# rrwick/Autocycler

Measured on AMD Instinct MI355X. Metric: Mbp/sec through compress->unitig GFA (k=51), higher is better.
Workload: dtype u64

## Files before the change

### autocycler_amd/csrc/capi.cpp

```cpp
#include <algorithm>
#include <cstring>
#include <memory>

#include "capi_common.hpp"
#include "gfa_writer.hpp"

using namespace ac;
using namespace ac::abi;

static void select_device(int device, bool refresh_tuning = true) {
    if (refresh_tuning) tuning_refresh();
#ifndef AC_EMU
    int n = 0;
    hipError_t e = hipGetDeviceCount(&n);
    if (e != hipSuccess || n == 0)
        throw DeviceError("no HIP device available: the MI355X backend has no CPU fallback");
    if (device < 0 || device >= n) throw DeviceError("invalid HIP device ordinal " + std::to_string(device));
    AC_HIP_CHECK(hipSetDevice(device));
    hipDeviceProp_t prop;
    AC_HIP_CHECK(hipGetDeviceProperties(&prop, device));
    if (std::string(prop.gcnArchName).rfind("gfx950", 0) != 0)
        throw DeviceError(std::string("device is ") + prop.gcnArchName + "; this library is built for gfx950 only");
#endif
    int& arena_device = device_ctx().arena_device;
    if (arena_device != device) {
        if (arena_device >= 0) {
            if (g_live_shards) throw DeviceError("a sharded build is in flight on device " + std::to_string(arena_device) + ": this process cannot use device " + std::to_string(device) + " until it is freed");
            Arena::device().release_all();
#ifndef AC_EMU
            Mailbox::get().release();
#endif
        }
        arena_device = device;
    }
}

namespace ac {
void select_device_checked(int device) { select_device(device, false); }

namespace abi __attribute__((visibility("hidden"))) {

std::string& last_error() { static thread_local std::string err; return err; }
std::mutex g_build_mutex;
int g_live_shards = 0;
std::atomic<int> g_host_side_device{0};

DeviceCall::DeviceCall(int device, Kind kind) : lock(g_build_mutex) {
    if (g_live_shards && kind != SHARD_PHASE)
        throw DeviceError(kind == SHARD_BEGIN ? "another sharded build is in flight in this process" : "a sharded build is in flight in this process");
    if (kind == ALL_DEVICES) tuning_refresh();
    else select_device(device);
}

void validate(uint32_t k, const ac_seq_view* seqs, uint32_t n_seqs) {
    if (!seqs || n_seqs == 0) throw DeviceError("no sequences found in input assemblies");
    if (k % 2 == 0) throw DeviceError("--kmer must be odd");
    if (n_seqs > 32767) throw DeviceError("no more than 32767 input sequences are allowed");
    for (uint32_t i = 0; i < n_seqs; i++) {
        if (!seqs[i].fwd) throw DeviceError("null sequence pointer");
        if (seqs[i].length < k) throw DeviceError("sequence shorter than k");
    }
}

void validate_layout(uint32_t k, uint64_t n_text, const uint64_t* off, const uint32_t* len, const uint16_t* d1, const uint16_t* d2,
                     uint32_t n_seqs) {
    if (k < 1 || k % 2 == 0) throw DeviceError("--kmer must be odd");
    if (!off || !len || !d1 || !d2) throw DeviceError("null sequence table");
    uint64_t prev_end = 0;
    for (uint32_t i = 0; i < n_seqs; i++) {
        if (len[i] < k) throw DeviceError("sequence " + std::to_string(i + 1) + " is shorter than k");
        const uint64_t plen = (uint64_t)len[i] + k - 1;
        if (off[i] != prev_end + 1) throw DeviceError("sequence table: sequence " + std::to_string(i + 1) + " does not start right behind the separator of the previous one");
        if (off[i] + plen + 1 > n_text) throw DeviceError("sequence table: sequence " + std::to_string(i + 1) + " runs past the end of the text");
        if (d1[i] > k - 1 || d2[i] > k - 1 || (uint32_t)d1[i] + d2[i] > k - 1) throw DeviceError("sequence table: more padding dots than k - 1 on sequence " + std::to_string(i + 1));
        prev_end = off[i] + plen;
    }
    if (n_seqs && prev_end + 1 != n_text) throw DeviceError("sequence table: the text does not end with the separator of the last sequence");
}

std::vector<SeqView> seq_views(const ac_seq_view* seqs, uint32_t n_seqs, std::vector<uint16_t>* seq_ids, std::vector<uint32_t>* seq_lens) {
    std::vector<SeqView> v(n_seqs);
    for (uint32_t i = 0; i < n_seqs; i++) {
        v[i] = SeqView{seqs[i].fwd, seqs[i].length};
        seq_ids->push_back(seqs[i].id);
        seq_lens->push_back(seqs[i].length);
    }
    return v;
}

void set_device_text(GraphBuilder& b, const void* d_text, uint64_t n_text, const uint64_t* seq_off, const uint32_t* seq_len,
                     const uint16_t* ids, const uint16_t* seq_d1, const uint16_t* seq_d2, uint32_t n_seqs,
                     std::vector<uint16_t>* seq_ids, std::vector<uint32_t>* seq_lens) {
    std::vector<uint64_t> off(seq_off, seq_off + n_seqs);
    std::vector<uint32_t> len(seq_len, seq_len + n_seqs);
    std::vector<uint16_t> d1(seq_d1, seq_d1 + n_seqs), d2(seq_d2, seq_d2 + n_seqs);
    seq_ids->assign(ids, ids + n_seqs);
    *seq_lens = len;
    b.set_text_device((const uint8_t*)d_text, n_text, off, len, d1, d2);
}

}
}

static void build_graph(GraphBuilder& b, uint32_t assembly_count, ac_graph* h) {
    b.build(assembly_count, &h->g);
    h->tm = b.timings();
}

template <class T> static size_t copy_sized(const T& full, T* out, size_t out_size) {
    memcpy(out, &full, std::min(out_size, sizeof full));
    return sizeof full;
}

extern "C" {

const char* ac_last_error(void) { return last_error().c_str(); }
const char* ac_version(void) {
#ifdef AC_EMU
    return "autocycler_amd 0.1 (CPU emulation, tests only)";
#else
    return "autocycler_amd 0.1 (gfx950)";
#endif
}
int ac_abi_version(void) { return AC_ABI_VERSION; }
int ac_set_host_side_device(int device) { if (device < 0) return fail("invalid HIP device ordinal"); g_host_side_device.store(device); return 0; }
void ac_set_stage_timing(int on) { set_stage_timing(on != 0); }
int ac_release_memory(void) {
    return guarded([&] {
        std::lock_guard<std::mutex> lock(g_build_mutex);
        if (g_live_shards) throw DeviceError("a sharded build is in flight in this process");
        Arena::device().release_all();
        release_multi_contexts();
        PinnedPool::get().trim();
        release_host_stager();
        scan_pool().release();
#ifndef AC_EMU
        Mailbox::get().release();
#endif
    });
}
uint32_t ac_max_kmer(void) { int m = max_supported_k(); return (uint32_t)(m % 2 ? m : m - 1); }
int ac_device_count(void) {
#ifndef AC_EMU
    int n = 0;
    if (hipGetDeviceCount(&n) != hipSuccess) return 0;
    return n;
#else
    return 0;
#endif
}

uint64_t ac_text_size(uint32_t k, const ac_seq_view* seqs, uint32_t n_seqs) {
    uint64_t n = 1;
    for (uint32_t i = 0; i < n_seqs; i++) n += (uint64_t)seqs[i].length + k - 1 + 1;
    return n;
}
int ac_layout_text(uint32_t k, const ac_seq_view* seqs, uint32_t n_seqs, uint8_t* text, uint64_t* seq_off,
                   uint16_t* seq_d1, uint16_t* seq_d2) {
    return guarded([&] {
        std::vector<SeqView> v(n_seqs);
        for (uint32_t i = 0; i < n_seqs; i++) v[i] = SeqView{seqs[i].fwd, seqs[i].length};
        std::vector<uint64_t> off; std::vector<uint32_t> len; std::vector<uint16_t> d1, d2;
        std::vector<uint8_t> t = layout_text(v, k, &off, &len, &d1, &d2);
        memcpy(text, t.data(), t.size());
        for (uint32_t i = 0; i < n_seqs; i++) { seq_off[i] = off[i]; seq_d1[i] = d1[i]; seq_d2[i] = d2[i]; }
    });
}

int ac_pack_text(const uint8_t* text, uint64_t n_text, uint64_t* bits, uint32_t* mask32, int force_scalar) {
    return guarded([&] {
        if (!text || !bits || !mask32) throw DeviceError("null pointer");
        pack_text_host(text, n_text, bits, mask32, force_scalar != 0);
    });
}

int ac_compress_build(uint32_t k, uint32_t assembly_count, const ac_seq_view* seqs, uint32_t n_seqs, int device,
                      ac_graph** out) {
    return guarded([&] {
        validate(k, seqs, n_seqs);
        DeviceCall call(device);
        auto h = std::make_unique<ac_graph>();
        const std::vector<SeqView> v = seq_views(seqs, n_seqs, &h->seq_ids, &h->seq_lens);
        GraphBuilder b(k);
        b.set_sequences_host(v);
        build_graph(b, assembly_count, h.get());
        *out = h.release();
    });
}

int ac_compress_build_multi(uint32_t k, uint32_t assembly_count, const ac_seq_view* seqs, uint32_t n_seqs, const int* devices, int n_devices,
                            ac_graph** out) {
    return guarded([&] {
        validate(k, seqs, n_seqs);
        if (!devices || n_devices < 1) throw DeviceError("ac_compress_build_multi: no devices");
        if (n_devices > 64) throw DeviceError("ac_compress_build_multi: more than 64 devices");
        DeviceCall call(-1, DeviceCall::ALL_DEVICES);
        auto h = std::make_unique<ac_graph>();
        const std::vector<SeqView> v = seq_views(seqs, n_seqs, &h->seq_ids, &h->seq_lens);
        int transport = MULTI_AUTO;
        if (const int e = tuning_multi_transport()) transport = e == 1 ? MULTI_HOST_STAGED : MULTI_RCCL;
        build_multi(k, assembly_count, v, std::vector<int>(devices, devices + n_devices), transport, &h->g, &h->tm, &h->multi);
        *out = h.release();
    });
}
int ac_multi_info_get(const ac_graph* g, ac_multi_info* o) {
    if (!g || !o) return fail("null pointer");
    const MultiStats& m = g->multi;
    memset(o, 0, sizeof *o);
    o->n_ranks = m.n_ranks; o->transport = m.transport;
    o->bytes_fragments = m.bytes_fragments; o->bytes_bitmap = m.bytes_bitmap; o->bytes_degrees = m.bytes_degrees; o->bytes_links = m.bytes_links;
    o->bytes_queries = m.bytes_queries; o->bytes_answers = m.bytes_answers; o->bytes_reduce = m.bytes_reduce;
    o->queries_total = m.queries_total; o->queries_sent_away = m.queries_sent_away;
    o->table_capacity_max = m.table_capacity_max; o->table_capacity_sum = m.table_capacity_sum;
    o->union_text_bytes = m.union_text_bytes; o->fragments = m.fragments; o->distinct = m.distinct;
    o->seconds_total = m.seconds_total; o->seconds_exchange_max = m.seconds_exchange_max;
    o->candidates_total = m.candidates_total; o->candidates_owned_max = m.candidates_owned_max;
    o->bytes_sibling = m.bytes_sibling; o->bytes_tail = m.bytes_tail; o->degrees_open = m.degrees_open; o->bytes_received_max = m.bytes_received_max;
    o->path_runs_copied = m.path_runs_copied;
    return 0;
}
size_t ac_multi_info_get_sized(const ac_graph* g, ac_multi_info* out, size_t out_size) {
    ac_multi_info t;
    if (!g || !out) { fail("null pointer"); return sizeof t; }
    ac_multi_info_get(g, &t);
    return copy_sized(t, out, out_size);
}

int ac_compress_build_device(uint32_t k, uint32_t assembly_count, const void* d_text, uint64_t n_text,
                             const uint64_t* seq_off, const uint32_t* seq_len, const uint16_t* seq_ids,
                             const uint16_t* seq_d1, const uint16_t* seq_d2, uint32_t n_seqs, int device,
                             ac_graph** out) {
    return guarded([&] {
        if (!d_text || n_seqs == 0) throw DeviceError("no sequences found in input assemblies");
        if (n_seqs > 32767) throw DeviceError("no more than 32767 input sequences are allowed");
        validate_layout(k, n_text, seq_off, seq_len, seq_d1, seq_d2, n_seqs);
        DeviceCall call(device);
        auto h = std::make_unique<ac_graph>();
        GraphBuilder b(k);
        set_device_text(b, d_text, n_text, seq_off, seq_len, seq_ids, seq_d1, seq_d2, n_seqs, &h->seq_ids, &h->seq_lens);
        build_graph(b, assembly_count, h.get());
        *out = h.release();
    });
}

uint32_t ac_graph_seq_count(const ac_graph* g) { return (uint32_t)g->seq_ids.size(); }
int ac_path_counts(const ac_graph* g, uint64_t* counts) {
    for (size_t s = 0; s + 1 < g->g.path_off.size(); s++) counts[s] = g->g.path_off[s + 1] - g->g.path_off[s];
    return 0;
}

uint32_t ac_graph_kmer_size(const ac_graph* g) { return g->g.k; }
int ac_graph_seq_info(const ac_graph* g, uint32_t i, uint16_t* id, uint32_t* length, const char** filename, const char** header) {
    if (i >= g->seq_ids.size()) return fail("sequence index out of range");
    if (id) *id = g->seq_ids[i];
    if (length) *length = g->seq_lens[i];
    if (filename) *filename = i < g->filenames.size() ? g->filenames[i].c_str() : nullptr;
    if (header) *header = i < g->headers.size() ? g->headers[i].c_str() : nullptr;
    return 0;
}

uint64_t ac_kmer_count(const ac_graph* g) { return g->g.n_kmers; }
ac_stats ac_stats_pre(const ac_graph* g) { return ac_stats{g->g.pre.unitigs, g->g.pre.links_one_way, g->g.pre.total_length}; }
ac_stats ac_stats_post(const ac_graph* g) { return ac_stats{g->g.post.unitigs, g->g.post.links_one_way, g->g.post.total_length}; }
uint32_t ac_unitig_count(const ac_graph* g) { return g->g.n_unitigs; }

int ac_unitig(const ac_graph* g, uint32_t idx, const uint8_t** seq, uint32_t* len, double* depth) {
    if (idx >= g->g.n_unitigs) return fail("unitig index out of range");
    if (!g->host_arrays) return fail("this rank kept no host arrays (sharded build, not the writing rank)");
    if (seq) *seq = (const uint8_t*)g->g.seq(idx);
    if (len) *len = g->g.seq_len[idx];
    if (depth) *depth = g->g.depth[idx];
    return 0;
}
int ac_unitig_positions(ac_graph* g, uint32_t idx, int forward, const ac_position** positions, uint32_t* n) {
    if (idx >= g->g.n_unitigs) return fail("unitig index out of range");
    return guarded([&] {
        if (!g->host_arrays || !g->host_paths) throw DeviceError("this rank kept no host arrays (sharded build, not the writing rank)");
        if (!g->positions_built) { build_positions(&g->g, g->seq_ids, g->seq_lens); g->positions_built = true; }
        auto& v = forward ? g->g.fwd_positions[idx] : g->g.rev_positions[idx];
        static_assert(sizeof(ac_position) == sizeof(Position), "layout");
        *positions = (const ac_position*)v.data();
        *n = (uint32_t)v.size();
    });
}
int ac_links(const ac_graph* g, const ac_link** links, uint64_t* n) {
    static_assert(sizeof(ac_link) == sizeof(Link), "layout");
    if (!g->host_arrays) return fail("this rank kept no host arrays (sharded build, not the writing rank)");
    *links = (const ac_link*)g->g.links;
    *n = g->g.n_links;
    return 0;
}
int ac_path(const ac_graph* g, uint32_t seq_index, const int32_t** signed_unitigs, uint32_t* n) {
    if ((size_t)seq_index + 1 >= g->g.path_off.size()) return fail("sequence index out of range");
    if (!g->host_paths) return fail("this rank kept no paths on the host (sharded build)");
    uint64_t b = g->g.path_off[seq_index], e = g->g.path_off[seq_index + 1];
    *signed_unitigs = g->g.path + b;
    *n = (uint32_t)(e - b);
    return 0;
}
int ac_unitigs_bulk(const ac_graph* g, const uint8_t** seq_bytes, const uint64_t** seq_begin, const uint32_t** seq_len, const double** depth) {
    if (!g->host_arrays) return fail("this rank kept no host arrays (sharded build, not the writing rank)");
    if (seq_bytes) *seq_bytes = (const uint8_t*)g->g.seq_block.p;
    if (seq_begin) *seq_begin = g->g.seq_begin;
    if (seq_len) *seq_len = g->g.seq_len;
    if (depth) *depth = g->g.depth;
    return 0;
}
int ac_paths_bulk(const ac_graph* g, const int32_t** path_entries, const uint64_t** path_off, uint64_t* n_entries) {
    if (!g->host_paths) return fail("this rank kept no paths on the host (sharded build)");
    if (path_entries) *path_entries = g->g.path;
    if (path_off) *path_off = g->g.path_off.data();
    if (n_entries) *n_entries = g->g.n_path;
    return 0;
}
int ac_timings_get(const ac_graph* g, ac_timings* o) {
    const BuildTimings& t = g->tm;
    o->h2d = t.h2d; o->pack = t.pack; o->insert = t.insert; o->collect_sort = t.collect_sort; o->degree = t.degree;
    o->segment = t.segment; o->minkey = t.minkey; o->rank = t.rank; o->paths = t.paths; o->links = t.links; o->seqs = t.seqs;
    o->d2h = t.d2h; o->total_device = t.total_device; o->expand = t.expand;
    o->insert_kernel_ms = t.insert_kernel_ms; o->insert_positions = t.insert_positions;
    o->table_capacity = t.table_capacity; o->n_distinct = t.n_distinct; o->n_path_entries = t.n_path_entries;
    o->simplify_passes = t.simplify_passes; o->n_candidates = t.n_candidates; o->n_levels = t.n_levels;
    o->insert_launches = t.insert_launches; o->insert_real = t.insert_real;
    o->analysis = t.analysis; o->finalize = t.finalize;
    o->fragments = t.fragments; o->union_pack = t.union_pack; o->union_insert = t.union_insert;
    o->n_local_distinct = t.n_local_distinct; o->n_fragments = t.n_fragments; o->fragment_bytes = t.fragment_bytes;
    o->upload_device_ms = t.upload_device_ms;
    o->path_runs_copied = t.path_runs_copied; o->path_entries_walked = t.path_entries_walked; o->position_retries = t.position_retries;
    o->n_candidates_owned = t.n_candidates_owned;
    o->launches = t.launches; o->readbacks = t.readbacks; o->n_degrees_open = t.n_degrees_open; o->sort_retries = t.sort_retries;
    o->insert_rest_known = t.insert_rest_known; o->insert_rest_sampled = t.insert_rest_sampled; o->path_stretches = t.path_stretches;
    o->expand_sparse_sweeps = t.expand_sparse_sweeps; o->expand_sparse_start = t.expand_sparse_start;
    return 0;
}
size_t ac_timings_get_sized(const ac_graph* g, ac_timings* out, size_t out_size) {
    ac_timings t;
    memset(&t, 0, sizeof t);
    ac_timings_get(g, &t);
    return out ? copy_sized(t, out, out_size) : sizeof t;
// ... 29 lines not shown
```

### autocycler_amd/csrc/device_rt.hpp

```cpp
#pragma once
#include <cstdio>
#include <cstdlib>
#include <cstring>
#include <stdexcept>
#include <string>
#include <vector>
#include <algorithm>

#include <mutex>
#include <time.h>
#include <unistd.h>

#include "kmer_ops.hpp"
#include "graph_types.hpp"
#include "wave_rt.hpp"

#ifndef AC_EMU
#include <hip/hip_runtime.h>
#endif
#if defined(AC_EMU) && defined(AC_ARENA_GUARD)
#include <sanitizer/asan_interface.h>
#define AC_GUARD_LEVEL AC_ARENA_GUARD
#else
#define AC_GUARD_LEVEL 0
#endif

namespace ac {

struct DeviceError : std::runtime_error { using std::runtime_error::runtime_error; };
struct NeedExactPositions {};
struct NeedCheckedSorts {};

#ifndef AC_EMU
#define AC_HIP_CHECK(expr)                                                                              \
    do {                                                                                                \
        hipError_t _e = (expr);                                                                         \
        if (_e != hipSuccess)                                                                           \
            throw ::ac::DeviceError(std::string("HIP error: ") + hipGetErrorString(_e) + " at " + __FILE__ + ":" + \
                                    std::to_string(__LINE__) + " (" #expr ")");                        \
    } while (0)
typedef hipStream_t stream_t;
#else
typedef int stream_t;
#endif

#ifdef AC_EMU
inline u64 atomic_cas64(u64* p, u64 expected, u64 desired) { u64 old = *p; if (old == expected) *p = desired; return old; }
inline u64 atomic_min64(u64* p, u64 v) { u64 o = *p; if (v < o) *p = v; return o; }
inline void atomic_max64(u64* p, u64 v) { if (v > *p) *p = v; }
inline void atomic_xor64(u64* p, u64 v) { *p ^= v; }
inline u32 atomic_add32(u32* p, u32 v) { u32 o = *p; *p += v; return o; }
inline u64 atomic_add64(u64* p, u64 v) { u64 o = *p; *p += v; return o; }
inline void atomic_or32(u32* p, u32 v) { *p |= v; }
inline void atomic_or64(u64* p, u64 v) { *p |= v; }
inline void atomic_min32(u32* p, u32 v) { if (v < *p) *p = v; }
inline void atomic_max32(u32* p, u32 v) { if (v > *p) *p = v; }
inline u32 atomic_cas32(u32* p, u32 expected, u32 desired) { u32 old = *p; if (old == expected) *p = desired; return old; }
inline u32 atomic_load32(const u32* p) { return *p; }
inline u32 atomic_fetch_or32(u32* p, u32 v) { u32 o = *p; *p |= v; return o; }
inline u32 atomic_fetch_and32(u32* p, u32 v) { u32 o = *p; *p &= v; return o; }
#else
__device__ inline u64 atomic_cas64(u64* p, u64 expected, u64 desired) {
    return (u64)atomicCAS((unsigned long long*)p, (unsigned long long)expected, (unsigned long long)desired);
}
__device__ inline u64 atomic_min64(u64* p, u64 v) { return (u64)atomicMin((unsigned long long*)p, (unsigned long long)v); }
__device__ inline void atomic_max64(u64* p, u64 v) { atomicMax((unsigned long long*)p, (unsigned long long)v); }
__device__ inline void atomic_xor64(u64* p, u64 v) { atomicXor((unsigned long long*)p, (unsigned long long)v); }
__device__ inline u32 atomic_add32(u32* p, u32 v) { return atomicAdd(p, v); }
__device__ inline u64 atomic_add64(u64* p, u64 v) { return (u64)atomicAdd((unsigned long long*)p, (unsigned long long)v); }
__device__ inline void atomic_or32(u32* p, u32 v) { atomicOr(p, v); }
__device__ inline void atomic_or64(u64* p, u64 v) { atomicOr((unsigned long long*)p, (unsigned long long)v); }
__device__ inline void atomic_min32(u32* p, u32 v) { atomicMin(p, v); }
__device__ inline void atomic_max32(u32* p, u32 v) { atomicMax(p, v); }
__device__ inline u32 atomic_cas32(u32* p, u32 expected, u32 desired) { return atomicCAS(p, expected, desired); }
__device__ inline u32 atomic_load32(const u32* p) { return __hip_atomic_load(p, __ATOMIC_RELAXED, __HIP_MEMORY_SCOPE_AGENT); }
__device__ inline u32 atomic_fetch_or32(u32* p, u32 v) { return atomicOr(p, v); }
__device__ inline u32 atomic_fetch_and32(u32* p, u32 v) { return atomicAnd(p, v); }
#endif

struct RtCounters { u32 launches = 0, readbacks = 0; };
inline RtCounters& rt_counters() { static thread_local RtCounters c; return c; }

struct DeviceCtx {
    static const int SLOTS = 10;
    void* obj[SLOTS] = {}; void (*del[SLOTS])(void*) = {};
    int arena_device = -1;
    DeviceCtx() {}
    DeviceCtx(const DeviceCtx&) = delete;
    DeviceCtx& operator=(const DeviceCtx&) = delete;
    ~DeviceCtx() { for (int i = SLOTS; i-- > 0;) if (obj[i]) del[i](obj[i]); }
};
inline DeviceCtx*& tl_device_ctx() { static thread_local DeviceCtx* p = nullptr; return p; }
inline DeviceCtx& device_ctx() {
    static DeviceCtx* const process_wide = new DeviceCtx;
    DeviceCtx* p = tl_device_ctx();
    return p ? *p : *process_wide;
}
inline void set_device_ctx(DeviceCtx* c) { tl_device_ctx() = c; }
enum { CTX_ARENA = 0, CTX_FILLS, CTX_MAILBOX, CTX_SIDE, CTX_SCRATCH, CTX_STAGER, CTX_POOL, CTX_SCANPOOL_RESERVED, CTX_POOL2 };
template <class T> T& ctx_object(int slot) {
    DeviceCtx& c = device_ctx();
    if (!c.obj[slot]) { c.obj[slot] = new T(); c.del[slot] = [](void* p) { delete (T*)p; }; }
    return *(T*)c.obj[slot];
}

class Arena {
  public:
    static Arena& device() { return ctx_object<Arena>(CTX_ARENA); }
    Arena() : host_(false) {}
    ~Arena() { for (auto& b : blocks_) raw_free(b.p); }
    static const size_t COALESCE_LIMIT = (size_t)16 << 30;
#if AC_GUARD_LEVEL
    static const size_t RED_ZONE = 256;
    static void guard_poison(const void* p, size_t n) { if (n) __asan_poison_memory_region(p, n); }
    static void guard_unpoison(const void* p, size_t n) { if (n) __asan_unpoison_memory_region(p, n); }
#else
    static const size_t RED_ZONE = 0;
    static void guard_poison(const void*, size_t) {}
    static void guard_unpoison(const void*, size_t) {}
#endif
    static void keep_readable(const void* p, size_t bytes) { guard_unpoison(p, bytes); }
    void* alloc(size_t bytes) {
        [[maybe_unused]] const size_t asked = bytes;
        bytes = (bytes + 255) & ~(size_t)255;
        if (bytes == 0) bytes = 256;
        bytes += RED_ZONE;
        size_t i = cur_;
        while (i < blocks_.size() && blocks_[i].used + bytes > blocks_[i].cap) i++;
        if (i == blocks_.size()) {
            Block b; b.cap = std::max(bytes, grow_); b.used = 0; b.p = raw_alloc(b.cap);
            blocks_.push_back(b);
        }
        cur_ = i;
        Block& b = blocks_[i];
        void* r = (char*)b.p + b.used;
        b.used += bytes;
        peak_ = std::max(peak_, total_used());
        guard_poison(r, bytes); guard_unpoison(r, asked);
        return r;
    }
    void reset() {
        on_reset();
        const size_t last_peak = peak_;
        peak_ = 0; cur_ = 0;
        size_t total = 0;
        for (auto& b : blocks_) total += b.cap;
        if (blocks_.size() > 1 && total <= COALESCE_LIMIT) {
            for (auto& b : blocks_) raw_free(b.p);
            if (last_peak) total = std::min(total, last_peak + last_peak / 8 + ((size_t)256 << 20));
            blocks_.clear();
            Block b; b.cap = total; b.used = 0; b.p = raw_alloc(total);
            blocks_.push_back(b);
        } else {
            for (auto& b : blocks_) { b.used = 0; guard_poison(b.p, b.cap); }
        }
    }
    void reserve(size_t bytes) {
        if (capacity() >= bytes || total_used() != 0) return;
        release_all();
        Block b; b.cap = bytes; b.used = 0; b.p = raw_alloc(bytes);
        blocks_.push_back(b);
    }
    void release_all() {
        on_reset();
        for (auto& b : blocks_) raw_free(b.p);
        blocks_.clear(); cur_ = 0;
    }
    struct Mark { size_t block, used; bool empty; };
    Mark mark() const { return blocks_.empty() ? Mark{0, 0, true} : Mark{cur_, blocks_[cur_].used, false}; }
    void rewind(const Mark& m) {
        on_rewind();
        if (blocks_.empty()) return;
        cur_ = m.empty ? 0 : m.block;
        const size_t keep = m.empty ? 0 : m.used;
        if (AC_GUARD_LEVEL >= 2) {
            if (blocks_[cur_].used > keep) guard_poison((char*)blocks_[cur_].p + keep, blocks_[cur_].used - keep);
            for (size_t i = cur_ + 1; i < blocks_.size(); i++) guard_poison(blocks_[i].p, blocks_[i].used);
        }
        blocks_[cur_].used = keep;
        for (size_t i = cur_ + 1; i < blocks_.size(); i++) blocks_[i].used = 0;
    }
    size_t peak() const { return peak_; }
    double alloc_seconds() const { return alloc_s_; }
    size_t total_used() const { size_t t = 0; for (auto& b : blocks_) t += b.used; return t; }
    size_t capacity() const { size_t t = 0; for (auto& b : blocks_) t += b.cap; return t; }
    void set_grow(size_t g) { grow_ = g; }
    size_t grow() const { return grow_; }
    bool locate(const void* p, size_t* block, size_t* offset, size_t* used) const {
        for (size_t i = 0; i < blocks_.size(); i++) {
            const char* lo = (const char*)blocks_[i].p;
            if ((const char*)p < lo || (const char*)p >= lo + blocks_[i].cap) continue;
            *block = i; *offset = (size_t)((const char*)p - lo); *used = blocks_[i].used;
            return true;
        }
        return false;
    }

  private:
    struct Block { void* p; size_t cap, used; };
    void on_reset();
    void on_rewind();
    static double wall() { timespec ts; clock_gettime(CLOCK_MONOTONIC, &ts); return (double)ts.tv_sec + 1e-9 * (double)ts.tv_nsec; }
    void* raw_alloc(size_t bytes) {
        const double t0 = wall();
        struct Acc { double& a; double t0; ~Acc() { a += wall() - t0; } } acc{alloc_s_, t0};
#ifdef AC_EMU
        void* p = malloc(bytes);
        if (!p) throw DeviceError("emu malloc failed");
        guard_poison(p, bytes);
        return p;
#else
        void* p = nullptr;
        if (host_) AC_HIP_CHECK(hipHostMalloc(&p, bytes, hipHostMallocDefault));
        else AC_HIP_CHECK(hipMalloc(&p, bytes));
        return p;
#endif
    }
    void raw_free(void* p) {
        const double t0 = wall();
#ifdef AC_EMU
        for (auto& b : blocks_) if (b.p == p) guard_unpoison(b.p, b.cap);
        free(p);
#else
        if (host_) (void)hipHostFree(p); else (void)hipFree(p);
#endif
        alloc_s_ += wall() - t0;
    }
    double alloc_s_ = 0;
    bool host_;
    std::vector<Block> blocks_;
    size_t grow_ = (size_t)64 << 20;
    size_t peak_ = 0, cur_ = 0;
};

class PinnedPool {
  public:
    static PinnedPool& get() { static PinnedPool p; return p; }
    HostBlock alloc(size_t bytes) {
        if (bytes == 0) bytes = 1;
        HostBlock b;
        {
            std::lock_guard<std::mutex> lock(mu_);
            size_t best = free_.size();
            for (size_t i = 0; i < free_.size(); i++)
                if (free_[i].cap >= bytes && free_[i].cap <= 2 * bytes + 4096 && (best == free_.size() || free_[i].cap < free_[best].cap)) best = i;
            if (best != free_.size()) {
                b.p = free_[best].p; b.bytes = free_[best].cap;
                held_ -= free_[best].cap;
                free_.erase(free_.begin() + (long)best);
            }
        }
        if (!b.p) {
// ... 671 lines not shown
```

### autocycler_amd/csrc/graph_build.hpp

```cpp
#pragma once
#include <cstdint>
#include <functional>
#include <string>
#include <vector>

#include "graph_types.hpp"
#include "trim_host.hpp"
#include "resolve_host.hpp"
#include "components_host.hpp"
#include "merge_host.hpp"
#include "subset_host.hpp"
#include "trim_apply_host.hpp"
#include "finish_host.hpp"
#include "apply_host.hpp"
#include "clean_host.hpp"
#include "cluster_host.hpp"
#include "cluster_qc_host.hpp"

namespace ac {

struct SeqView {
    const uint8_t* fwd;
    uint32_t length;
};

struct BuildTimings {
    double h2d = 0, pack = 0, insert = 0, collect_sort = 0, degree = 0, segment = 0, minkey = 0, rank = 0,
           paths = 0, links = 0, seqs = 0, d2h = 0, total_device = 0;
    double expand = 0;
    double analysis = 0;
    double finalize = 0;
    double insert_kernel_ms = 0;
    uint64_t insert_positions = 0;
    uint64_t table_capacity = 0;
    uint64_t n_distinct = 0;
    uint64_t n_path_entries = 0;
    uint32_t insert_launches = 0;
    uint64_t insert_real = 0;
    uint32_t simplify_passes = 0, n_candidates = 0, n_levels = 0;
    uint32_t n_candidates_owned = 0;
    uint32_t local_hint = 0, graph_hint = 0;
    double fragments = 0;
    double union_pack = 0, union_insert = 0;
    uint64_t n_local_distinct = 0, n_fragments = 0, fragment_bytes = 0;
    double upload_device_ms = 0;
    double insert_rest_known = 0;
    uint64_t path_stretches = 0;
    uint32_t expand_sparse_sweeps = 0;
    uint32_t expand_sparse_start = 0;
    double insert_rest_sampled = 0;
    uint32_t sort_retries = 0;
    uint32_t position_retries = 0;
    uint32_t launches = 0, readbacks = 0;
    uint64_t n_degrees_open = 0;
    uint64_t path_runs_copied = 0, path_entries_walked = 0;
};

struct RepairTimings { double total = 0, scan_ms = 0; uint64_t hits = 0, matches = 0; uint32_t patterns = 0; };

class GraphBuilder {
  public:
    explicit GraphBuilder(uint32_t k);
    ~GraphBuilder();
    void set_sequences_host(const std::vector<SeqView>& seqs, bool pack_now = true);
    void repair_ends(RepairTimings* tm);
    void set_text_device(const uint8_t* d_text, uint64_t n_text, const std::vector<uint64_t>& off,
                         const std::vector<uint32_t>& len, const std::vector<uint16_t>& d1,
                         const std::vector<uint16_t>& d2);
    void build(uint32_t assembly_count_hint, FinalGraph* out);

    void shard_begin(uint32_t local_assembly_hint);
    uint64_t local_distinct_count() const;
    void set_distinct_upper_bound(uint64_t n);
    uint64_t fragment_text_bytes() const;
    uint64_t fragment_count() const;
    void fragments_export(void* d_text_out, void* d_meta_out);
    uint64_t fragment_packed_words(uint64_t union_off) const;
    void fragments_export_packed(uint64_t union_off, void* d_words_out, void* d_meta_out);
    void shard_build_union_packed(uint32_t rank, uint32_t n_shards, const void* d_staged_words, const uint64_t* first_word, const uint64_t* n_words,
                                  uint64_t n_union_text, const void* d_meta, uint64_t n_frags_total);
    void shard_build_union(uint32_t rank, uint32_t n_shards, const uint8_t* d_union_text, uint64_t n_union_text,
                           const void* d_meta, uint64_t n_frags_total);
    uint64_t bitmap_words() const;
    void bitmap_export(void* d_out);
    void shard_build_novel(const void* d_bitmap_sum);
    uint64_t sib_words() const;
    void sib_export(void* d_out);
    void shard_degrees(const void* d_sib_sum);
    uint64_t degree_bytes() const;
    uint64_t distinct_count() const;
    void degrees_export(void* d_out);
    void shard_build_graph(const void* d_kinfo_sum);
    uint32_t unitig_count() const;
    void links_export(void* d_links_i32, void* d_wlinks_i64);
    void links_import(const void* d_links_i32, const void* d_wlinks_i64);
    uint64_t query_count() const;
    uint32_t query_key_words() const;
    void queries_export(void* d_out);
    void answer_queries(const void* d_keys, uint64_t n, void* d_out);
    void shard_walk(const void* d_answers_mine);
    void queries_route(uint32_t n_shards, void* d_routed_keys, uint64_t* counts_host);
    void shard_walk_routed(const void* d_routed_answers);
    void reduce_export(int32_t* d_sum, int32_t* d_min);
    void reduce_import(const int32_t* d_sum, const int32_t* d_min);
    void set_tail_exchange(std::function<void(void*, uint64_t, int, int)> all_reduce);
    void shard_finish(FinalGraph* out, bool want_graph, bool want_paths);
    uint64_t path_entry_count() const;
    void paths_export(void* d_out);
    const BuildTimings& timings() const { return tm_; }
    void set_sequence_index_base(uint64_t n);
    static void set_upload_threads_cap(int n);
    uint64_t n_text() const;
    uint64_t n_bases() const;

    struct Impl;

  private:
    void build_union_impl(uint32_t rank, uint32_t n_shards, const uint8_t* d_union_text, const void* d_staged_words, const uint64_t* first_word,
                          const uint64_t* n_words, uint64_t n_union_text, const void* d_meta, uint64_t n_frags_total);
    void upload_packed(const std::vector<SeqView>& seqs, const std::vector<uint64_t>& off);
    Impl* impl_;
    BuildTimings tm_;
};

std::vector<uint8_t> layout_text(const std::vector<SeqView>& seqs, uint32_t k, std::vector<uint64_t>* off,
                                 std::vector<uint32_t>* len, std::vector<uint16_t>* d1, std::vector<uint16_t>* d2);

void end_repair_device(uint32_t k, uint8_t* d_text, uint64_t n_text, const std::vector<uint64_t>& off, const std::vector<uint32_t>& len,
                       std::vector<uint16_t>* d1, std::vector<uint16_t>* d2, RepairTimings* tm, bool reset_arena = true);

void pairwise_distances_device(const FinalGraph& g, uint32_t n_seqs, double* out);

struct VerifyReport {
    uint32_t failed = 0;
    uint64_t first_bad_unitig = ~0ULL, first_bad_link = ~0ULL, first_bad_path_entry = ~0ULL, first_bad_sequence = ~0ULL, first_bad_base = ~0ULL;
    uint64_t unitigs = 0, links = 0, path_entries = 0, bases_checked = 0, self_mirror_links = 0;
    double seconds = 0;
    uint32_t checks = 0;
    uint64_t first_bad_junction = ~0ULL;
};
void verify_graph_device(const FinalGraph& g, const uint8_t* d_text, uint64_t n_text, const std::vector<uint64_t>& off,
                         const std::vector<uint32_t>& len, VerifyReport* rep);

void decompress_device(const FinalGraph& g, const std::vector<uint32_t>& seq_len, uint8_t* out_host);
struct TrimDeviceStats { double seconds_device = 0; uint64_t cells = 0; uint32_t jobs = 0, launches = 0; };
void overlap_alignment_batch(const std::vector<AlignJob>& jobs, const uint32_t* weights, uint32_t max_unitigs, std::vector<AlignOut>* outs,
                             TrimDeviceStats* st);
uint32_t trim_max_unitigs();
struct ResolveDeviceStats { double seconds_device = 0; uint64_t cells = 0, jobs = 0, largest_job_cells = 0; uint32_t launches = 0; };
void path_distance_batch(const PathPool& pool, const std::vector<PathPair>& pairs, const uint32_t* weights, std::vector<uint32_t>* dist,
                         ResolveDeviceStats* st);
uint32_t resolve_max_path();
struct ClusterDeviceStats { double seconds = 0; uint64_t rescans = 0, compares = 0; uint32_t launches = 0; };
void cluster_merges_device(const double* asym, uint32_t n, std::vector<ClusterRowMerge>* merges, ClusterDeviceStats* st);
void cluster_merges_graph_device(const FinalGraph& g, uint32_t n_seqs, double* asym_out, std::vector<ClusterRowMerge>* merges, ClusterDeviceStats* st);
uint32_t cluster_max_seqs();
struct ClusterQcDeviceStats {
    double seconds = 0;
    uint32_t launches = 0, readbacks = 0, evaluations = 0, pair_batches = 0;
    uint64_t alternatives = 0, pairs_counted = 0, bytes_read_back = 0;
};
void cluster_qc_device(const double* asym, uint32_t n, const uint32_t* dfs_tip, double cutoff, const std::function<void(const ClusterQcEvaluate&)>& body,
                       ClusterQcDeviceStats* st);
void components_device(uint32_t n_unitigs, const Link* links, uint64_t n_links, const uint32_t* unitig_len, const uint8_t* alive, const uint8_t* marked,
                       ComponentsResult* out);
struct MergePlanInput {
    uint32_t n_unitigs = 0; const Link* links = nullptr; uint64_t n_links = 0; const uint32_t* unitig_len = nullptr; const uint8_t* alive = nullptr;
    const uint8_t* seed_fixed = nullptr; const int32_t* path = nullptr; uint64_t n_path = 0;
    const uint8_t* seq_bytes = nullptr; const uint64_t* seq_begin = nullptr; uint64_t seq_total = 0;
};
void merge_plan_device(const MergePlanInput& in, MergeResult* out);
struct SubsetInput {
    uint32_t n_unitigs = 0; const Link* links = nullptr; uint64_t n_links = 0; const uint32_t* unitig_len = nullptr; const uint8_t* alive = nullptr;
    const int32_t* path = nullptr; const uint64_t* path_off = nullptr; uint32_t n_clusters = 0; const SubsetPlan* plan = nullptr;
};
void subsets_device(const SubsetInput& in, SubsetResult* out);
struct MergedPathsInput {
    uint32_t n_unitigs = 0; const uint32_t* unitig_len = nullptr; const int32_t* path = nullptr; const uint64_t* path_off = nullptr;
    const SubsetPlan* plan = nullptr; size_t kept_first = 0, kept_count = 0; const MergeResult* merge = nullptr;
};
void merged_paths_device(const MergedPathsInput& in, MergedPathsResult* out);
struct TrimApplyInput {
    uint32_t n_unitigs = 0; const Link* links = nullptr; uint64_t n_links = 0; const uint32_t* unitig_len = nullptr; const uint8_t* alive = nullptr;
    const int32_t* path = nullptr; const uint64_t* path_off = nullptr; double mad = 0;
};
void trim_apply_device(const TrimApplyInput& in, TrimApplyPlan* tp, SubsetPlan* plan, SubsetResult* out);
struct FinishInput {
    uint32_t n_unitigs = 0; const Link* links = nullptr; uint64_t n_links = 0; const uint32_t* unitig_len = nullptr; const uint8_t* alive = nullptr;
    const double* depth = nullptr; const uint8_t* type = nullptr; const uint8_t* seq_bytes = nullptr; const uint64_t* seq_begin = nullptr; uint64_t seq_total = 0;
    const MergeResult* plan = nullptr; const int32_t* path = nullptr; uint64_t n_path = 0; bool renumber = false; uint64_t unitigs_after = 0;
};
void merge_finish_device(const FinishInput& in, FinishResult* out);
void apply_bridges_device(const ApplyInput& in, const ApplyPlan& plan, ApplyResult* out);
void clean_device(const CleanInput& in, CleanResult* out);
void primitives_selftest(uint64_t n, uint64_t seed, int end_bit, int key_kind);
void selftest_scan(int kind, const void* in, uint64_t n, bool in_place, int misalign_in, int misalign_out, void* out);
void selftest_radix(const uint64_t* keys, const void* vals, uint64_t n, int begin_bit, int end_bit, int val_kind, uint64_t prep_n, int prep_bits, bool prep_reuse,
                    uint64_t* keys_out, void* vals_out);
void selftest_segments(int op, const uint32_t* seg, const uint64_t* vals, uint64_t n, uint64_t n_segments, bool deferred_err, void* out, uint32_t* err_out);
void selftest_sort_cmp(int form, const uint64_t* a, const uint32_t* b, const uint32_t* vals, uint64_t n, uint64_t* a_out, uint32_t* b_out, uint32_t* vals_out);
void selftest_scan_pool(int op, uint64_t value, uint64_t* out);
void selftest_wave(int program, const uint64_t* in_u64, const int32_t* aux_i32, const uint64_t* live_mask, uint64_t* out_u64);
void selftest_fills(const uint64_t* regions, uint64_t n_regions, int trigger, int mode, uint8_t* span, uint64_t span_bytes, uint32_t* launches_out);
void selftest_fill_order(uint64_t n, int byte1, uint64_t w_lo, uint64_t w_hi, int w_val, uint64_t from2, int byte2, uint64_t upto3, int byte3, uint8_t* out);
void selftest_readback(const uint8_t* data, uint64_t n_data, int path, const uint64_t* items, uint64_t n_items, uint8_t* out, uint32_t* counters_out);
void selftest_scalar_chain(const uint64_t* values, uint64_t n, uint64_t* out, uint32_t* counters_out);
void selftest_arena(const uint64_t* ops, uint64_t n_ops, uint64_t* totals_out, uint64_t* allocs_out, const uint8_t* live, uint64_t* wrong_out);
void selftest_launch(int which, uint64_t n, uint64_t* slots_out, uint32_t* info_out);
void selftest_atomics(int op, uint64_t init, uint64_t expected, const uint64_t* operand, const uint32_t* target, uint32_t n_words, uint64_t* words_out, uint64_t* returns_out);
void selftest_side_order(int mode, int which, uint32_t seed, uint64_t n_words, uint32_t* out_words);
void selftest_event_ring(int op, const uint8_t* kinds, uint32_t n_more, uint64_t* out);

void random_access_ceilings(double* cas_gops, double* read_gops, uint64_t table_slots = (uint64_t)1 << 24);

void device_warmup(int device, uint32_t k = 0, uint64_t text_bytes_estimate = 0);

void pack_text_host(const uint8_t* text, uint64_t n_text, uint64_t* bits, uint32_t* mask32, bool force_scalar);

void release_host_stager();

int max_supported_k();
void tuning_refresh();
int tuning_multi_transport();
bool tuning_multi_fragments_as_bytes();
bool tuning_multi_tail_replicated();
void set_stage_timing(bool on);
bool stage_timing();

}
```

### autocycler_amd/csrc/graph_impl.hpp

```cpp
#pragma once
#include "graph_build.hpp"

#include <chrono>
#include <cmath>
#include <map>
#include <string>
#include <algorithm>
#include <atomic>
#include <thread>
#include <functional>
#include <condition_variable>
#include <mutex>
#include <fcntl.h>
#include <unistd.h>
#if defined(__x86_64__)
#include <immintrin.h>
#endif

#include "device_rt.hpp"

namespace ac {

static double now_s() {
    return std::chrono::duration<double>(std::chrono::steady_clock::now().time_since_epoch()).count();
}



static const int MAX_PROBES = 1 << 14;
static const int MAX_PROBES_INSERT = 1 << 10;
#ifndef AC_W_ONLY
#define AC_W_ONLY 0
#endif
extern bool g_stage_timing;

static const u32 KI_OUT_MASK = 7u, KI_IN_SHIFT = 3, KI_FIRST_T = 1u << 6, KI_FIRST_RCT = 1u << 7;

struct TextCtx {
    const u64* bits;
    const u64* mask;
    u64 n_text;
    int k;
    const u64* seq_off;
    const u32* seq_len;
    const u16* seq_d1;
    const u16* seq_d2;
    u32 n_seqs;
};

struct Table {
    u64* slots;
    u64 cap_mask;
    const u64* occ;
    u64* novel;
    u32 n_owners;
    u32 my_owner;
    u64* sflags;
    u64* full_at;
    u64* runs; u32* run_count; u64 run_row0;
};
static const u64 RUN_MIN = 128;
static const u32 RUN_ROW = 128;
AC_D void run_note(const Table& tb, u64 wave, u32& noted, u64 pj, u64 qj, bool same, u64 n) {
    if (!tb.runs || n < RUN_MIN || noted >= RUN_ROW) return;
    u64* rec = tb.runs + 3 * ((tb.run_row0 + wave) * RUN_ROW + noted);
    noted++;
    const bool with_anchor = ((tb.novel[qj >> 6] >> (qj & 63)) & 1) != 0;
    if (with_anchor) { rec[0] = pj; rec[1] = n + 1; rec[2] = qj | ((u64)(same ? 1 : 0) << 63); }
    else { rec[0] = pj + 1; rec[1] = n; rec[2] = (same ? qj + 1 : qj - 1) | ((u64)(same ? 1 : 0) << 63); }
}
AC_D void run_note_done(const Table& tb, u64 wave, u32 noted) { if (tb.runs) tb.run_count[tb.run_row0 + wave] = noted; }
AC_D void sib_note(const Table& tb, u64 s, u32 fl) { if (fl) atomic_or64(&tb.sflags[s >> 5], (u64)fl << (2 * (s & 31))); }
AC_HD u32 sib_bits(u64 v, u64 mine) {
    const u64 d = v ^ mine;
    if ((d >> TAG_MFP_SHIFT) != 0 || slot_isdot(v) || (d >> 41) == 0) return 0;
    return (((d >> TAG_X_SHIFT) & 3) == 0 ? 1u : 0u) | (((d >> TAG_Y_SHIFT) & 3) == 0 ? 2u : 0u);
}
AC_HD bool table_owns(const Table& tb, u64 home_hash) { return tb.n_owners <= 1 || (u32)((home_hash >> 40) % tb.n_owners) == tb.my_owner; }

AC_HD bool locate(const TextCtx& t, u64 p, u32* s_out, u32* f_out) {
    if (t.n_seqs == 0 || p < t.seq_off[0]) return false;
    u32 lo = 0, hi = t.n_seqs;
    while (hi - lo > 1) {
        u32 mid = lo + ((hi - lo) >> 1);
        if (t.seq_off[mid] <= p) lo = mid; else hi = mid;
    }
    u64 f = p - t.seq_off[lo];
    if (f >= (u64)t.seq_len[lo]) return false;
    *s_out = lo; *f_out = (u32)f;
    return true;
}

template <int W> AC_HD bool xkmer_at(const TextCtx& t, u64 p, XKmer<W>* x) {
    u32 s, f;
    if (!locate(t, p, &s, &f)) return false;
    int k = t.k;
    int plen = (int)t.seq_len[s] + k - 1;
    int ld = (int)t.seq_d1[s] - (int)f;
    int td = (int)f + k - (plen - (int)t.seq_d2[s]);
    x->ld = ld > 0 ? ld : 0;
    x->td = td > 0 ? td : 0;
    x->fwd = text_extract<W>(t.bits, p, k);
    return true;
}

template <int W> AC_HD int claimant_match(const TextCtx& t, u64 v, const Key<W>& ukey) {
    XKmer<W> y;
    if (!slot_isdot(v)) {
        y.fwd = text_extract<W>(t.bits, slot_pos(v), t.k);
        y.ld = 0; y.td = 0;
    } else {
        if (!xkmer_at<W>(t, slot_pos(v), &y)) return 0;
    }
    bool yf;
    Key<W> yk = xk_canonical<W>(y, t.k, &yf);
    if (!key_eq<W>(yk, ukey)) return 0;
    return yf ? 2 : 1;
}

struct FindResult { u64 pos; int claimant_flipped; bool found; };

template <int W> AC_HD FindResult table_find(const TextCtx& t, const Table& tb, const Key<W>& ukey, bool isdot) {
    const KeyPlace pl = key_place<W>(ukey, t.k, isdot, key_hash<W>(ukey));
    u64 tag = slot_make(pl.tag, isdot, 0);
    const u64 hh = pl.home;
    u64 s = hh & tb.cap_mask;
    FindResult r; r.found = false; r.pos = 0; r.claimant_flipped = 0;
    if (!table_owns(tb, hh)) return r;
    if (tb.occ && !((tb.occ[s >> 6] >> (s & 63)) & 1)) return r;
    for (int probes = 0; probes < MAX_PROBES; probes++) {
        u64 v = tb.slots[s];
        if (v == SLOT_EMPTY) return r;
        if (slot_tag_eq(v, tag)) {
            int m = claimant_match<W>(t, v, ukey);
            if (m) { r.found = true; r.pos = slot_pos(v); r.claimant_flipped = (m == 2); return r; }
        }
        s = (s + 1) & tb.cap_mask;
    }
    return r;
}

template <int W> AC_HD bool find_xk(const TextCtx& t, const Table& tb, const XKmer<W>& x, u64* pos, bool* rel_same) {
    bool flipped;
    Key<W> uk = xk_canonical<W>(x, t.k, &flipped);
    FindResult r = table_find<W>(t, tb, uk, x.ld > 0 || x.td > 0);
    if (!r.found) return false;
    *pos = r.pos;
    *rel_same = ((r.claimant_flipped != 0) == flipped);
    return true;
}

template <int W> AC_HD bool owns_xk(const TextCtx& t, const Table& tb, const XKmer<W>& x) {
    if (tb.n_owners <= 1) return true;
    bool flipped;
    Key<W> uk = xk_canonical<W>(x, t.k, &flipped);
    return table_owns(tb, key_home<W>(uk, t.k, x.ld > 0 || x.td > 0, key_hash<W>(uk)));
}

struct Novel {
    const u64* bm;
    const u32* wprefix;
};
AC_HD int popc64(u64 x) {
#ifdef AC_EMU
    return __builtin_popcountll(x);
#else
    return __popcll(x);
#endif
}
AC_HD u32 novel_rank(const Novel& nv, u64 pos) {
    u64 w = pos >> 6;
    int b = (int)(pos & 63);
    u64 below = b ? (nv.bm[w] & ((1ULL << b) - 1)) : 0;
    return nv.wprefix[w] + (u32)popc64(below);
}

static const u64 NOREF = ~0ULL;

template <int W> AC_D u64 table_insert(const TextCtx& t, const Table& tb, const Key<W>& ukey, bool isdot, bool flipped, u64 p,
                                       u32* claimed, u32* err, bool* same, bool* mine_now) {
    const KeyPlace pl = key_place<W>(ukey, t.k, isdot, key_hash<W>(ukey));
    u64 mine = slot_make(pl.tag, isdot, p);
    const u64 hh = pl.home;
    u64 s = hh & tb.cap_mask;
    *mine_now = false;
    if (!table_owns(tb, hh)) return NOREF;
    const bool note = tb.sflags != nullptr && !isdot;
    u32 my_fl = 0;
    for (int probes = 0; probes < MAX_PROBES_INSERT; probes++) {
        u64 v = tb.slots[s];
        if (v == SLOT_EMPTY) {
            u64 old = atomic_cas64(&tb.slots[s], SLOT_EMPTY, mine);
            if (old == SLOT_EMPTY) { (*claimed)++; *mine_now = true; if (note) sib_note(tb, s, my_fl); return NOREF; }
            v = old;
        }
        if (slot_tag_eq(v, mine)) {
            if (slot_pos(v) == p) { if (note) sib_note(tb, s, my_fl); return NOREF; }
            int m = claimant_match<W>(t, v, ukey);
            if (m) {
                if (note) sib_note(tb, s, my_fl);
                if (slot_pos(v) > p) {
                    u64 old = atomic_min64(&tb.slots[s], mine);
                    if (old > mine) {
                        *mine_now = true;
                        u64 q = slot_pos(old);
                        atomic_xor64(&tb.novel[q >> 6], 1ULL << (q & 63));
                    }
                    return NOREF;
                }
                *same = ((m == 2) == flipped);
                return slot_pos(v);
            }
        } else if (note) {
            const u32 fl = sib_bits(v, mine);
            if (fl) { sib_note(tb, s, fl); my_fl |= fl; }
        }
        s = (s + 1) & tb.cap_mask;
    }
    atomic_or32(err, 1u);
    if (tb.full_at) atomic_max64(tb.full_at, ~p);
    return NOREF;
}

struct alignas(16) V16 { u32 a, b, c, d; };

#include "kernels_table.inc"
#include "kernels_unitigs.inc"
#include "kernels_paths.inc"
#include "kernels_tail.inc"
#include "kernels_shard.inc"
struct PathRemapJob {
    int32_t* path = nullptr; u64 n_ent = 0;
    const int32_t* rec_val = nullptr; const u32* rec_pos = nullptr; u64 n_rec = 0;
    const u32* number = nullptr; u32 n_unitigs = 0;
    u64 ent_limit = ~0ULL;
    void* landed = nullptr; SideStream* side = nullptr;
    int dev = 0;
    std::atomic<u64> next{0}; std::atomic<int> ready{0};
    std::atomic<u32> bad{0};
    u64 ticket = 0; bool started = false;
    std::atomic<double> t_ready{0}, t_last{0};
};
void path_remap_range(int32_t* p, u64 n, const u32* number, u32 n_unitigs, std::atomic<u32>* bad);
void path_stretch_range(const PathRemapJob& j, u64 s0, u64 s1, std::atomic<u32>* bad);
bool path_remap_is_wide();
void path_remap_start(PathRemapJob& j, int threads);
void path_remap_finish(PathRemapJob& j) noexcept;
struct SeqExpandJob {
    const u64* words = nullptr; u8* out = nullptr; u64 total = 0;
    void* landed = nullptr; SideStream* side = nullptr; int dev = 0;
    std::atomic<u64> next{0}; std::atomic<int> ready{0};
    u64 ticket = 0; bool started = false;
    std::atomic<double> t_start{0}, t_ready{0}, t_last{0};
};
void seq_expand_range(const u64* words, u8* out, u64 b, u64 e);
void seq_expand_start(SeqExpandJob& j, int threads);
void seq_expand_finish(SeqExpandJob& j) noexcept;
[[maybe_unused]] static int key_words(int k) { int w = words_for_k(k); return w <= 4 ? w : (w <= 8 ? 8 : 16); }
[[maybe_unused]] static u64 next_pow2(u64 x) { u64 p = 1; while (p < x) p <<= 1; return p; }
[[maybe_unused]] static size_t arena_estimate(u64 n_text, bool owns_text) { return (size_t)n_text * (owns_text ? 8 : 7) + ((size_t)768 << 20); }
struct Knobs {
    int minkey_variant;
    int path_copy;
    u64 run_piece;
    u32 pos_cap;
    bool path_filter;
    int host_remap_mode;
    u32 remap_block;
    int minkey_prefix_bases;
    bool seed_prefix_sort;
    u32 seed_max_group;
    int seed_prefix_bits;
    u32 degree_region_cap;
    int upload_direct_mode;
    int upload_slots;
    int degree_flags;
    int table_shift;
    u64 wave_chunk_max;
    u64 insert_chunk_rest_env;
    bool host_pack;
    u32 expand_level_table;
    bool shard_path_copy;
    bool expand_rewrite_always;
    u32 expand_sparse_max, expand_sparse_list, expand_sparse_batch;
    u32 stretch_device_share;
    int seq_codes_transfer;
    int late_copies;
    bool seq_writer_plain;
    bool seq_writer_forced;
    u64 seed_radix_limit;
    bool upload_overlap;
    bool sort_checks_deferrable;
    bool shard_host_remap;
    bool shard_degree_flags;
    bool insert_adaptive;
    u64 insert_growth;
    u64 insert_waves_target;
    bool renum_two_pass;
    u32 renum_max_group;
    u32 path_chunk_env;
    long upload_threads_env;
    bool debug_arena;
    bool degree_diag;
    int multi_transport;
    int multi_fragments;
    int multi_tail;
    u64 trim_batch_bytes;
    u64 resolve_batch_bytes;
    static Knobs read() {
        Knobs k;
        k.minkey_variant = [&]() -> int { const char* e = getenv("AC_MINKEY_VARIANT"); return e ? atoi(e) : -1; }();
        k.path_copy = [&]() -> int { const char* e = getenv("AC_PATH_COPY"); return e ? (atoi(e) != 0 ? 1 : 0) : 2; }();
        k.run_piece = [&]() -> u64 { const char* e = getenv("AC_RUN_PIECE"); const long v = e ? atol(e) : 0; return v > 0 ? (u64)v : 4096; }();
        k.pos_cap = [&]() -> u32 { const char* e = getenv("AC_POS_CAP"); const long v = e ? atol(e) : 65536; return v < 0 ? 0u : (u32)std::min<long>(v, 0x3FFFFFFF); }();
        k.path_filter = [&]() -> bool { const char* e = getenv("AC_PATH_FILTER"); return e ? atoi(e) != 0 : true; }();
        k.host_remap_mode = [&]() -> int { const char* e = getenv("AC_HOST_REMAP"); return e ? (atoi(e) == 2 ? 2 : (atoi(e) != 0 ? 1 : 0)) : -1; }();
        k.remap_block = [&]() -> u32 { const char* e = getenv("AC_REMAP_BLOCK"); int v = e ? atoi(e) : 4096; v = v < 64 ? 64 : (v > 65536 ? 65536 : v); return (u32)(v & ~63); }();
        k.minkey_prefix_bases = [&]() -> int { const char* e = getenv("AC_MINKEY_PREFIX_BASES"); int v = e ? atoi(e) : 31; return v < 1 ? 1 : (v > 31 ? 31 : v); }();
        k.seed_prefix_sort = [&]() -> bool { const char* e = getenv("AC_SEED_PREFIX_SORT"); return e ? atoi(e) != 0 : true; }();
        k.seed_max_group = [&]() -> u32 { const char* e = getenv("AC_SEED_MAX_GROUP"); int v = e ? atoi(e) : 1024; return (u32)(v < 1 ? 1 : v); }();
        k.seed_prefix_bits = [&]() -> int { const char* e = getenv("AC_SEED_PREFIX_BITS"); if (!e) return 0; int v = atoi(e); return v < 1 ? 1 : (v > 64 ? 64 : v); }();
        k.degree_region_cap = [&]() -> u32 { const char* e = getenv("AC_DEGREE_REGION_CAP"); int v = e ? atoi(e) : 0; return (u32)(v < 0 ? 0 : v); }();
        k.upload_direct_mode = [&]() -> int { const char* e = getenv("AC_UPLOAD_DIRECT"); return e ? (atoi(e) != 0 ? 1 : 0) : -1; }();
        k.upload_slots = [&]() -> int { const char* e = getenv("AC_UPLOAD_SLOTS"); int v = e ? atoi(e) : 1 << 20; return v < 1 ? 1 : v; }();
        k.degree_flags = [&]() -> int { const char* e = getenv("AC_DEGREE_FLAGS"); return e ? (atoi(e) != 0 ? 1 : 0) : 1; }();
        k.table_shift = [&]() -> int { const char* e = getenv("AC_TABLE_SHIFT"); if (!e) return -1; int v = atoi(e); return v < 0 ? 0 : (v > 3 ? 3 : v); }();
        k.wave_chunk_max = [&]() -> u64 { const char* e = getenv("AC_INSERT_CHUNK"); u64 x = e ? (u64)atoll(e) : 8192; return (std::max<u64>(x, 256) + 63) & ~63ULL; }();
        k.insert_chunk_rest_env = [&]() -> u64 { const char* e = getenv("AC_INSERT_CHUNK_REST"); if (!e) return 0; return (std::max<u64>((u64)atoll(e), 256) + 63) & ~63ULL; }();
        k.host_pack = [&]() -> bool { const char* e = getenv("AC_HOST_PACK"); return e ? atoi(e) != 0 : true; }();
        k.expand_level_table = [&]() -> u32 { const char* e = getenv("AC_EXPAND_LEVEL_TABLE"); int v = e ? atoi(e) : 1024; return (u32)(v < 1 ? 1 : v); }();
        k.shard_path_copy = [&]() -> bool { const char* e = getenv("AC_SHARD_PATH_COPY"); return !(e && atoi(e) == 0); }();
        k.expand_rewrite_always = [&]() -> bool { return getenv("AC_EXPAND_REWRITE_ALWAYS") != nullptr; }();
        k.expand_sparse_max = [&]() -> u32 { const char* e = getenv("AC_EXPAND_SPARSE_MAX"); int v = e ? atoi(e) : 256; return (u32)(v < 0 ? 0 : v); }();
        k.late_copies = [&]() -> int { const char* e = getenv("AC_LATE_COPIES"); return e ? atoi(e) : 1; }();
        k.seq_codes_transfer = [&]() -> int { const char* e = getenv("AC_SEQ_CODES"); return e ? atoi(e) : 1; }();
        k.stretch_device_share = [&]() -> u32 { const char* e = getenv("AC_STRETCH_DEVICE_SHARE"); int v = e ? atoi(e) : 30; return (u32)(v < 0 ? 0 : v); }();
        k.expand_sparse_list = [&]() -> u32 { const char* e = getenv("AC_EXPAND_SPARSE_LIST"); int v = e ? atoi(e) : 0; return (u32)(v < 0 ? 0 : v); }();
        k.expand_sparse_batch = [&]() -> u32 { const char* e = getenv("AC_EXPAND_SPARSE_BATCH"); int v = e ? atoi(e) : 4096; return (u32)(v < 1 ? 1 : v); }();
        k.seq_writer_plain = [&]() -> bool { const char* e = getenv("AC_SEQ_WRITER"); return e && atoi(e) == 0; }();
        k.seq_writer_forced = [&]() -> bool { const char* e = getenv("AC_SEQ_WRITER"); return e && atoi(e) == 1; }();
        k.seed_radix_limit = [&]() -> u64 { const char* e = getenv("AC_SEED_RADIX_LIMIT"); return e ? (u64)atoll(e) : (1u << 19); }();
        k.upload_overlap = [&]() -> bool { const char* e = getenv("AC_UPLOAD_OVERLAP"); return e ? atoi(e) != 0 : true; }();
        k.sort_checks_deferrable = [&]() -> bool { const char* e = getenv("AC_SORT_CHECKS"); return !(e && atoi(e) == 1); }();
        k.shard_host_remap = [&]() -> bool { const char* e = getenv("AC_SHARD_HOST_REMAP"); return e ? atoi(e) != 0 : true; }();
        k.shard_degree_flags = [&]() -> bool { const char* e = getenv("AC_SHARD_DEGREE_FLAGS"); return e ? atoi(e) != 0 : true; }();
        k.insert_adaptive = [&]() -> bool { const char* e = getenv("AC_INSERT_ADAPT"); return e ? atoi(e) != 0 : true; }();
        k.insert_growth = [&]() -> u64 { const char* e = getenv("AC_INSERT_GROWTH"); long x = e ? atol(e) : 2; return (u64)(x < 2 ? 2 : x); }();
        k.insert_waves_target = [&]() -> u64 { const char* e = getenv("AC_INSERT_WAVES"); long x = e ? atol(e) : 16384; return (u64)(x < 1024 ? 1024 : x); }();
        k.renum_two_pass = [&]() -> bool { const char* e = getenv("AC_RENUM_TWO_PASS"); return e && atoi(e) != 0; }();
        k.renum_max_group = [&]() -> u32 { const char* e = getenv("AC_RENUM_MAX_GROUP"); int v = e ? atoi(e) : 64; return (u32)(v < 1 ? 1 : (v > 64 ? 64 : v)); }();
        k.path_chunk_env = [&]() -> u32 { const char* e = getenv("AC_PATH_CHUNK"); if (!e) return 0; int v = atoi(e); return (u32)(v < 64 ? 64 : (v > 4096 ? 4096 : v)); }();
        k.upload_threads_env = [&]() -> long { const char* e = getenv("AC_UPLOAD_THREADS"); return e ? atol(e) : 24; }();
        k.debug_arena = [&]() -> bool { return getenv("AC_DEBUG_ARENA") != nullptr; }();
        k.degree_diag = [&]() -> bool { return getenv("AC_DEGREE_DIAG") != nullptr; }();
        k.multi_transport = [&]() -> int { const char* e = getenv("AC_MULTI_TRANSPORT"); return !e ? 0 : (!strcmp(e, "host") ? 1 : (!strcmp(e, "rccl") ? 2 : 0)); }();
        k.multi_fragments = [&]() -> int { const char* e = getenv("AC_MULTI_FRAGMENTS"); return e && !strcmp(e, "bytes") ? 1 : 0; }();
        k.multi_tail = [&]() -> int { const char* e = getenv("AC_MULTI_TAIL"); return e && !strcmp(e, "replicated") ? 1 : 0; }();
        k.trim_batch_bytes = [&]() -> u64 { const char* e = getenv("AC_TRIM_BATCH_BYTES"); const long long v = e ? atoll(e) : 0; return v > 0 ? (u64)v : (u64)4 << 30; }();
        k.resolve_batch_bytes = [&]() -> u64 { const char* e = getenv("AC_RESOLVE_BATCH_BYTES"); const long long v = e ? atoll(e) : 0; return v > 0 ? (u64)v : (u64)1 << 30; }();
        return k;
    }
};
const Knobs& knobs();
void knobs_refresh();

[[maybe_unused]] static int minkey_variant() { return knobs().minkey_variant; }
[[maybe_unused]] static int path_copy() { return knobs().path_copy; }
[[maybe_unused]] static bool path_copy_pays(u64 n_text, u32 assemblies, u32 k, double r2) {
    const double A = (double)std::max<u32>(assemblies, 1);
    const double entries = (double)n_text * std::min(1.0, 2.0 * A * r2 / (double)k);
    const double saving = entries * 53e-12 * std::max(0.0, 1.0 - 2.0 / A), cost = 0.25e-3 + 0.3e-12 * (double)n_text;
    return saving > 1.5 * cost;
}
[[maybe_unused]] static u64 run_piece() { return knobs().run_piece; }
[[maybe_unused]] static u32 pos_cap() { return knobs().pos_cap; }
[[maybe_unused]] static bool path_filter() { return knobs().path_filter; }
#ifdef AC_MEASUREMENT_KNOBS
[[maybe_unused]] static int path_diag() { const char* e = getenv("AC_PATH_DIAG"); return e ? (atoi(e) & 3) : 0; }
#else
[[maybe_unused]] static int path_diag() { return 0; }
#endif
[[maybe_unused]] static u32 path_chunk(u64 n_kmers, u32 n_unitigs) {
    if (knobs().path_chunk_env) return knobs().path_chunk_env;
    const u64 want = 5 * n_kmers / std::max<u32>(n_unitigs, 1);
    u32 pc = 64;
    while (pc < 2048 && (u64)pc * 3 / 2 < want) pc *= 2;
    return pc;
}
[[maybe_unused]] static int host_remap_mode() { return knobs().host_remap_mode; }
[[maybe_unused]] static u32 remap_block() { return knobs().remap_block; }
[[maybe_unused]] static int minkey_prefix_bases() { return knobs().minkey_prefix_bases; }
[[maybe_unused]] static bool seed_prefix_sort() { return knobs().seed_prefix_sort; }
[[maybe_unused]] static u32 seed_max_group() { return knobs().seed_max_group; }
[[maybe_unused]] static int seed_prefix_bits() { return knobs().seed_prefix_bits; }
[[maybe_unused]] static u32 degree_region_cap() { return knobs().degree_region_cap; }
[[maybe_unused]] static u64 upload_chunk_bytes() { return (u64)64 << 20; }
[[maybe_unused]] static int upload_direct_mode() { return knobs().upload_direct_mode; }
[[maybe_unused]] static int upload_slots() { return knobs().upload_slots; }
[[maybe_unused]] static int degree_flags() { return knobs().degree_flags; }
[[maybe_unused]] static int table_shift() { return knobs().table_shift; }
[[maybe_unused]] static u64 wave_chunk_max() { return knobs().wave_chunk_max; }
[[maybe_unused]] static u64 wave_chunk_rest() { return 16384; }
[[maybe_unused]] static u64 insert_chunk_rest_env() { return knobs().insert_chunk_rest_env; }
static thread_local int tl_upload_threads_cap = 0;
[[maybe_unused]] static u64 upload_threads() {

    long x = knobs().upload_threads_env;
    if (tl_upload_threads_cap > 0 && x > tl_upload_threads_cap) x = tl_upload_threads_cap;
    return (u64)(x < 1 ? 1 : (x > 128 ? 128 : x));
}
[[maybe_unused]] static bool host_pack() { return knobs().host_pack; }
[[maybe_unused]] static bool insert_profile() { static const bool v = getenv("AC_INSERT_PROFILE") != nullptr; return v; }
[[maybe_unused]] static u32 expand_level_table() { return knobs().expand_level_table; }
[[maybe_unused]] static bool shard_path_copy() { return knobs().shard_path_copy; }
[[maybe_unused]] static u32 expand_sparse_max() { return knobs().expand_sparse_max; }
[[maybe_unused]] static int late_copies() { return knobs().late_copies; }
[[maybe_unused]] static int seq_codes_transfer() { return knobs().seq_codes_transfer; }
[[maybe_unused]] static u32 stretch_device_share() { return knobs().stretch_device_share; }
[[maybe_unused]] static u32 expand_sparse_list() { return knobs().expand_sparse_list; }
[[maybe_unused]] static u32 expand_sparse_batch() { return knobs().expand_sparse_batch; }
[[maybe_unused]] static bool expand_rewrite_always() { return knobs().expand_rewrite_always; }
[[maybe_unused]] static bool seq_writer_plain() { return knobs().seq_writer_plain; }
[[maybe_unused]] static bool seq_writer_forced() { return knobs().seq_writer_forced; }
[[maybe_unused]] static u64 seed_radix_limit() { return knobs().seed_radix_limit; }
[[maybe_unused]] static bool upload_overlap() { return knobs().upload_overlap; }
[[maybe_unused]] static bool sort_checks_deferrable() { return knobs().sort_checks_deferrable; }
[[maybe_unused]] static bool shard_host_remap() { return knobs().shard_host_remap; }
[[maybe_unused]] static bool shard_degree_flags() { return knobs().shard_degree_flags; }
[[maybe_unused]] static bool insert_adaptive() { return knobs().insert_adaptive; }
[[maybe_unused]] static u64 insert_growth() { return knobs().insert_growth; }
[[maybe_unused]] static u64 insert_waves_target() { return knobs().insert_waves_target; }

struct PackedText {
    const u8* d_text = nullptr;
    u64 n_text = 0, n_bases = 0;
    u32 n_seqs = 0;
    int any_dots = 0; u64 n_dotted = 0;
    DBuf<u64> seq_off; DBuf<u32> seq_len; DBuf<u16> seq_d1, seq_d2; DBuf<u8> seq_flags;
    bool has_flags = false;
    DBuf<u64> bits, mask;
    DBuf<u32> pack_bad; bool check_alphabet = false; int k = 0; u64 expected_nonbase = 0;
    u64 index_base = 0;
    PackCheck chk() const { return PackCheck{seq_off.ptr(), seq_len.ptr(), seq_d1.ptr(), seq_d2.ptr(), n_seqs, k, check_alphabet ? const_cast<u32*>(pack_bad.ptr()) : nullptr}; }
    std::vector<u64> h_off; std::vector<u32> h_len;
    void set_table(const std::vector<uint64_t>& off, const std::vector<uint32_t>& len, const std::vector<uint16_t>& d1,
                   const std::vector<uint16_t>& d2, const std::vector<uint8_t>* flags = nullptr) {
        n_seqs = (u32)off.size();
        h_off = off; h_len = len;
        seq_off.alloc(n_seqs); seq_len.alloc(n_seqs); seq_d1.alloc(n_seqs); seq_d2.alloc(n_seqs);
        copy_h2d(seq_off.ptr(), off.data(), (size_t)n_seqs * 8);
        copy_h2d(seq_len.ptr(), len.data(), (size_t)n_seqs * 4);
        copy_h2d(seq_d1.ptr(), d1.data(), (size_t)n_seqs * 2);
        copy_h2d(seq_d2.ptr(), d2.data(), (size_t)n_seqs * 2);
        has_flags = flags != nullptr;
        if (flags) { seq_flags.alloc(n_seqs); copy_h2d(seq_flags.ptr(), flags->data(), n_seqs); }
        n_bases = 0; any_dots = 0; n_dotted = 0; expected_nonbase = (u64)n_seqs + 1;
        for (u32 i = 0; i < n_seqs; i++) { n_bases += len[i]; if (d1[i] || d2[i]) { any_dots = 1; n_dotted++; } expected_nonbase += (u64)d1[i] + d2[i]; }
        stream_sync();
    }
    void alloc_table(u32 n) { n_seqs = n; h_off.clear(); h_len.clear(); seq_off.alloc(n); seq_len.alloc(n); seq_d1.alloc(n); seq_d2.alloc(n); seq_flags.alloc(n); has_flags = true; }
    void set_sums(u64 bases, u64 dotted, u64 dots) { n_bases = bases; n_dotted = dotted; any_dots = dotted ? 1 : 0; expected_nonbase = (u64)n_seqs + 1 + dots; }
    TextCtx ctx(int k) const { return TextCtx{bits.ptr(), mask.ptr(), n_text, k, seq_off.ptr(), seq_len.ptr(), seq_d1.ptr(), seq_d2.ptr(), n_seqs}; }
    bool packed = false;
    void pack_alloc(stream_t s = 0) {
        u64 n_bits_words = n_text / 32 + 24, n_mask_words = n_text / 64 + 12;
        bits.alloc(n_bits_words); mask.alloc(n_mask_words);
        const u64 groups = (n_text + 31) / 32;
        bits.fill_bytes_from(groups * 8, 0, s);
        mask.fill_bytes_from(groups * 4, 0xFF, s);
        if (check_alphabet) { pack_bad.alloc(2); pack_bad.fill_bytes(0xFF, s); }
    }
    void verify_alphabet(const u32* bad) const {
        if (!check_alphabet) return;
        if (bad[0] != 0xFFFFFFFFu) throw DeviceError("input sequence " + std::to_string(index_base + bad[0]) + " contains non-ACGT characters");
        const u64 found = (u64)(u32)(bad[1] + 1u);
        if (found != (expected_nonbase & 0xFFFFFFFFULL))
            throw DeviceError("the text does not match its sequence table: " + std::to_string(expected_nonbase) + " padding dots and separators expected, " +
                              std::to_string(found) + " non-ACGT characters found");
    }
    void pack() {
        if (packed) return;
        pack_alloc();
        launch((n_text + 31) / 32, PackFunctor{d_text, n_text, bits.ptr(), (u32*)mask.ptr(), 0, chk()});
        packed = true;
    }
};

struct GraphBuilder::Impl {
    u32 k = 0;
    DBuf<u8> text_owned;
    PackedText loc;
    PackedText uni;
    PackedText* G = &loc;
    BuildTimings* tm = nullptr;
    double t0 = 0, t_begin = 0;
    void lap(double* acc) { if (!g_stage_timing) return; stream_sync(); double t = now_s(); *acc += t - t0; t0 = t; }

    DBuf<u32> counters;
    DBuf<u64> slots; u64 cap = 0; u64 N = 0;
    DBuf<u64> bm; DBuf<u32> wprefix; DBuf<u64> npos;
    u32 U = 0;
    DBuf<u32> kinfo, head, scan, ustart, order, rank, ulen;
    DBuf<u64> ustartpos, useq_off; DBuf<u8> uorient;
    DBuf<int32_t> links; DBuf<u64> wlinks;
    DBuf<u32> depth, minpos_fwd, minpos_rev; DBuf<u64> path_off; DBuf<int32_t> ent_val; u64 n_ent = 0;
    DBuf<u64> wl_text; DBuf<u32> depth_u, minpos_fwd_u, minpos_rev_u, run_start, run_end;
    void walk_arrays();
    void walk_tables(bool filter);
    void walk_to_seed_order();
    bool walked_plain = false;
    DBuf<u8> fs0, fe0;
    u32 pos_cap_now = 0xFFFFFFFFu; bool exact_positions = false;
    bool host_remap_allowed = false;
    bool paths_in_seed_numbers = false;
    bool checked_sorts = false; DBuf<u32> sort_flags;
    bool deferred_sort_checks() const { return host_remap_allowed_build && !checked_sorts && sort_checks_deferrable(); }
    bool host_remap_allowed_build = false;
    DBuf<u8> maybe_dest; bool maybe_dest_valid = false;
    DBuf<u8> frag_text; DBuf<u64> frag_meta, frag_fpos, frag_boff; u64 frag_bytes = 0, n_frags = 0;
    u64 distinct_upper = 0;

    void begin(BuildTimings* t) {
        tm = t; t_begin = t0 = now_s();
        rt_counters() = RtCounters();
        host_remap_allowed = false;
        counters.alloc(8); counters.fill_bytes(0);
        sort_flags.alloc(2); sort_flags.fill_bytes(0);
    }
    void check_sizes(const PackedText& t) const {
        if (t.n_text >= POS_MASK) throw DeviceError("input too large for 40-bit text positions");
        if (t.n_seqs == 0 || t.n_text < (u64)k + 2) throw DeviceError("no sequences");
    }
    template <int W> void insert(const PackedText& t, u32 hint, DBuf<u64>* slots_out, u64* cap_out, u64* n_distinct_out, DBuf<u64>* bm_out, bool want_sib = false);
    DBuf<u64> sflags;
    DBuf<u64> runs; DBuf<u32> run_count; u64 run_rows = 0, run_rows_cap = 0;
    DBuf<u64> loc_bm; DBuf<u32> loc_wprefix; bool local_insert_of_shard = false;
    struct CopyPlan { bool ok = false; u64 R = 0, NW = 0, Rb = 0; DBuf<RunRec> rr; DBuf<u32> rseq; DBuf<u64> wfirst, w_begin, w_end; DBuf<u32> w_gap; } cplan;
    void occupancy_bitmap(const DBuf<u64>& sl, u64 c, DBuf<u64>* occ_out, const u64* sflags_in, u64* sib_out, stream_t s = 0);
    DBuf<u64> occ;
    DBuf<u64> sib;
    DBuf<u64> sibn; bool sib_pending = false;
    DBuf<u32> kcontrib, pend, pidx; u64 n_pending = 0, n_first = 0;
    DBuf<u64> endset, endset_bloom; u64 endset_mask = 0;
    u32 n_owners = 1, my_owner = 0;
    void* upload_done = nullptr; u64 upload_avail = 0; bool upload_pending = false;
    struct UploadJob {
#ifndef AC_EMU
        const std::vector<SeqView>* seqs = nullptr;
        std::vector<uint64_t> off;
        uint32_t k = 0; u64 n = 0, CH = 0, SUB = 0, n_chunks = 0, slot_bytes = 0; int NSLOT = 0, dev = 0;
        hipStream_t up = nullptr, pk = nullptr;
        u64* d_bits = nullptr;
        bool direct = false;
        double t_start = 0; std::atomic<u64> chunks_issued{0}; std::atomic<double> t_last{0};
        hipEvent_t fills_done = nullptr;
        std::atomic<u64> next{0}, nonbase{0}, bar_sink{0}; u64 expected_nonbase = 0;
        std::vector<std::atomic<u32>> done, slot_state, issued;
        std::vector<hipEvent_t> landed;
        std::mutex hip_mu; std::string fail; std::atomic<bool> stop{false};
        u64 ticket = 0;
        void* stager = nullptr;
        u64 next_wait = 0;
        void run();
#endif
    };
    UploadJob* job = nullptr;
    u64 upload_rest_limit(u64 pb) const;
    void need_text(u64 upto);
    void finish_upload();
    ~Impl();
    void pack_overlapped(u32 hint) {
        PackedText& pt = loc;
        if (pt.packed) return;
#ifndef AC_EMU
        const u64 p_end_all = pt.n_text - (u64)k + 1;
        const u64 first = std::max<u64>(p_end_all / std::max<u32>(hint, 1), 1u << 16);
        const u64 H = (first + (u64)k + 8192 + 4095) & ~4095ULL;
        const u64 cap_est = next_pow2(std::max<u64>(1024, pt.n_bases / std::max<u32>(hint, 1) * 3 + 4096));
        if (cap_est <= (1ULL << 25) && H + (1u << 22) < pt.n_text) {
            pt.pack_alloc();
            launch(H / 32, PackFunctor{pt.d_text, pt.n_text, pt.bits.ptr(), (u32*)pt.mask.ptr(), 0, pt.chk()});
            SideStream& side = SideStream::get();
            side.after_main();
            launch((pt.n_text + 31) / 32 - H / 32, PackFunctor{pt.d_text, pt.n_text, pt.bits.ptr(), (u32*)pt.mask.ptr(), H / 32, pt.chk()}, side.stream());
            upload_done = side.mark(); upload_avail = H; upload_pending = true;
            pt.packed = true;
            return;
        }
#endif
        pt.pack();
    }
    Table graph_table() const { return Table{const_cast<u64*>(slots.ptr()), cap - 1, occ.ptr(), nullptr, n_owners, my_owner, nullptr, nullptr, nullptr, nullptr, 0}; }
    template <int W> void fragments();
    template <int W> void table();
    void novel_list(u64 known_n);
    template <int W> void degrees();
    template <int W> void walk_queries();
    template <int W> void answer_queries(const u64* d_keys, u64 n, u64* d_out);
    DBuf<u64> qkeys; u64 n_queries = 0;
    DBuf<u32> qidx;
    DBuf<u64> qanswers;
    template <int W> void route_queries(u32 n_shards, u64* d_routed_keys, u64* counts_host);
    const u64* walk_answers = nullptr;
    template <int W> void unitigs();
    template <int W> void walk();
    template <int W> bool walk_copy_prepare(u32 PC, const Novel& nv_text);
    template <int W> void walk_copy_finish(u32 PC);
    void tail(FinalGraph* out, bool want_graph, bool want_paths);
    std::function<void(void*, uint64_t, int, int)> tail_xchg;
};

inline void GraphBuilder::Impl::occupancy_bitmap(const DBuf<u64>& sl, u64 c, DBuf<u64>* occ_out, const u64* sflags_in, u64* sib_out, stream_t s) {
    occ_out->alloc((c + 63) / 64);
#ifdef AC_EMU
    occ_out->fill_bytes(0);
#endif
    launch_full(c, MarkFunctor{sl.ptr(), occ_out->ptr(), sflags_in, sib_out}, s);
}
inline void GraphBuilder::Impl::novel_list(u64 known_n) {
    PackedText& g = *G;
    u64 n_bm_words = g.n_text / 64 + 1;
    DBuf<u32> wcnt(n_bm_words + 1);
    wprefix.alloc(n_bm_words + 1);
    launch(n_bm_words + 1, PopcFunctor{bm.ptr(), wcnt.ptr(), n_bm_words});
    exclusive_scan_u32(wcnt.ptr(), wprefix.ptr(), n_bm_words + 1);
    if (known_n) N = known_n;
    else {
        N = read_scalar(wprefix.ptr() + n_bm_words);
        if (N == 0) throw DeviceError("internal error: no k-mers in the union of the shards");
        tm->n_distinct = N;
    }
    npos.alloc(N);
    launch_wave_kernel(fill_novel_wave_kernel<0>, (n_bm_words + 255) / 256, 0, (const u64*)bm.ptr(), (const u32*)wprefix.ptr(), npos.ptr(), n_bm_words);
    kinfo.alloc(N, true);
    head.alloc(N + 1); scan.alloc(N + 1);
    head.fill_bytes_from(N * 4, 0); scan.fill_bytes_from(N * 4, 0);
    lap(&tm->collect_sort);
}

inline void GraphBuilder::Impl::walk_arrays() {
    wl_text.alloc((u64)U * 10);
    depth_u.alloc(U, true); minpos_fwd_u.alloc(U); minpos_rev_u.alloc(U);
    run_start.alloc((u64)U + 1, true); run_end.alloc((u64)U + 1, true);
}
inline void GraphBuilder::Impl::walk_tables(bool filter) {
    launch((u64)U * 10, WlinkFlagFunctor{filter ? maybe_dest.ptr() : nullptr, wlinks.ptr(), counters.ptr() + 4});
    const u32 pos_init = pos_cap_now == 0xFFFFFFFFu ? 0xFFFFFFFFu : ((pos_cap_now + 1) | POS_BOUND);
    launch((u64)U * 10, WlinkTextOrderFunctor{wlinks.ptr(), rank.ptr(), order.ptr(), uorient.ptr(), wl_text.ptr(), minpos_fwd_u.ptr(), minpos_rev_u.ptr(), pos_init});
}
inline void GraphBuilder::Impl::walk_to_seed_order() {
    depth.alloc(U); minpos_fwd.alloc(U); minpos_rev.alloc(U);
    DBuf<u32> started, ended;
    if (walked_plain) {
        started.alloc((u64)U + 1); ended.alloc((u64)U + 1);
        inclusive_scan_u32(run_start.ptr(), started.ptr(), (u64)U + 1);
        exclusive_scan_u32(run_end.ptr(), ended.ptr(), (u64)U + 1);
    }
    launch(U, WalkToSeedOrderFunctor{order.ptr(), depth_u.ptr(), walked_plain ? started.ptr() : nullptr, walked_plain ? ended.ptr() : nullptr,
                                     minpos_fwd_u.ptr(), minpos_rev_u.ptr(), depth.ptr(), minpos_fwd.ptr(), minpos_rev.ptr()});
}

template <int W> struct Stages {
    static void table(GraphBuilder::Impl& m);
    static void degrees(GraphBuilder::Impl& m);
    static void walk_queries(GraphBuilder::Impl& m);
    static void answer_queries(GraphBuilder::Impl& m, const u64* d_keys, u64 n, u64* d_out);
    static void route_queries(GraphBuilder::Impl& m, u32 n_shards, u64* d_routed_keys, u64* counts_host);
    static void unitigs(GraphBuilder::Impl& m);
    static void walk(GraphBuilder::Impl& m);
    static void fragments(GraphBuilder::Impl& m);
    static void warm();
};

void tail_warm();

#define AC_DISPATCH_W(NAME, ARGS)                                        \
    switch (key_words((int)impl_->k)) {                                  \
        case 1: Stages<1>::NAME ARGS; break;                             \
        case 2: Stages<2>::NAME ARGS; break;                             \
        case 3: Stages<3>::NAME ARGS; break;                             \
        case 4: Stages<4>::NAME ARGS; break;                             \
        case 8: Stages<8>::NAME ARGS; break;                             \
        case 16: Stages<16>::NAME ARGS; break;                           \
        default: throw DeviceError("unsupported k");                     \
    }

}
```

### autocycler_amd/csrc/graph_stages.hip

```cpp
#include "graph_impl.hpp"

namespace ac {

template <int W>
void GraphBuilder::Impl::insert(const PackedText& pt, u32 hint, DBuf<u64>* slots_out, u64* cap_out, u64* n_distinct_out, DBuf<u64>* bm_out, bool want_sib) {
    TextCtx t = pt.ctx((int)k);
    const u64 p_end_all = pt.n_text - (u64)k + 1;
    if (hint == 0) hint = 1;
    u64 est = pt.n_bases / hint;
    u64 c = next_pow2(std::max<u64>(1024, est * 3 + 4096));
    if (&pt == &uni && distinct_upper) {
        const u64 mine = distinct_upper / std::max<u32>(n_owners, 1) + distinct_upper / (8 * (u64)std::max<u32>(n_owners, 1)) + 4096;
        c = next_pow2(std::max<u64>(1024, mine * 10 / 7));
    }
    if (c > next_pow2(pt.n_bases * 2 + 1024)) c = next_pow2(pt.n_bases * 2 + 1024);
    const int shift = table_shift() >= 0 ? table_shift() : (c > (1ULL << 25) ? 0 : 1);
    c <<= shift;
    struct CapMemo { u64 n_text = 0, cap = 0; u32 k = 0; int shift = -2; u32 owners = 0; };
    static thread_local CapMemo memo[4]; static thread_local unsigned memo_next = 0;
    const u32 memo_owners = (&pt == &uni) ? n_owners : 1u;
    for (const CapMemo& m : memo)
        if (pt.n_text == m.n_text && k == m.k && m.shift == table_shift() && m.owners == memo_owners && m.cap > c) c = m.cap;
    const int copy_mode = (&pt == &loc && (want_sib || (local_insert_of_shard && shard_path_copy()))) ? path_copy() : 0;
    bool want_runs = false;
    DBuf<InsertStats> istats(257);
    DBuf<u64> sl;
    DBuf<u64> nbm(pt.n_text / 64 + 2);
    u64 n_distinct = 0;
    const Arena::Mark retry_mark = Arena::device().mark();
    std::vector<u64> phase_end;
    for (;;) {
        sl.alloc(c);
        sl.fill_bytes(0xFF);
        nbm.fill_bytes(0);
        counters.fill_bytes(0);
        istats.fill_bytes(0);
        if (want_sib) { sflags.alloc(c / 32 + 1); sflags.fill_bytes(0); }
        else sflags = DBuf<u64>();
        u32* ierr = (u32*)&istats.ptr()[256].real;
        Table tb{sl.ptr(), c - 1, nullptr, nbm.ptr(), (&pt == &uni) ? n_owners : 1u, (&pt == &uni) ? my_owner : 0u, want_sib ? sflags.ptr() : nullptr,
                 &istats.ptr()[256].claimed, nullptr, nullptr, 0};
        if (&pt == &loc) { runs = DBuf<u64>(); run_count = DBuf<u32>(); run_rows = run_rows_cap = 0; cplan = CopyPlan(); }
        phase_end.clear();
        stream_sync();
#ifndef AC_EMU
        std::vector<hipEvent_t> evs;
        flush_fills();
#endif
        u32 launches = 0;
        u64 rest_chunk = wave_chunk_rest();
        u64 first = std::max<u64>(p_end_all / hint, 1u << 16);
        u64 pb = 0;
        bool rest_at_once = false;
        while (pb < p_end_all) {
            const bool diverse = launches >= 2 && !rest_at_once && insert_adaptive();
            u64 pe = (pb == 0) ? first : pb * (diverse ? std::max<u64>(insert_growth(), 4) : insert_growth());
            if (rest_at_once || pe > p_end_all || p_end_all - pe < (1u << 16)) pe = p_end_all;
#ifndef AC_EMU
            if (upload_pending && &pt == &loc && pe + (u64)k + 8192 > upload_avail) {
                flush_fills();
                SideStream::get().consumed(upload_done);
                AC_HIP_CHECK(hipStreamWaitEvent(0, (hipEvent_t)upload_done, 0));
                upload_pending = false;
            }
            if (job && &pt == &loc) {
                if (rest_at_once) pe = std::min<u64>(pe, upload_rest_limit(pb));
                need_text(pe + (u64)k + 8192);
            }
#endif
            const u64 len = pe - pb;
            {
                u64 c = (len / (diverse ? std::max<u64>(insert_waves_target(), 65536) : insert_waves_target()) + 63) & ~63ULL;
                u32 chunk = (u32)std::min<u64>(std::max<u64>(c, 256), rest_at_once ? rest_chunk : wave_chunk_max());
                u64 n_waves = (len + chunk - 1) / chunk;
                if (want_runs && rest_at_once) {
                    if (!run_rows_cap) {
                        run_rows_cap = 2 * ((p_end_all - pb) / chunk + 1) + n_waves + 64;
                        run_rows_cap = std::min<u64>(run_rows_cap, 4 * (pt.n_text / rest_chunk + 1) + n_waves + 1024);
                        runs.alloc(3 * run_rows_cap * RUN_ROW); run_count.alloc(run_rows_cap + 1);
                        run_count.fill_bytes(0);
                    }
                    if (run_rows + n_waves <= run_rows_cap) { tb.runs = runs.ptr(); tb.run_count = run_count.ptr(); tb.run_row0 = run_rows; run_rows += n_waves; }
                    else tb.runs = nullptr;
                }
                const u64 blocks = (n_waves + 3) / 4;
#ifndef AC_EMU
                if (insert_profile()) {
                    DBuf<u64> prof(16);
                    prof.fill_bytes(0);
                    launch_wave_kernel(insert_wave_kernel<W, true>, blocks, 0, t, tb, pb, pe, chunk, istats.ptr(), ierr, prof.ptr());
                    std::vector<u64> h = to_host(prof, 16);
                    fprintf(stderr, "insert launch %u: positions %llu chunk %u waves %llu | opener %llu steps avg %.0f cy | wide %llu steps avg %.0f cy | follow %llu runs avg %.0f cy | "
                            "wave avg %.0f cy, longest %llu cy\n", launches, (unsigned long long)len, chunk, (unsigned long long)h[7],
                            (unsigned long long)h[1], h[1] ? (double)h[0] / h[1] : 0.0, (unsigned long long)h[3], h[3] ? (double)h[2] / h[3] : 0.0,
                            (unsigned long long)h[5], h[5] ? (double)h[4] / h[5] : 0.0, h[7] ? (double)h[6] / h[7] : 0.0, (unsigned long long)h[8]);
                } else {
                    hipEvent_t ea, eb;
                    AC_HIP_CHECK(hipEventCreate(&ea)); AC_HIP_CHECK(hipEventCreate(&eb));
                    evs.push_back(ea); evs.push_back(eb);
                    flush_fills();
                    AC_HIP_CHECK(hipEventRecord(ea, 0));
                    launch_wave_kernel(insert_wave_kernel<W, false>, blocks, 0, t, tb, pb, pe, chunk, istats.ptr(), ierr, (u64*)nullptr);
                    AC_HIP_CHECK(hipEventRecord(eb, 0));
                }
#else
                launch_wave_kernel(insert_wave_kernel<W, false>, blocks, 0, t, tb, pb, pe, chunk, istats.ptr(), ierr, (u64*)nullptr);
#endif
            }
            launches++;
            pb = pe;
            phase_end.push_back(pe);
            if (launches == 2 && insert_adaptive() && pb < p_end_all && (p_end_all - pb) > 4 * first) {
                u64 probe_end = p_end_all;
#ifndef AC_EMU
                if (&pt == &loc) {
                    if (job) {
                        need_text(std::min<u64>(p_end_all, pb + (1u << 20)) + (u64)k + 8192);
                        const u64 avail = job ? std::min<u64>(job->n, job->next_wait * job->CH) : pt.n_text;
                        probe_end = std::min<u64>(p_end_all, avail > (u64)k + 64 ? avail - (u64)k - 64 : 0);
                    } else if (upload_pending) probe_end = std::min<u64>(p_end_all, upload_avail > (u64)k + 64 ? upload_avail - (u64)k - 64 : 0);
                }
#endif
                if (probe_end < pb) probe_end = pb;
                DBuf<u32> probe(2);
                probe.fill_bytes(0);
                const u64 n_probe = std::min<u64>(32768, (probe_end - pb) / 4096 + 1);
                if (probe_end > pb) launch(n_probe, RestProbeFunctor<W>{t, tb, pb, probe_end, (probe_end - pb) / n_probe, probe.ptr()});
                tm->insert_rest_sampled = (double)(probe_end - pb) / (double)(p_end_all - pb);
                std::vector<InsertStats> st2(257); u32 h_probe[2] = {0, 0};
                { ReadBatch rb; rb.add(st2.data(), istats.ptr(), 257 * sizeof(InsertStats)); rb.add(h_probe, probe.ptr(), 8); rb.run(); }
                u64 claimed = 0;
                for (size_t q = 0; q < 256; q++) claimed += st2[q].claimed;
                if (st2[256].real == 0 && claimed * 4 <= first * 5) rest_at_once = true;
                const double known = h_probe[0] ? (double)h_probe[1] / (double)h_probe[0] : 1.0;
                rest_chunk = insert_chunk_rest_env() ? insert_chunk_rest_env() : (known >= 0.9 ? 16384 : known >= 0.6 ? 8192 : known >= 0.3 ? 4096 : 2048);
                tm->insert_rest_known = known;
                const double r2 = claimed > first ? (double)(claimed - first) / (double)first : 0.0;
                want_runs = rest_at_once && (copy_mode == 1 || (copy_mode == 2 && path_copy_pays(pt.n_text, hint, k, r2)));
                if (knobs().debug_arena) fprintf(stderr, "insert: second stretch %.4f new, one-launch rest %d, copying walk %d (mode %d)\n", r2, (int)rest_at_once, (int)want_runs, copy_mode);
            }
        }
#ifndef AC_EMU
        flush_fills();
        if (!evs.empty()) AC_HIP_CHECK(hipEventSynchronize(evs.back()));
        for (size_t i = 0; i + 1 < evs.size(); i += 2) {
            float ms = 0; AC_HIP_CHECK(hipEventElapsedTime(&ms, evs[i], evs[i + 1]));
            tm->insert_kernel_ms += ms;
        }
        for (hipEvent_t e : evs) (void)hipEventDestroy(e);
#endif
        tm->insert_launches += launches;
        std::vector<InsertStats> st = to_host(istats, 257);
        const bool ins_err = st[256].real != 0;
        const u64 full_at = ~st[256].claimed;
        st.pop_back();
        n_distinct = 0;
        u64 real = 0;
        for (auto& x : st) { n_distinct += x.claimed; real += x.real; }
        bool overflow = ins_err || (n_distinct * 10 > c * 7);
        if (!overflow) { tm->insert_real += real; tm->insert_positions += pt.n_text; break; }
        const u64 c_max = next_pow2(pt.n_bases * 4 + 1024);
        if (c >= c_max) throw DeviceError("k-mer table overflow");
        u64 want = c * 4;
        if (!ins_err) want = std::max(want, next_pow2(n_distinct * 2));
        else {
            u64 pb_full = 0, pe_full = p_end_all;
            for (u64 e : phase_end) { if (full_at < e) { pe_full = e; break; } pb_full = e; }
            const double done = std::sqrt((double)std::max<u64>(pb_full, pe_full / 4) * (double)pe_full);
            const double need = (double)c * 0.7 * (double)p_end_all / std::max(done, 1.0);
            want = std::max(want, next_pow2((u64)std::min(need * 2.0, 9.0e18)));
        }
        c = std::min(want, c_max);
        tm->insert_kernel_ms = 0; tm->insert_launches = 0;
        stream_sync();
        sl = DBuf<u64>(); sflags = DBuf<u64>();
        Arena::device().rewind(retry_mark);
    }
    if (n_distinct >= 0xFFFFFFF0ULL) throw DeviceError("too many distinct k-mers for 32-bit novel indices");
    {
        CapMemo* slot = nullptr;
        for (CapMemo& m : memo) if (m.n_text == pt.n_text && m.k == k && m.owners == memo_owners) slot = &m;
        if (!slot) slot = &memo[memo_next++ % 4];
        slot->n_text = pt.n_text; slot->k = k; slot->shift = table_shift(); slot->owners = memo_owners;
        slot->cap = (n_distinct * 2 > c && c * 2 <= next_pow2(pt.n_bases * 4 + 1024)) ? c * 2 : c;
    }
    *slots_out = std::move(sl);
    *cap_out = c;
    *n_distinct_out = n_distinct;
    *bm_out = std::move(nbm);
}

template <int W> void GraphBuilder::Impl::fragments() {
    DBuf<u64> lslots; DBuf<u64>& lbm = loc_bm; u64 lcap = 0, ln = 0;
    local_insert_of_shard = true;
    insert<W>(loc, tm->local_hint, &lslots, &lcap, &ln, &lbm);
    local_insert_of_shard = false;
    tm->n_local_distinct = ln;
    lap(&tm->insert);
    u64 nw = loc.n_text / 64 + 1;
    DBuf<u32> ns(nw + 1), ne(nw + 1), so(nw + 1), eo(nw + 1);
    ns.fill_bytes(0); ne.fill_bytes(0);
    launch(nw, RunEdgeCountFunctor{lbm.ptr(), nw, ns.ptr(), ne.ptr()});
    exclusive_scan_u32(ns.ptr(), so.ptr(), nw + 1);
    exclusive_scan_u32(ne.ptr(), eo.ptr(), nw + 1);
    u64 n_runs = read_scalar(so.ptr() + nw);
    if (n_runs != (u64)read_scalar(eo.ptr() + nw)) throw DeviceError("internal error: unbalanced novel runs");
    DBuf<u64> run_start(n_runs), run_end(n_runs);
    launch(nw, RunEdgeFillFunctor{lbm.ptr(), nw, so.ptr(), eo.ptr(), run_start.ptr(), run_end.ptr()});
    n_frags = n_runs + 2 * (u64)loc.n_seqs;
    DBuf<u64> blen(n_frags + 1);
    DBuf<u64>& fpos = frag_fpos; DBuf<u64>& boff = frag_boff;
    fpos.alloc(n_frags); boff.alloc(n_frags + 1);
    frag_meta.alloc(n_frags);
    launch(n_frags + 1, FragMetaFunctor{loc.ctx((int)k), run_start.ptr(), run_end.ptr(), n_runs, n_frags, fpos.ptr(), frag_meta.ptr(),
                                        blen.ptr(), counters.ptr() + 6});
    exclusive_scan_u64(blen.ptr(), boff.ptr(), n_frags + 1);
    frag_bytes = read_scalar(boff.ptr() + n_frags);
    {
        u32 frag_err = 0, pack_bad[2] = {0xFFFFFFFFu, 0xFFFFFFFFu};
        ReadBatch rb;
        rb.add(&frag_err, counters.ptr() + 6, 4);
        if (loc.check_alphabet && loc.pack_bad.size()) rb.add(pack_bad, loc.pack_bad.ptr(), 8);
        rb.run();
        if (loc.pack_bad.size()) loc.verify_alphabet(pack_bad);
        if (frag_err) throw DeviceError("internal error: novel run outside a sequence");
    }
    tm->n_fragments = n_frags; tm->fragment_bytes = frag_bytes;
    lap(&tm->fragments);
}

template <int W> void GraphBuilder::Impl::table() {
    PackedText& g = *G;
    check_sizes(g);
    const bool want_sib = k >= 3 && degree_flags() && (n_owners <= 1 || shard_degree_flags());
    insert<W>(g, tm->graph_hint, &slots, &cap, &N, &bm, want_sib);
    tm->table_capacity = cap;
    tm->n_distinct = N;
    lap(G == &loc ? &tm->insert : &tm->union_insert);
    const bool sib_by_pos = want_sib && n_owners <= 1;
    if (sib_by_pos) { sib.alloc(2 * (g.n_text / 64 + 2)); sib.fill_bytes(0); }
    else sib = DBuf<u64>();
    sibn = DBuf<u64>(); sib_pending = false;
    occupancy_bitmap(slots, cap, &occ, sib_by_pos ? sflags.ptr() : nullptr, sib_by_pos ? sib.ptr() : nullptr);
    if (n_owners <= 1) novel_list(N);
}

template <int W> void GraphBuilder::Impl::degrees() {
    PackedText& g = *G;
    Table tb = graph_table();
    Novel nv{bm.ptr(), wprefix.ptr()};
    kcontrib = DBuf<u32>(); pend = DBuf<u32>(); pidx = DBuf<u32>(); n_pending = n_first = 0;
    u32* kout = kinfo.ptr();
    const bool by_index = n_owners > 1 && sibn.size() != 0;
    const u64* sib_ptr = by_index ? sibn.ptr() : (sib.size() ? sib.ptr() : nullptr);
    EndSet es{nullptr, 0, nullptr, nullptr};
    if (sib_ptr && g.any_dots) {
        endset_mask = next_pow2(4 * (g.has_flags ? g.n_dotted : (u64)g.n_seqs) + 16) - 1;
        endset.alloc((endset_mask + 1) * W);
        endset.fill_bytes(0xFF);
        endset_bloom.alloc(2 * ENDSET_BLOOM_WORDS);
        endset_bloom.fill_bytes(0);
        es = EndSet{endset.ptr(), endset_mask, endset_bloom.ptr(), endset_bloom.ptr() + ENDSET_BLOOM_WORDS};
    }
    auto fill_end_set = [&] { if (es.keys) launch(2 * (u64)g.n_seqs, EndSetFunctor<W>{g.ctx((int)k), es}); };
    const u8* fflags = g.has_flags ? g.seq_flags.ptr() : nullptr;
    if (sib_ptr && degree_flags() == 1 && (!g.any_dots || es.keys)) {
        DBuf<u32> fslot;
        if (by_index) {
            pend.alloc(N + 1); pidx.alloc(N + 1);
            pend.fill_bytes_from(N * 4, 0);
            fslot.alloc((u64)g.n_seqs + 1);
            DBuf<u32> fcnt((u64)g.n_seqs + 1);
            fill_end_set();
            launch((u64)g.n_seqs + 1, FirstSlotCountFunctor{fflags, g.n_seqs, fcnt.ptr()});
            exclusive_scan_u32(fcnt.ptr(), fslot.ptr(), (u64)g.n_seqs + 1);
        }
        const Arena::Mark deg_mark = Arena::device().mark();
        DegWork wk;
        const u64 max_generic = std::min<u64>(N, 2 * ((u64)k - 1) * g.n_seqs);
        wk.rcap[0] = (u32)(N / DEG_REGIONS + N / (4 * DEG_REGIONS) + 64 * DEG_BATCH); wk.ocap[0] = N;
        wk.rcap[1] = (u32)(max_generic / DEG_REGIONS + 64 * DEG_BATCH); wk.ocap[1] = max_generic;
        if (degree_region_cap()) { wk.rcap[0] = std::min(wk.rcap[0], degree_region_cap()); wk.rcap[1] = std::min(wk.rcap[1], degree_region_cap()); }
        DBuf<u64> items(wk.words()); DBuf<u32> counts(DEG_LISTS * (DEG_REGIONS + 1));
        counts.fill_bytes(0);
        wk.items = items.ptr(); wk.counts = counts.ptr();
        if (!by_index) fill_end_set();
        const u64 n_thr = (((N + DEG_BATCH - 1) / DEG_BATCH) + 63) & ~63ULL;
        launch_full(n_thr, DegreeLightFunctor<W>{g.ctx((int)k), npos.ptr(), kinfo.ptr(), g.any_dots, bm.ptr(), sib_ptr, es, wk, N, n_thr, by_index ? 1 : 0,
                                                 by_index ? pend.ptr() : nullptr});
        DBuf<u32> kc_tmp;
        if (by_index) {
            exclusive_scan_u32(pend.ptr(), pidx.ptr(), N + 1);
            u32 hp[2];
            { ReadBatch rb; rb.add(&hp[0], pidx.ptr() + N, 4); rb.add(&hp[1], fslot.ptr() + g.n_seqs, 4); rb.run(); }
            n_pending = hp[0]; n_first = hp[1];
            kc_tmp.alloc(n_pending + n_first + 1); kc_tmp.fill_bytes(0);
            kout = kc_tmp.ptr();
        }
        launch((u64)DEG_LISTS * DEG_REGIONS * DEG_PROBE_THREADS, DegreeProbeFunctor<W>{g.ctx((int)k), tb, npos.ptr(), kout, g.any_dots, wk, es, by_index ? pidx.ptr() : nullptr});
#ifdef AC_EMU
        if (knobs().degree_diag) {
            u64 c0 = 0, c1 = 0;
            for (u32 r = 0; r <= DEG_REGIONS; r++) { c0 += wk.count(0)[r]; c1 += wk.count(1)[r]; }
            fprintf(stderr, "degree diag: N %llu, queued real %llu, generic %llu, left open %llu, any_dots %d\n", (unsigned long long)N,
                    (unsigned long long)c0, (unsigned long long)c1, (unsigned long long)n_pending, (int)g.any_dots);
        }
#endif
        if (by_index) launch(g.n_seqs, FirstFunctor<W>{g.ctx((int)k), tb, nv, kinfo.ptr(), fflags, fslot.ptr(), kc_tmp.ptr() + n_pending});
        items = DBuf<u64>(); counts = DBuf<u32>();
        const u32* kc_src = kc_tmp.ptr();
        kc_tmp = DBuf<u32>();
        Arena::device().rewind(deg_mark);
        if (by_index) {
            kcontrib.alloc(n_pending + n_first + 1);
            const u64 kc_bytes = (n_pending + n_first + 1) * 4;
            if (kcontrib.ptr() != kc_src) {
                const u8* dst_b = (const u8*)kcontrib.ptr(); const u8* src_b = (const u8*)kc_src;
                if (dst_b + kc_bytes <= src_b || src_b + kc_bytes <= dst_b) { Arena::keep_readable(kc_src, kc_bytes); copy_d2d(kcontrib.ptr(), kc_src, kc_bytes); }
                else {
                    const Arena::Mark bounce_mark = Arena::device().mark();
                    DBuf<u32> pad((u64)(src_b + kc_bytes - dst_b) / 4 + 1), bounce(n_pending + n_first + 1);
                    Arena::keep_readable(kc_src, kc_bytes);
                    copy_d2d(bounce.ptr(), kc_src, kc_bytes);
                    copy_d2d(kcontrib.ptr(), bounce.ptr(), kc_bytes);
                    stream_sync();
                    pad = DBuf<u32>(); bounce = DBuf<u32>();
                    Arena::device().rewind(bounce_mark);
                }
            }
            tm->n_degrees_open = n_pending;
            lap(&tm->degree);
            return;
        }
    } else {
        fill_end_set();
        launch(N, DegreeFunctor<W>{g.ctx((int)k), tb, npos.ptr(), kinfo.ptr(), g.any_dots, 0, bm.ptr(), sib.size() && n_owners <= 1 ? sib.ptr() : nullptr, es});
    }
    launch(g.n_seqs, FirstFunctor<W>{g.ctx((int)k), tb, nv, kout, fflags, nullptr, nullptr});
    lap(&tm->degree);
}

template <int W> void GraphBuilder::Impl::unitigs() {
    PackedText& g = *G;
    TextCtx t = g.ctx((int)k);
    Table tb = graph_table();
    Novel nv{bm.ptr(), wprefix.ptr()};
    launch(N, HeadFunctor{npos.ptr(), kinfo.ptr(), head.ptr(), N});
    inclusive_scan_u32(head.ptr(), scan.ptr(), N);
    U = read_scalar(scan.ptr() + (N - 1));
    ustart.alloc((u64)U + 1);
    int seed_keep = seed_prefix_bits();
    if (seed_keep <= 0) { int lg = 1; while ((1ULL << lg) < (u64)U) lg++; seed_keep = std::min(64, ((2 * lg + 8 + 7) / 8) * 8); }
    RadixScratch seed_rs; DBuf<u32> seed_big(1, true);
    if (seed_prefix_sort()) seed_rs.prepare(U, seed_keep);
    launch(N, UnitigStartFunctor{head.ptr(), scan.ptr(), ustart.ptr(), N});
    lap(&tm->segment);

    DBuf<MinVal<W>> umin(U);
    const int mk = minkey_variant() >= 0 ? minkey_variant() : ((W > 4 || (W >= 3 && N >= 32 * (u64)U)) ? 2 : 1);
    if (mk == 2) {
        const u64 n_waves = (N + 63) / 64;
        DBuf<MinPre> upre(U), wfirst(n_waves), wlast(n_waves);
        MinPreArgs a{t, npos.ptr(), scan.ptr(), N, upre.ptr(), wfirst.ptr(), wlast.ptr(), minkey_prefix_bases()};
        launch_wave_kernel(minpre_wave_kernel<W>, (N + 255) / 256, 0, a);
        launch(U, MinFinishFunctor<W>{t, npos.ptr(), ustart.ptr(), U, N, upre.ptr(), wfirst.ptr(), wlast.ptr(), umin.ptr()});
    } else if constexpr (W <= 4) {
        if (mk == 1) {
            const u64 n_waves = (N + 63) / 64;
            DBuf<MinVal<W>> wfirst(n_waves), wlast(n_waves);
            MinWaveArgs<W> a{t, npos.ptr(), scan.ptr(), N, umin.ptr(), wfirst.ptr(), wlast.ptr()};
            launch_wave_kernel(minkey_wave_kernel<W>, (N + 255) / 256, 0, a);
            launch(U, MinJoinFunctor<W>{ustart.ptr(), U, N, wfirst.ptr(), wlast.ptr(), umin.ptr()});
        } else {
            DBuf<MinVal<W>> vals(N); DBuf<u32> seg(N);
            launch(N, CKeyFunctor<W>{t, npos.ptr(), scan.ptr(), vals.ptr(), seg.ptr()});
            reduce_by_segment(seg.ptr(), vals.ptr(), N, umin.ptr(), U, MinOp<W>(), counters.ptr() + 3);
        }
    } else {
        DBuf<u32> umin_idx(U);
        segment_argmin(scan.ptr(), N, umin_idx.ptr(), U, MinIdxOp<W>{t, npos.ptr()}, counters.ptr() + 3);
        launch(U, UnitigMinFunctor<W>{t, npos.ptr(), umin_idx.ptr(), umin.ptr()});
    }
    lap(&tm->minkey);

    order.alloc(U);
    bool seeds_ordered = false;
    if (seed_prefix_sort()) {
        DBuf<u64> wkey(U);
        const int keep = seed_keep;
        DBuf<u32> by_prefix(U);
        launch(U, SeedPrefixFunctor<W>{umin.ptr(), (int)k, wkey.ptr(), keep, by_prefix.ptr()});
        sort_pairs_u64_u32(wkey, by_prefix, U, 64, 0, 64 - keep, &seed_rs);
        DBuf<u32> settled(U); DBuf<u32>& big = seed_big;
        const bool defer = deferred_sort_checks();
        launch(U, SeedTieFunctor<W>{by_prefix.ptr(), wkey.ptr(), U, umin.ptr(), settled.ptr(), seed_max_group(), defer ? sort_flags.ptr() : big.ptr()});
        if (defer || read_scalar(big.ptr()) == 0) {
// ... 245 lines not shown
```

### autocycler_amd/csrc/graph_tail.hip

```cpp
#include "graph_impl.hpp"

namespace ac {

[[maybe_unused]] static bool renum_two_pass() { return knobs().renum_two_pass; }
[[maybe_unused]] static u32 renum_max_group() { return knobs().renum_max_group; }
[[maybe_unused]] static void renumber_sort(DBuf<u32>& order, u32 U, const u32* len, const u64* off, const u8* seq, const u32* depth, u32* flag, bool deferred = false,
                                           RadixScratch* sc = nullptr, int len_bits = 32, bool order_is_identity = false) {
    if (U <= 1) return;
    DBuf<u32> backup(deferred && !renum_two_pass() ? 0 : U);
    if (backup.size()) copy_d2d(backup.ptr(), order.ptr(), (size_t)U * 4);
    DBuf<u64> prefix(U), key(U);
    UnitigLess less{len, off, seq, depth};
    u32 zero = 0;
    if (!renum_two_pass()) {
        if (order_is_identity) launch(U, RenumKeyPassFunctor{RenumKeyFunctor{len, off, seq, prefix.ptr()}, RenumPassFunctor{order.ptr(), len, depth, prefix.ptr(), 2, key.ptr()}});
        else {
            launch(U, RenumKeyFunctor{len, off, seq, prefix.ptr()});
            launch(U, RenumPassFunctor{order.ptr(), len, depth, prefix.ptr(), 2, key.ptr()});
        }
        sort_pairs_u64_u32(key, order, U, 32 + std::min(std::max(len_bits, 1), 32), 0, 0, sc);
        launch(U, RenumTieFunctor{order.ptr(), U, len, depth, prefix.ptr(), less, flag, 0, renum_max_group()});
#ifdef AC_EMU
        if (knobs().degree_diag) {
            u64 groups = 0, members = 0, biggest = 0, cur = 1, longest = 0;
// ... 361 lines not shown
        {
            ReadBatch rb;
            rb.add(&final_total, noff.ptr() + U, 8);
            rb.add(&min_neg, lens3.ptr() + (u64)U * 3, 4);
            rb.add(&n_cand_owned, owned_count.ptr(), 4);
            rb.run();
        }
        passes = -min_neg;
        if (final_total > seq_alt.size()) throw DeviceError("internal error: merged sequences longer than before expand_repeats");
        const u32 per = 16;
        launch((final_total + per - 1) / per, MergeSeqFunctor{e, fown.ptr(), gpre.ptr(), gpost.ptr(), m.my_owner, lens3.ptr(), noff.ptr(), U, final_total, alt, per});
        stream_sync();
        m.tail_xchg(alt, final_total, 0, 0);
        launch(U, ExpResetFunctor{e, noff.ptr(), coff.ptr(), clen.ptr()});
        std::swap(cur, alt);
        e.cur = cur;
    }

    void send_sequences() {
        if (!want_graph) return;
        const u32 U = m.U;
        out->seq_block = PinnedPool::get().alloc(final_total + 64);
        const u64 other_late = (u64)U * 28 + n_links * sizeof(Link);
        if (seq_codes_transfer() == 2 || (seq_codes_transfer() == 1 && final_total >= ((u64)32 << 20) && final_total > 2 * other_late)) {
            const u64 nw = (final_total + 31) / 32;
            seq_words.alloc(nw); seq_bad.alloc(1); seq_bad.fill_bytes(0);
            launch(nw, SeqPack2Functor{cur, final_total, seq_words.ptr(), seq_bad.ptr()});
            seq_words_block = PinnedPool::get().alloc(nw * 8);
            side.after_main();
            copy_d2h_async(seq_words_block.p, seq_words.ptr(), nw * 8, side.stream());
            seq_job.words = (const u64*)seq_words_block.p; seq_job.out = (u8*)out->seq_block.p; seq_job.total = final_total;
            seq_job.landed = side.mark(); seq_job.side = &side;
#ifndef AC_EMU
            AC_HIP_CHECK(hipGetDevice(&seq_job.dev));
            seq_expand_start(seq_job, 12);
#endif
            seq_as_codes = true;
        } else {
            side.after_main();
            copy_d2h_async(out->seq_block.p, cur, final_total, side.stream());
        }
    }

    void finalise_records() {
        const u32 U = m.U;
        order2.alloc(U);
        copy_d2d(order2.ptr(), order1.ptr(), (size_t)U * 4);
        renumber_sort(order2, U, clen.ptr(), coff.ptr(), cur, m.depth.ptr(), defer_sorts ? m.sort_flags.ptr() + 1 : renum_flag.ptr(), defer_sorts, &sort2, len_bits);
        number_len.alloc(U); number_len_text.alloc(U); loff.alloc((u64)U + 1);
        number_only.alloc(host_numbers ? U : 0);
        meta.alloc((size_t)U * 24);
        u64* d_seq_begin = (u64*)meta.ptr();
        double* d_depth = (double*)(meta.ptr() + (size_t)U * 8);
        u32* d_seq_len = (u32*)(meta.ptr() + (size_t)U * 16);
        u32* d_seed_index = (u32*)(meta.ptr() + (size_t)U * 20);
        out->k = m.k;
        out->n_kmers = 2 * (u64)m.N;
        out->n_unitigs = U;
        late_by_host = late_copies() == 2 || (late_copies() == 1 && final_total + (u64)U * 28 + n_links * sizeof(Link) >= ((u64)256 << 20));
        launch(U, FinalMetaFunctor{order2.ptr(), coff.ptr(), clen.ptr(), m.depth.ptr(), lcnt.ptr(), number_len.ptr(), d_seq_begin, d_depth,
                                   d_seq_len, lcount.ptr(), host_numbers ? number_only.ptr() : nullptr, d_seed_index, m.order.ptr(), number_len_text.ptr(), m.uorient.ptr()});
        if (host_numbers) {
            number_block = PinnedPool::get().alloc((size_t)U * 4);
            remap_job.path = (int32_t*)out->path_block.p; remap_job.n_ent = m.n_ent;
            if (host_stretch) { remap_job.rec_val = (const int32_t*)rec_val_block.p; remap_job.rec_pos = (const u32*)rec_pos_block.p; remap_job.n_rec = n_stretch; }
            remap_job.number = (const u32*)number_block.p; remap_job.n_unitigs = U;
            remap_job.ent_limit = host_stretch ? (u64)stretch_split_wave * remap_block() : ~0ULL;
            const u32* d_number_only = number_only.ptr();
            const int remap_threads = (int)(host_stretch ? 2 * upload_threads() : upload_threads());
            late_copy([this, U, d_number_only, remap_threads]() {
                copy_d2h_async(number_block.p, d_number_only, (size_t)U * 4, side.stream());
                remap_job.landed = side.mark(); remap_job.side = &side;
#ifndef AC_EMU
                AC_HIP_CHECK(hipGetDevice(&remap_job.dev));
                path_remap_start(remap_job, remap_threads);
#endif
            });
        }
        if (want_graph) {
            out->meta_block = PinnedPool::get().alloc((size_t)U * 24);
            const u8* d_meta = meta.ptr();
            late_copy([this, U, d_meta]() { copy_d2h_async(out->meta_block.p, d_meta, (size_t)U * 24, side.stream()); });
        }
        exclusive_scan_u64(lcount.ptr(), loff.ptr(), (u64)U + 1);
        links_out.alloc(n_links);
        launch(U, LinkOutFunctor{order2.ptr(), L, number_len.ptr(), loff.ptr(), links_out.ptr()});
        if (want_graph) {
            out->links_block = PinnedPool::get().alloc(n_links * sizeof(Link));
            const Link* d_links_out = links_out.ptr();
            late_copy([this, d_links_out]() { copy_d2h_async(out->links_block.p, d_links_out, n_links * sizeof(Link), side.stream()); });
        }
    }

    void finalise_paths() {
        const u64 n_ent = m.n_ent;
        if (host_numbers) {
            const u64 RB = remap_block();
            const u64 n_waves = (n_ent + RB - 1) / RB;
            const u64 w_split = host_stretch ? std::min<u64>(stretch_split_wave, n_waves) : n_waves;
            if (w_split) launch_full(w_split * 64, RemapFunctor{m.ent_val.ptr(), number_len_text.ptr(), m.path_off.ptr(), n_seqs, n_ent, sums.ptr(), 0, (u32)RB, nullptr, false});
            if (w_split < n_waves) {
                const u64 n_chunks = 4, per_chunk = std::max<u64>((n_waves - w_split + n_chunks - 1) / n_chunks, 64);
                for (u64 w = w_split; w < n_waves; w += per_chunk) {
                    const u64 cnt = std::min<u64>(per_chunk, n_waves - w);
                    launch_full(cnt * 64, RemapFunctor{m.ent_val.ptr(), number_len_text.ptr(), m.path_off.ptr(), n_seqs, n_ent, sums.ptr(), w, (u32)RB, nullptr, true});
                    const u64 b = w * RB, e2 = std::min<u64>((w + cnt) * RB, n_ent);
                    const int32_t* d_ent = m.ent_val.ptr();
                    late_copy([this, d_ent, b, e2]() { copy_d2h_async((int32_t*)out->path_block.p + b, d_ent + b, (e2 - b) * 4, side.stream()); });
                }
            }
        } else {
            if (want_paths) out->path_block = PinnedPool::get().alloc(n_ent * 4);
            const u64 RB = remap_block();
            const u64 n_waves = (n_ent + RB - 1) / RB;
            const u64 n_chunks = n_ent * 4 >= ((u64)256 << 20) ? 8 : 4;
            const u64 per_chunk = std::max<u64>((n_waves + n_chunks - 1) / n_chunks, 64);
            int turn = 0;
            for (u64 w = 0; w < n_waves; w += per_chunk) {
                u64 cnt = std::min<u64>(per_chunk, n_waves - w);
                launch_full(cnt * 64, RemapFunctor{m.ent_val.ptr(), number_len_text.ptr(), m.path_off.ptr(), n_seqs, n_ent, sums.ptr(), w, (u32)RB, nullptr, true});
                if (want_paths) {
                    u64 b = w * RB, e2 = std::min<u64>((w + cnt) * RB, n_ent);
                    const int which = n_chunks == 8 ? (turn++ & 1) : 0;
                    side.after_main(which);
                    copy_d2h_async((int32_t*)out->path_block.p + b, m.ent_val.ptr() + b, (e2 - b) * 4, side.stream(which));
                }
            }
        }
        issue_late_copies();
        m.lap(&m.tm->finalize);
    }

    void collect_and_check() {
        const u32 U = m.U; const u64 n_ent = m.n_ent;
        PackedText& loc = m.loc;
        std::vector<u64> h_sums(n_seqs);
        out->path_off.resize((size_t)n_seqs + 1);
        std::vector<u32> errs(8);
        u32 pack_bad[2] = {0xFFFFFFFFu, 0xFFFFFFFFu};
        u32 h_sort_flags[2] = {0, 0};
        u64 n_links_check = 0, final_total_read = 0; u32 h_seq_bad = 0;
        {
            ReadBatch rb;
            rb.add(h_sums.data(), sums.ptr(), (size_t)n_seqs * 8);
            rb.add(out->path_off.data(), m.path_off.ptr(), ((size_t)n_seqs + 1) * 8);
            rb.add(errs.data(), m.counters.ptr(), 8 * 4);
            rb.add(h_sort_flags, m.sort_flags.ptr(), 8);
            rb.add(&n_links_check, loff.ptr() + U, 8);
            if (final_total_pending) rb.add(&final_total_read, noff.ptr() + U, 8);
            if (loc.check_alphabet && loc.pack_bad.size()) rb.add(pack_bad, loc.pack_bad.ptr(), 8);
            if (seq_as_codes) rb.add(&h_seq_bad, seq_bad.ptr(), 4);
            rb.run();
        }
        const double t_main_done = now_s();
        side.sync();
        const double t_copies_done = now_s();
        if (seq_as_codes) {
#ifdef AC_EMU
            for (u64 b = 0; b < final_total; b += 4096) seq_expand_range(seq_job.words, seq_job.out, b, std::min<u64>(b + 4096, final_total));
#endif
            seq_expand_finish(seq_job);
            if (seq_job.ready.load() == 3) throw DeviceError("internal error: the sequence codes did not reach the host");
            if (h_seq_bad) {
                copy_d2h_async(out->seq_block.p, cur, final_total, side.stream());
                side.sync();
            }
        }
        if (host_numbers) {
#ifdef AC_EMU
            if (host_stretch) { for (u64 b = 0; b < n_stretch; b += 7) path_stretch_range(remap_job, b, std::min<u64>(b + 7, n_stretch), &remap_job.bad); }
            else path_remap_range(remap_job.path, n_ent, remap_job.number, U, &remap_job.bad);
#endif
            path_remap_finish(remap_job);
        }
        m.tm->path_stretches = host_stretch ? n_stretch : 0;
        if (knobs().debug_arena && seq_as_codes)
            fprintf(stderr, "d2h: sequence codes: job started %.3f ms before stream 0 drained, its codes had landed %.3f ms after that start, %.1f MB written out in %.3f ms more\n",
                    (t_main_done - seq_job.t_start.load()) * 1e3, (seq_job.t_ready.load() - seq_job.t_start.load()) * 1e3, final_total / 1e6, (seq_job.t_last.load() - seq_job.t_ready.load()) * 1e3);
        if (knobs().debug_arena && host_numbers)
            fprintf(stderr, "d2h: the host's renumbering threads started %.3f ms %s stream 0 drained (their table had landed) and were done %.3f ms later\n",
                    std::fabs(remap_job.t_ready.load() - t_main_done) * 1e3, remap_job.t_ready.load() < t_main_done ? "before" : "after", (remap_job.t_last.load() - remap_job.t_ready.load()) * 1e3);
        if (knobs().debug_arena)
            fprintf(stderr, "d2h: copies landed %.3f ms after stream 0 drained, host renumbering done %.3f ms later; late results %.1f MB (sequences %.1f, unitig records %.1f, links %.1f, number table %.1f), entries %.1f MB\n",
                    (t_copies_done - t_main_done) * 1e3, (now_s() - t_copies_done) * 1e3, (final_total + (double)U * 24 + n_links * sizeof(Link) + (host_numbers ? (double)U * 4 : 0)) / 1e6,
                    final_total / 1e6, (double)U * 24 / 1e6, n_links * sizeof(Link) / 1e6, host_numbers ? (double)U * 4 / 1e6 : 0.0, n_ent * 4 / 1e6);
        if (loc.pack_bad.size()) loc.verify_alphabet(pack_bad);
        if (errs[7] & 128u) throw NeedExactPositions();
        if (h_sort_flags[0] || h_sort_flags[1]) {
            if (!m.deferred_sort_checks()) throw DeviceError("internal error: a sort flag was left set by a checked sort");
            throw NeedCheckedSorts();
        }
        if (errs[7]) throw DeviceError("internal error: expand_repeats pool overflow");
        if (n_links_check != n_links) throw DeviceError("internal error: link counts disagree");
        if (final_total_pending) { if (final_total_read > final_total) throw DeviceError("internal error: expand_repeats lengthened the sequences"); final_total = final_total_read; }
        if (errs[3] || errs[4])
            throw DeviceError("internal error: inconsistent unitig ends (codes " + std::to_string(errs[3]) + "/" + std::to_string(errs[4]) + ")");
        if (remap_job.bad.load()) throw DeviceError("internal error: path entries without a unitig");
        if (want_graph) {
            out->seq_begin = (const u64*)out->meta_block.p;
            out->depth = (const double*)((const u8*)out->meta_block.p + (size_t)U * 8);
            out->seq_len = (const u32*)((const u8*)out->meta_block.p + (size_t)U * 16);
            out->seed_index = (const u32*)((const u8*)out->meta_block.p + (size_t)U * 20);
            out->links = (const Link*)out->links_block.p;
        }
        if (want_paths) out->path = (const int32_t*)out->path_block.p;
        out->n_links = n_links;
        out->n_path = n_ent;
        u64 n_self = errs[5];
        u64 links_one_way = (n_links + n_self) / 2;
        out->pre = GraphStats{U, links_one_way, total};
        out->post = GraphStats{U, links_one_way, final_total};
        out->simplify_passes = passes;
        for (u32 s = 0; s < n_seqs; s++)
            if (h_sums[s] != (u64)loc.h_len[s])
                throw DeviceError("internal error: path length mismatch for sequence " + std::to_string(s + 1));
        m.lap(&m.tm->d2h);
        m.tm->total_device = now_s() - m.t_begin;
        m.tm->launches = rt_counters().launches; m.tm->readbacks = rt_counters().readbacks;
        if (knobs().debug_arena)
            fprintf(stderr, "arena: used %.1f MB (peak %.1f) of %.1f MB (n_text %.1f MB), %.3f s in hipMalloc / hipFree so far\n", Arena::device().total_used() / 1e6,
                    Arena::device().peak() / 1e6, Arena::device().capacity() / 1e6, loc.n_text / 1e6, Arena::device().alloc_seconds());
    }
};

}

void GraphBuilder::Impl::tail(FinalGraph* out, bool want_graph, bool want_paths) {
    TailRun run(*this, out, want_graph, want_paths);
    run.run();
}

void tail_warm() {
#ifndef AC_EMU
    hipLaunchKernelGGL((expand_wave_kernel<16>), dim3(1), dim3(256), 0, 0, ExpState{}, (const u32*)nullptr, (u64)0, (u64)0, 0u, (u32*)nullptr);
    (void)hipGetLastError();
#endif
}

}
```

### autocycler_amd/csrc/graph_upload.hip

```cpp
#include "upload_rt.hpp"

namespace ac {

#ifndef AC_EMU
template <int UNUSED> __global__ void __launch_bounds__(256) bar_selftest_kernel(const u64* p, u64 n, u64* out) {
    u64 acc = 0;
    for (u64 i = (u64)blockIdx.x * 256 + threadIdx.x; i < n; i += (u64)gridDim.x * 256) acc += p[i] * (i + 1);
    if (acc) atomicAdd((unsigned long long*)out, (unsigned long long)acc);
}
static bool bar_selftest(int dev) {
    const u64 n = (u64)1 << 17;
    u64* d = nullptr; u64* d_out = nullptr;
    bool ok = false;
    int fd = -1;
    do {
        if (hipSetDevice(dev) != hipSuccess) break;
        if (hipMalloc((void**)&d, n * 8) != hipSuccess || hipMalloc((void**)&d_out, 8) != hipSuccess) break;
        if (hipMemset(d, 0, n * 8) != hipSuccess || hipMemset(d_out, 0, 8) != hipSuccess || hipDeviceSynchronize() != hipSuccess) break;
        fd = ::open("/dev/zero", O_RDONLY);
        if (fd < 0) break;
        if (::read(fd, (void*)d, 4096) != 4096 || ::read(fd, (void*)(d + n - 512), 4096) != 4096) break;
        u64 expect = 0;
        for (u64 i = 0; i < n; i++) { const u64 v = (i * 0x9E3779B97F4A7C15ULL) | 1ULL; d[i] = v; expect += v * (i + 1); }
#if defined(__x86_64__)
// ... 68 lines not shown
        }
        bits[g] = w;
        if (mask) mask[g] = m;
        nonbase += (u64)__builtin_popcount(m);
    }
    return nonbase;
}
#if defined(__x86_64__)
}
#include <immintrin.h>
namespace ac {
__attribute__((target("avx2,bmi2,popcnt"))) static u64 pack_groups_avx2(const u8* t, u64 n_groups, u64* bits, u32* mask) {
    const __m256i vA = _mm256_set1_epi8('A'), vC = _mm256_set1_epi8('C'), vG = _mm256_set1_epi8('G'), vT = _mm256_set1_epi8('T');
    const __m256i three = _mm256_set1_epi8(3);
    const u64 M = 0x0303030303030303ULL;
    u64 nonbase = 0;
    for (u64 g = 0; g < n_groups; g++) {
        const __m256i v = _mm256_loadu_si256((const __m256i*)(t + g * 32));
        const __m256i good = _mm256_or_si256(_mm256_or_si256(_mm256_cmpeq_epi8(v, vA), _mm256_cmpeq_epi8(v, vC)),
                                             _mm256_or_si256(_mm256_cmpeq_epi8(v, vG), _mm256_cmpeq_epi8(v, vT)));
        __m256i c = _mm256_and_si256(_mm256_xor_si256(_mm256_srli_epi16(v, 1), _mm256_srli_epi16(v, 2)), three);
        c = _mm256_and_si256(c, good);
        const u32 bad = ~(u32)_mm256_movemask_epi8(good);
        if (mask) mask[g] = bad;
        nonbase += (u64)__builtin_popcount(bad);
        alignas(32) u64 q[4];
        _mm256_store_si256((__m256i*)q, c);
        bits[g] = (_pext_u64(__builtin_bswap64(q[0]), M) << 48) | (_pext_u64(__builtin_bswap64(q[1]), M) << 32) |
                  (_pext_u64(__builtin_bswap64(q[2]), M) << 16) | _pext_u64(__builtin_bswap64(q[3]), M);
    }
    return nonbase;
}
__attribute__((target("avx512f,avx512bw,avx512vl,ssse3,popcnt"))) static u64 pack_groups_avx512(const u8* t, u64 n_groups, u64* bits, u32* mask) {
    const __m512i vA = _mm512_set1_epi8('A'), vC = _mm512_set1_epi8('C'), vG = _mm512_set1_epi8('G'), vT = _mm512_set1_epi8('T');
    const __m512i three = _mm512_set1_epi8(3);
    const __m512i w1 = _mm512_set1_epi16(0x0104);
    const __m512i w2 = _mm512_set1_epi32(0x00010010);
    const __m128i rev = _mm_set_epi8(8, 9, 10, 11, 12, 13, 14, 15, 0, 1, 2, 3, 4, 5, 6, 7);
    u64 g = 0, nonbase = 0;
    for (; g + 2 <= n_groups; g += 2) {
        const __m512i v = _mm512_loadu_si512((const void*)(t + g * 32));
        const __mmask64 good = _mm512_cmpeq_epi8_mask(v, vA) | _mm512_cmpeq_epi8_mask(v, vC) | _mm512_cmpeq_epi8_mask(v, vG) | _mm512_cmpeq_epi8_mask(v, vT);
        __m512i c = _mm512_and_si512(_mm512_xor_si512(_mm512_srli_epi16(v, 1), _mm512_srli_epi16(v, 2)), three);
        c = _mm512_maskz_mov_epi8(good, c);
        const __m512i n16 = _mm512_maddubs_epi16(c, w1);
        const __m512i n32 = _mm512_madd_epi16(n16, w2);
        const __m128i by = _mm_shuffle_epi8(_mm512_cvtepi32_epi8(n32), rev);
        _mm_storeu_si128((__m128i*)(bits + g), by);
        const u64 bad = ~(u64)good;
        if (mask) { mask[g] = (u32)bad; mask[g + 1] = (u32)(bad >> 32); }
        nonbase += (u64)__builtin_popcountll(bad);
    }
    if (g < n_groups) nonbase += pack_groups_avx2(t + g * 32, n_groups - g, bits + g, mask ? mask + g : nullptr);
    return nonbase;
}
#endif
static u64 pack_groups(const u8* t, u64 n_groups, u64* bits, u32* mask) {
#if defined(__x86_64__)
    static const bool simd_off = getenv("AC_PACK_SCALAR") != nullptr;
    static const bool fast = __builtin_cpu_supports("avx2") && __builtin_cpu_supports("bmi2") && !simd_off;
    static const bool wide = fast && __builtin_cpu_supports("avx512f") && __builtin_cpu_supports("avx512bw") && __builtin_cpu_supports("avx512vl") &&
                             getenv("AC_PACK_AVX2") == nullptr;
    if (wide) return pack_groups_avx512(t, n_groups, bits, mask);
    if (fast) return pack_groups_avx2(t, n_groups, bits, mask);
#endif
    return pack_groups_scalar(t, n_groups, bits, mask);
}

static void path_remap_scalar(int32_t* p, u64 n, const u32* number, u32 n_unitigs, std::atomic<u32>* bad) {
    u32 wrong = 0;
    for (u64 i = 0; i < n; i++) {
        const int32_t v = p[i];
        const u32 r = (u32)(v > 0 ? v : -v) - 1u;
        if (r >= n_unitigs) { wrong++; continue; }
        const int32_t f = (int32_t)number[r], m = v >> 31;
        p[i] = (f ^ m) - m;
    }
    if (wrong) bad->fetch_add(wrong);
}
#if defined(__x86_64__)
__attribute__((target("avx512f"))) static void path_remap_avx512(int32_t* p, u64 n, const u32* number, u32 n_unitigs, std::atomic<u32>* bad) {
    const __m512i one = _mm512_set1_epi32(1), zero = _mm512_setzero_si512(), lim = _mm512_set1_epi32((int)n_unitigs);
    u64 i = 0;
    for (; i + 16 <= n; i += 16) {
        const __m512i v = _mm512_loadu_si512((const void*)(p + i));
        const __m512i r = _mm512_sub_epi32(_mm512_abs_epi32(v), one);
        const __mmask16 ok = _mm512_cmplt_epu32_mask(r, lim);
        if (ok != 0xFFFF) { path_remap_scalar(p + i, 16, number, n_unitigs, bad); continue; }
        __m512i f = _mm512_i32gather_epi32(r, (const void*)number, 4);
        f = _mm512_mask_sub_epi32(f, _mm512_cmplt_epi32_mask(v, zero), zero, f);
        _mm512_storeu_si512((void*)(p + i), f);
    }
    path_remap_scalar(p + i, n - i, number, n_unitigs, bad);
}
#endif
void path_stretch_range(const PathRemapJob& j, u64 s0, u64 s1, std::atomic<u32>* bad) {
    u32 wrong = 0;
    const u64 AHEAD = 16;
    for (u64 s = s0; s < s1; s++) {
        if (s + AHEAD < s1) { const int64_t va = j.rec_val[s + AHEAD]; const u64 fa = (u64)(va > 0 ? va : -va) - 1; if (fa < (u64)j.n_unitigs) __builtin_prefetch(j.number + fa); }
        const int64_t v0 = j.rec_val[s];
        const u64 b = j.rec_pos[s], e = s + 1 < j.n_rec ? (u64)j.rec_pos[s + 1] : j.n_ent, len = e - b;
        if (b >= j.ent_limit) break;
        int32_t* out = j.path + b;
        if (e > j.n_ent || e <= b) { wrong++; continue; }
        if (v0 > 0) {
            const u64 first = (u64)v0 - 1;
            if (first + len > (u64)j.n_unitigs) { wrong++; continue; }
            const u32* src = j.number + first;
            for (u64 i = 0; i < len; i++) out[i] = (int32_t)src[i];
        } else {
            const u64 first = (u64)(-v0) - 1;
            if (v0 == 0 || first >= (u64)j.n_unitigs || len > first + 1) { wrong++; continue; }
            const u32* src = j.number + first;
            for (u64 i = 0; i < len; i++) out[i] = -(int32_t)*(src - i);
        }
    }
    if (wrong) bad->fetch_add(wrong);
}
static void seq_expand_scalar(const u64* words, u8* out, u64 b, u64 e) {
    for (u64 i = b; i < e; i++) out[i] = (u8)"ACGT"[(words[i >> 5] >> (2 * (i & 31))) & 3];
}
#if defined(__x86_64__)
__attribute__((target("ssse3"))) static void seq_expand_ssse3(const u64* words, u8* out, u64 b, u64 e) {
    const __m128i m3 = _mm_set1_epi8(3), lut = _mm_setr_epi8('A', 'C', 'G', 'T', 'A', 'C', 'G', 'T', 'A', 'C', 'G', 'T', 'A', 'C', 'G', 'T');
    const u8* src = (const u8*)words;
    u64 i = b;
    for (; i + 64 <= e; i += 64) {
        const __m128i v = _mm_loadu_si128((const __m128i*)(src + i / 4));
        const __m128i x0 = _mm_and_si128(v, m3), x1 = _mm_and_si128(_mm_srli_epi16(v, 2), m3), x2 = _mm_and_si128(_mm_srli_epi16(v, 4), m3), x3 = _mm_and_si128(_mm_srli_epi16(v, 6), m3);
        const __m128i a = _mm_unpacklo_epi8(x0, x1), c = _mm_unpacklo_epi8(x2, x3), d = _mm_unpackhi_epi8(x0, x1), f = _mm_unpackhi_epi8(x2, x3);
        _mm_storeu_si128((__m128i*)(out + i), _mm_shuffle_epi8(lut, _mm_unpacklo_epi16(a, c)));
        _mm_storeu_si128((__m128i*)(out + i + 16), _mm_shuffle_epi8(lut, _mm_unpackhi_epi16(a, c)));
        _mm_storeu_si128((__m128i*)(out + i + 32), _mm_shuffle_epi8(lut, _mm_unpacklo_epi16(d, f)));
        _mm_storeu_si128((__m128i*)(out + i + 48), _mm_shuffle_epi8(lut, _mm_unpackhi_epi16(d, f)));
    }
    seq_expand_scalar(words, out, i, e);
}
#endif
void seq_expand_range(const u64* words, u8* out, u64 b, u64 e) {
#if defined(__x86_64__)
    static const bool fast = __builtin_cpu_supports("ssse3") && getenv("AC_PACK_SCALAR") == nullptr;
    if (fast) { seq_expand_ssse3(words, out, b, e); return; }
#endif
    seq_expand_scalar(words, out, b, e);
}
#ifndef AC_EMU
void seq_expand_start(SeqExpandJob& j, int threads) {
    const u64 BLOCK = (u64)1 << 18;
    const int T = (int)std::max<u64>(1, std::min<u64>({(j.total + BLOCK - 1) / BLOCK, (u64)std::max(threads, 1), (u64)std::max(1u, std::thread::hardware_concurrency())}));
    SeqExpandJob* job = &j;
    j.started = true;
    j.t_start.store(now_s());
    j.ticket = UploadPool::second().start(T, [job, BLOCK] {
        int expect = 0;
        if (job->ready.compare_exchange_strong(expect, 1)) {
            if (job->side) job->side->consumed(job->landed);
            const bool ok = hipSetDevice(job->dev) == hipSuccess && hipEventSynchronize((hipEvent_t)job->landed) == hipSuccess;
            job->t_ready.store(now_s());
            job->ready.store(ok ? 2 : 3, std::memory_order_release);
        } else {
            while (job->ready.load(std::memory_order_acquire) < 2) std::this_thread::yield();
        }
        if (job->ready.load(std::memory_order_acquire) != 2) return;
        for (u64 b; (b = job->next.fetch_add(BLOCK)) < job->total;) seq_expand_range(job->words, job->out, b, std::min(b + BLOCK, job->total));
        job->t_last.store(now_s());
    });
}
void seq_expand_finish(SeqExpandJob& j) noexcept {
    if (!j.started) return;
    UploadPool::second().wait(j.ticket);
    j.started = false;
}
#else
void seq_expand_start(SeqExpandJob&, int) {}
void seq_expand_finish(SeqExpandJob&) noexcept {}
#endif
bool path_remap_is_wide() {
#if defined(__x86_64__)
    static const bool wide = __builtin_cpu_supports("avx512f") && getenv("AC_PACK_SCALAR") == nullptr && getenv("AC_PACK_AVX2") == nullptr;
    return wide;
#else
    return false;
#endif
}
void path_remap_range(int32_t* p, u64 n, const u32* number, u32 n_unitigs, std::atomic<u32>* bad) {
#if defined(__x86_64__)
    if (path_remap_is_wide() && n_unitigs < 0x7FFFFFFFu) { path_remap_avx512(p, n, number, n_unitigs, bad); return; }
#endif
    path_remap_scalar(p, n, number, n_unitigs, bad);
}
#ifndef AC_EMU
void path_remap_start(PathRemapJob& j, int threads) {
    const u64 BLOCK = (u64)1 << 15;
    const u64 work_items = j.rec_val ? (j.n_rec + 4095) / 4096 : (j.n_ent + BLOCK - 1) / BLOCK;
    const int T = (int)std::max<u64>(1, std::min<u64>({work_items, (u64)std::max(threads, 1), (u64)std::max(1u, std::thread::hardware_concurrency())}));
    PathRemapJob* job = &j;
    j.started = true;
    j.ticket = UploadPool::get().start(T, [job, BLOCK] {
        int expect = 0;
        if (job->ready.compare_exchange_strong(expect, 1)) {
            if (job->side) job->side->consumed(job->landed);
            const bool ok = hipSetDevice(job->dev) == hipSuccess && hipEventSynchronize((hipEvent_t)job->landed) == hipSuccess;
            job->t_ready.store(now_s());
            job->ready.store(ok ? 2 : 3, std::memory_order_release);
        } else {
            while (job->ready.load(std::memory_order_acquire) < 2) std::this_thread::yield();
        }
        if (job->ready.load(std::memory_order_acquire) != 2) { job->bad.fetch_add(1); return; }
        if (job->rec_val) {
            const u64 SB = 4096;
            for (u64 b; (b = job->next.fetch_add(SB)) < job->n_rec;) path_stretch_range(*job, b, std::min(b + SB, job->n_rec), &job->bad);
            job->t_last.store(now_s());
            return;
        }
        for (u64 b; (b = job->next.fetch_add(BLOCK)) < job->n_ent;)
            path_remap_range(job->path + b, std::min(BLOCK, job->n_ent - b), job->number, job->n_unitigs, &job->bad);
        job->t_last.store(now_s());
    });
}
void path_remap_finish(PathRemapJob& j) noexcept {
    if (!j.started) return;
    UploadPool::get().wait(j.ticket);
    j.started = false;
}
#else
void path_remap_start(PathRemapJob&, int) {}
void path_remap_finish(PathRemapJob&) noexcept {}
#endif

void pack_text_host(const uint8_t* text, uint64_t n_text, uint64_t* bits, uint32_t* mask32, bool force_scalar) {
    const u64 full = n_text / 32;
    if (force_scalar) pack_groups_scalar(text, full, bits, mask32); else pack_groups(text, full, bits, mask32);
    if (n_text % 32) {
        u8 tail[32];
        for (u64 i = 0; i < 32; i++) tail[i] = (full * 32 + i < n_text) ? text[full * 32 + i] : (u8)'$';
        if (force_scalar) pack_groups_scalar(tail, 1, bits + full, mask32 + full); else pack_groups(tail, 1, bits + full, mask32 + full);
    }
}

static u64 pack_text_groups(const std::vector<SeqView>& seqs, const std::vector<uint64_t>& off, uint32_t k, u64 n_text, u64 g0, u64 g1,
                            u64* bits, u32* mask) {
    const u64 b = g0 * 32;
    size_t lo = 0, hi = seqs.size();
    while (lo < hi) { size_t mid = (lo + hi) / 2; if (off[mid] + (u64)seqs[mid].length + k - 1 + 1 <= b) lo = mid + 1; else hi = mid; }
    size_t i = lo;
    u64 g = g0, nonbase = 0;
    auto slow = [&](u64 gg) {
        u8 tmp[32];
        const u64 tb = gg * 32, te = std::min(n_text, tb + 32);
        if (tb < te) fill_text_range(seqs, off, k, tb, te, tmp);
        for (u64 j = te > tb ? te - tb : 0; j < 32; j++) tmp[j] = '$';
        nonbase += pack_groups(tmp, 1, bits + (gg - g0), mask ? mask + (gg - g0) : nullptr);
    };
    while (g < g1) {
        while (i < seqs.size() && off[i] + (u64)seqs[i].length + k - 1 <= g * 32) i++;
        if (i >= seqs.size()) { slow(g++); continue; }
        const u64 s0 = off[i], s1 = s0 + (u64)seqs[i].length + k - 1;
        if (g * 32 < s0) { slow(g++); continue; }
        const u64 g_in = std::min(g1, s1 / 32);
        if (g_in > g) {
            nonbase += pack_groups(seqs[i].fwd + (g * 32 - s0), g_in - g, bits + (g - g0), mask ? mask + (g - g0) : nullptr);
            g = g_in;
        } else {
            slow(g++);
        }
    }
    return nonbase;
}
[[maybe_unused]] static void throw_bad_alphabet(const std::vector<SeqView>& seqs, uint32_t k, u64 expected, u64 found, u64 index_base = 0) {
    for (size_t i = 0; i < seqs.size(); i++) {
        const u64 plen = (u64)seqs[i].length + k - 1;
        u64 a = 0, b = 0;
        while (a < plen && seqs[i].fwd[a] == '.') a++;
        while (b < plen - a && seqs[i].fwd[plen - 1 - b] == '.') b++;
        for (u64 j = a; j < plen - b; j++) {
            const u8 c = seqs[i].fwd[j];
            if (c != 'A' && c != 'C' && c != 'G' && c != 'T') throw DeviceError("input sequence " + std::to_string(index_base + i + 1) + " contains non-ACGT characters");
        }
    }
    throw DeviceError("internal error: the packed text holds " + std::to_string(found) + " non-base positions, " + std::to_string(expected) + " expected");
}

void GraphBuilder::upload_packed(const std::vector<SeqView>& seqs, const std::vector<uint64_t>& off) {
    const uint32_t k = impl_->k;
    PackedText& loc = impl_->loc;
    const u64 n = loc.n_text;
    HostStager& st = HostStager::get();
    st.ensure();
    const u64 CH = upload_chunk_bytes(), SUB = (u64)1 << 20;
    const u64 SLOT_BYTES = CH / 4;
    [[maybe_unused]] const int NSLOT = std::max(1, std::min((int)((HostStager::SLOT * HostStager::NS) / SLOT_BYTES), upload_slots()));
    [[maybe_unused]] const u64 n_chunks = (n + CH - 1) / CH, subs = CH / SUB;
    [[maybe_unused]] auto chunk_len = [&](u64 c) { return std::min(n, (c + 1) * CH) - c * CH; };
#ifdef AC_EMU
    loc.pack_alloc();
    u64 nonbase = 0;
    for (u64 b = 0; b < n; b += SUB) {
        const u64 e = std::min(n, b + SUB);
        nonbase += pack_text_groups(seqs, off, k, n, b / 32, (e + 31) / 32, loc.bits.ptr() + b / 32, (u32*)loc.mask.ptr() + b / 32);
    }
    const u64 expected = loc.expected_nonbase + ((n + 31) / 32 * 32 - n);
    if (nonbase != expected) throw_bad_alphabet(seqs, k, expected, nonbase, loc.index_base);
    {
        DBuf<u64> derived(loc.mask.size());
        derived.fill_bytes(0xFF);
        memset(derived.ptr(), 0, (size_t)((n + 63) / 64) * 8);
        launch((u64)loc.n_seqs + 1, MaskTableFunctor{loc.seq_off.ptr(), loc.seq_len.ptr(), loc.seq_d1.ptr(), loc.seq_d2.ptr(), loc.n_seqs, (int)k, n, derived.ptr()});
        if (memcmp(derived.ptr(), loc.mask.ptr(), loc.mask.size() * 8) != 0) throw DeviceError("internal error: the mask plane derived from the sequence table differs from the packed one");
    }
#else
    Impl::UploadJob* job = new Impl::UploadJob();
    impl_->job = job;
    job->seqs = &seqs; job->off = off; job->k = k; job->n = n; job->CH = CH; job->SUB = SUB; job->NSLOT = NSLOT; job->n_chunks = n_chunks;
    job->slot_bytes = SLOT_BYTES;
    job->stager = &st;
    job->expected_nonbase = loc.expected_nonbase + ((n + 31) / 32 * 32 - n);
    AC_HIP_CHECK(hipGetDevice(&job->dev));
    job->up = st.stream(); job->pk = st.pack_stream();
    flush_fills();
    AC_HIP_CHECK(hipEventRecord(st.begin(), 0));
    AC_HIP_CHECK(hipStreamWaitEvent(job->pk, st.begin(), 0));
    loc.pack_alloc(job->pk);
    AC_HIP_CHECK(hipMemsetAsync(loc.mask.ptr(), 0, (size_t)((n + 63) / 64) * 8, job->pk));
    launch((u64)loc.n_seqs + 1, MaskTableFunctor{loc.seq_off.ptr(), loc.seq_len.ptr(), loc.seq_d1.ptr(), loc.seq_d2.ptr(), loc.n_seqs, (int)k, n, loc.mask.ptr()}, job->pk);
    AC_HIP_CHECK(hipEventRecord(st.copied(), job->pk));
    AC_HIP_CHECK(hipStreamWaitEvent(job->up, st.copied(), 0));
    job->d_bits = loc.bits.ptr();
    {
        job->direct = upload_direct_for(job->dev);
        if (!job->direct) st.ensure_ring();
        job->fills_done = st.copied();
        if (job->direct) AC_HIP_CHECK(hipStreamWaitEvent(0, st.copied(), 0));
        job->t_start = now_s();
    }
    job->done = std::vector<std::atomic<u32>>(n_chunks); job->slot_state = std::vector<std::atomic<u32>>(n_chunks);
    job->issued = std::vector<std::atomic<u32>>(n_chunks);
    for (u64 c = 0; c < n_chunks; c++) { job->done[c].store(0); job->slot_state[c].store(0); job->issued[c].store(0); }
    job->landed.assign(n_chunks, nullptr);
    if (!job->direct) for (auto& e : job->landed) AC_HIP_CHECK(hipEventCreateWithFlags(&e, hipEventDisableTiming));
    const int T = (int)std::max<u64>(1, std::min<u64>({(n + SUB - 1) / SUB, upload_threads(), (u64)std::max(1u, std::thread::hardware_concurrency())}));
    job->ticket = UploadPool::get().start(T, [job] { job->run(); });
    if (!upload_overlap()) { impl_->need_text(n); impl_->finish_upload(); }
#endif
    loc.packed = true;
}

#ifndef AC_EMU
void GraphBuilder::Impl::UploadJob::run() {
    HostStager& st = *(HostStager*)stager;
    const u64 subs = CH / SUB;
    auto chunk_len = [&](u64 c) { return std::min(n, (c + 1) * CH) - c * CH; };
    auto slot_bits = [&](int sl) { return (u64*)(st.slot(0) + (u64)sl * slot_bytes); };
    try {
        AC_HIP_CHECK(hipSetDevice(dev));
        for (u64 item; (item = next.fetch_add(1)) < n_chunks * subs && !stop.load();) {
            const u64 c = item / subs, sub = item % subs;
            const u64 clen = chunk_len(c);
            if (sub * SUB >= clen) continue;
            if (direct) {
                const u64 b = c * CH + sub * SUB, e = std::min(c * CH + clen, b + SUB);
                if (e >= n) AC_HIP_CHECK(hipEventSynchronize(fills_done));
                u64* dst = d_bits + b / 32;
                const u64 ng = (e + 31) / 32 - b / 32;
                nonbase.fetch_add(pack_text_groups(*seqs, off, k, n, b / 32, (e + 31) / 32, dst, nullptr), std::memory_order_relaxed);
#if defined(__x86_64__)
                _mm_sfence();
#endif
                std::atomic_thread_fence(std::memory_order_release);
                if (ng) { const volatile u64* back = dst + (ng - 1); bar_sink.fetch_xor(*back, std::memory_order_relaxed); }
                const u32 n_sub = (u32)((clen + SUB - 1) / SUB);
                if (done[c].fetch_add(1, std::memory_order_acq_rel) + 1 == n_sub) {
                    issued[c].store(1, std::memory_order_release);
                    if (chunks_issued.fetch_add(1) + 1 == n_chunks) t_last.store(now_s());
                }
                continue;
            }
            const int sl = (int)(c % (u64)NSLOT);
            if (c >= (u64)NSLOT) {
                u32 expect = 0;
                if (slot_state[c].compare_exchange_strong(expect, 1)) {
                    while (!issued[c - NSLOT].load(std::memory_order_acquire) && !stop.load()) std::this_thread::yield();
                    if (!stop.load()) AC_HIP_CHECK(hipEventSynchronize(landed[c - NSLOT]));
                    slot_state[c].store(2, std::memory_order_release);
                } else {
                    while (slot_state[c].load(std::memory_order_acquire) != 2 && !stop.load()) std::this_thread::yield();
                }
                if (stop.load()) break;
            }
            const u64 b = c * CH + sub * SUB, e = std::min(c * CH + clen, b + SUB);
            nonbase.fetch_add(pack_text_groups(*seqs, off, k, n, b / 32, (e + 31) / 32, slot_bits(sl) + sub * SUB / 32, nullptr),
                              std::memory_order_relaxed);
            const u32 n_sub = (u32)((clen + SUB - 1) / SUB);
            if (done[c].fetch_add(1, std::memory_order_acq_rel) + 1 == n_sub) {
                const u64 g0 = c * CH / 32, ng = (clen + 31) / 32;
                std::lock_guard<std::mutex> lock(hip_mu);
                AC_HIP_CHECK(hipMemcpyAsync(d_bits + g0, slot_bits(sl), ng * 8, hipMemcpyHostToDevice, up));
                AC_HIP_CHECK(hipEventRecord(landed[c], up));
                issued[c].store(1, std::memory_order_release);
            }
        }
    } catch (const std::exception& ex) {
        std::lock_guard<std::mutex> lock(hip_mu);
        if (fail.empty()) fail = ex.what();
        stop.store(true);
    }
}
void GraphBuilder::Impl::need_text(u64 upto) {
    if (!job) return;
    while (job->next_wait < job->n_chunks && job->next_wait * job->CH < upto) {
        const u64 c = job->next_wait;
        while (!job->issued[c].load(std::memory_order_acquire) && !job->stop.load()) std::this_thread::yield();
        if (job->stop.load()) finish_upload();
        if (!job->direct) {
            flush_fills();
            AC_HIP_CHECK(hipStreamWaitEvent(0, job->landed[c], 0));
        }
        job->next_wait++;
    }
    if (job->next_wait == job->n_chunks) finish_upload();
}
u64 GraphBuilder::Impl::upload_rest_limit(u64 pb) const {
    if (!job) return ~0ULL;
    for (u64 c = job->next_wait; c < job->n_chunks; c++) {
        const u64 end = std::min(job->n, (c + 1) * job->CH);
        if (c + 1 == job->n_chunks) break;
        if (end > pb + (u64)k + 8192 + (1u << 20)) return end - (u64)k - 8192;
    }
    return ~0ULL;
}
void GraphBuilder::Impl::finish_upload() {
    if (!job) return;
    UploadJob* j = job;
    job = nullptr;
    UploadPool::get().wait(j->ticket);
    HostStager& st = HostStager::get();
    std::string fail = j->fail;
    if (fail.empty() && j->direct) {
        st.direct_ms = j->t_last.load() > 0 ? (j->t_last.load() - j->t_start) * 1e3 : -1.0;
    } else if (fail.empty()) {
        if (hipEventRecord(st.done(), j->up) != hipSuccess) fail = "hipEventRecord failed";
        st.timed = true;
    } else { (void)hipStreamSynchronize(j->up); (void)hipStreamSynchronize(j->pk); }
    if (fail.empty() && !j->stop.load() && j->nonbase.load() != j->expected_nonbase) {
        try { throw_bad_alphabet(*j->seqs, j->k, j->expected_nonbase, j->nonbase.load(), loc.index_base); } catch (const std::exception& ex) { fail = ex.what(); }
    }
    for (auto& e : j->landed) if (e) (void)hipEventDestroy(e);
    delete j;
    if (!fail.empty()) throw DeviceError(fail);
}
GraphBuilder::Impl::~Impl() {
    if (job) { job->stop.store(true); try { finish_upload(); } catch (...) {} }
}
#else
void GraphBuilder::Impl::need_text(u64) {}
u64 GraphBuilder::Impl::upload_rest_limit(u64) const { return ~0ULL; }
void GraphBuilder::Impl::finish_upload() {}
GraphBuilder::Impl::~Impl() {}
#endif

void GraphBuilder::set_sequences_host(const std::vector<SeqView>& seqs, bool pack_now) {
    const double t0 = now_s();
    const uint32_t k = impl_->k;
    const size_t S = seqs.size();
    std::vector<uint64_t> off(S); std::vector<uint32_t> len(S); std::vector<uint16_t> d1(S), d2(S);
    u64 n = 1;
    for (size_t i = 0; i < S; i++) {
        const u64 plen = (u64)seqs[i].length + k - 1;
        off[i] = n; len[i] = seqs[i].length;
        u16 a = 0, b = 0;
        while (a < plen && seqs[i].fwd[a] == '.') a++;
        while (b < plen && seqs[i].fwd[plen - 1 - b] == '.') b++;
        d1[i] = a; d2[i] = b;
        n += plen + 1;
    }
    PackedText& loc = impl_->loc;
    loc.n_text = n;
    if (pack_now && host_pack()) {
        Arena::device().reserve(arena_estimate(n, false));
        loc.d_text = nullptr;
        loc.check_alphabet = false;
        loc.set_table(off, len, d1, d2);
        upload_packed(seqs, off);
        tm_.h2d = now_s() - t0;
        return;
    }
    Arena::device().reserve(arena_estimate(n, true));
    impl_->text_owned.alloc(n + 64);
    loc.d_text = impl_->text_owned.ptr();
    loc.set_table(off, len, d1, d2);
    HostStager& st = HostStager::get();
    st.ensure();
    st.ensure_ring();
    const u64 C = HostStager::SLOT;
    const u64 n_chunks = (n + C - 1) / C;
    u8* const d_text = impl_->text_owned.ptr();
#ifdef AC_EMU
    if (pack_now) loc.pack_alloc();
    for (u64 c = 0; c < n_chunks; c++) {
        const u64 b = c * C, e = std::min(n, b + C);
        fill_text_range(seqs, off, k, b, e, st.slot(0));
        memcpy(d_text + b, st.slot(0), e - b);
        if (pack_now) launch((e - b + 31) / 32, PackFunctor{d_text, n, loc.bits.ptr(), (u32*)loc.mask.ptr(), b / 32, loc.chk()});
    }
#else
    int dev = 0;
    AC_HIP_CHECK(hipGetDevice(&dev));
    hipStream_t up = st.stream(), pk = st.pack_stream();
    {
        flush_fills();
        AC_HIP_CHECK(hipEventRecord(st.begin(), 0));
        AC_HIP_CHECK(hipStreamWaitEvent(up, st.begin(), 0));
        AC_HIP_CHECK(hipStreamWaitEvent(pk, st.begin(), 0));
    }
    if (pack_now) loc.pack_alloc(pk);
    std::atomic<u64> next{0};
    std::vector<std::atomic<u64>> issued(HostStager::NS);
    for (auto& x : issued) x.store(0);
    std::mutex hip_mu;
    std::string fail;
    std::atomic<bool> stop{false};
    auto worker = [&] {
        try {
            AC_HIP_CHECK(hipSetDevice(dev));
            for (u64 c; (c = next.fetch_add(1)) < n_chunks;) {
                const int sl = (int)(c % HostStager::NS);
                if (c >= (u64)HostStager::NS) {
                    while (issued[sl].load(std::memory_order_acquire) != c - HostStager::NS + 1 && !stop.load()) std::this_thread::yield();
                    if (stop.load()) break;
                    AC_HIP_CHECK(hipEventSynchronize(st.event(sl)));
                }
                const u64 b = c * C, e = std::min(n, b + C);
                fill_text_range(seqs, off, k, b, e, st.slot(sl));
                {
                    std::lock_guard<std::mutex> lock(hip_mu);
                    AC_HIP_CHECK(hipMemcpyAsync(d_text + b, st.slot(sl), e - b, hipMemcpyHostToDevice, up));
                    AC_HIP_CHECK(hipEventRecord(st.event(sl), up));
                    if (pack_now) {
                        AC_HIP_CHECK(hipStreamWaitEvent(pk, st.event(sl), 0));
                        launch((e - b + 31) / 32, PackFunctor{d_text, n, loc.bits.ptr(), (u32*)loc.mask.ptr(), b / 32, loc.chk()}, pk);
                    }
                }
                issued[sl].store(c + 1, std::memory_order_release);
            }
        } catch (const std::exception& ex) {
            std::lock_guard<std::mutex> lock(hip_mu);
            if (fail.empty()) fail = ex.what();
            next.store(n_chunks);
            stop.store(true);
        }
    };
    const int T = (int)std::min<u64>(n_chunks, std::min<u64>(upload_threads(), 8));
    std::vector<std::thread> pool;
    for (int i = 1; i < T; i++) pool.emplace_back(worker);
    worker();
    for (auto& t : pool) t.join();
    if (!fail.empty()) { (void)hipStreamSynchronize(up); (void)hipStreamSynchronize(pk); throw DeviceError(fail); }
    AC_HIP_CHECK(hipEventRecord(st.copied(), up));
    AC_HIP_CHECK(hipStreamWaitEvent(pk, st.copied(), 0));
    AC_HIP_CHECK(hipEventRecord(st.done(), pk));
    AC_HIP_CHECK(hipStreamWaitEvent(0, st.done(), 0));
    st.timed = true;
#endif
    loc.packed = pack_now;
    tm_.h2d = now_s() - t0;
}

}
```

### autocycler_amd/csrc/upload_rt.hpp

```cpp
#pragma once
#include "graph_impl.hpp"

namespace ac {

#ifndef AC_EMU
class UploadPool {
  public:
    static UploadPool& get() { return ctx_object<UploadPool>(CTX_POOL); }
    static UploadPool& second() { return ctx_object<UploadPool>(CTX_POOL2); }
    UploadPool() {}
    u64 start(int n, std::function<void()> fn) {
        std::unique_lock<std::mutex> lock(mu_);
        while ((int)threads_.size() < n) { const int idx = (int)threads_.size(); threads_.emplace_back([this, idx] { loop(idx); }); }
        fn_ = std::move(fn); want_ = n; active_ = n; gen_++;
        cv_.notify_all();
        return gen_;
    }
    void wait(u64 ticket) {
        std::unique_lock<std::mutex> lock(mu_);
        done_cv_.wait(lock, [&] { return gen_ != ticket || active_ == 0; });
    }
    ~UploadPool() {
        { std::unique_lock<std::mutex> lock(mu_); stop_ = true; cv_.notify_all(); }
        for (auto& t : threads_) t.join();
    }
  private:
    void loop(int idx) {
        u64 seen = 0;
        for (;;) {
            std::function<void()> fn;
            {
                std::unique_lock<std::mutex> lock(mu_);
                cv_.wait(lock, [&] { return stop_ || gen_ != seen; });
                if (stop_) return;
                seen = gen_;
                if (idx >= want_) continue;
                fn = fn_;
            }
            fn();
            std::unique_lock<std::mutex> lock(mu_);
            if (--active_ == 0) done_cv_.notify_all();
        }
    }
    std::mutex mu_; std::condition_variable cv_, done_cv_;
    std::vector<std::thread> threads_;
    std::function<void()> fn_;
    u64 gen_ = 0; int want_ = 0, active_ = 0; bool stop_ = false;
};
#endif

class HostStager {
  public:
    static const size_t SLOT = (size_t)16 << 20;
    static const int NS = 12;
    static HostStager& get() { return ctx_object<HostStager>(CTX_STAGER); }
    HostStager() {}
    ~HostStager() { release(); }
    void ensure() {
#ifndef AC_EMU
        int dev = 0;
        AC_HIP_CHECK(hipGetDevice(&dev));
        if (created_ && dev == dev_) return;
        if (created_) {
            (void)hipStreamDestroy(s_); (void)hipStreamDestroy(pk_);
            for (auto& e : ev_) (void)hipEventDestroy(e);
            (void)hipEventDestroy(done_); (void)hipEventDestroy(begin_); (void)hipEventDestroy(copied_); (void)hipEventDestroy(first_);
            created_ = false;
        }
        AC_HIP_CHECK(hipStreamCreateWithFlags(&s_, hipStreamNonBlocking));
        AC_HIP_CHECK(hipStreamCreateWithFlags(&pk_, hipStreamNonBlocking));
        for (auto& e : ev_) AC_HIP_CHECK(hipEventCreateWithFlags(&e, hipEventDisableTiming));
        AC_HIP_CHECK(hipEventCreate(&done_));
        AC_HIP_CHECK(hipEventCreate(&begin_));
        AC_HIP_CHECK(hipEventCreateWithFlags(&copied_, hipEventDisableTiming));
        AC_HIP_CHECK(hipEventCreateWithFlags(&first_, hipEventDisableTiming));
        created_ = true; dev_ = dev;
#else
        if (!ring_) ring_ = (u8*)malloc(SLOT * NS);
#endif
    }
    void release() {
#ifndef AC_EMU
        if (ring_) (void)hipHostFree(ring_);
#else
        free(ring_);
#endif
        ring_ = nullptr;
    }
    u8* slot(int i) {
#ifndef AC_EMU
        if (!ring_) AC_HIP_CHECK(hipHostMalloc((void**)&ring_, SLOT * NS, hipHostMallocDefault));
#endif
        return ring_ + (size_t)i * SLOT;
    }
    void ensure_ring() { (void)slot(0); }
#ifndef AC_EMU
    hipStream_t stream() { return s_; }
    hipStream_t pack_stream() { return pk_; }
    hipEvent_t& event(int i) { return ev_[i]; }
    hipEvent_t& done() { return done_; }
    hipEvent_t& begin() { return begin_; }
    hipEvent_t& copied() { return copied_; }
    hipEvent_t& first() { return first_; }
    bool timed = false;
    double direct_ms = -1;
#else
    stream_t stream() { return 0; }
#endif
  private:
    u8* ring_ = nullptr;
    bool created_ = false;
    int dev_ = -1;
#ifndef AC_EMU
    hipStream_t s_ = nullptr, pk_ = nullptr;
    hipEvent_t ev_[NS];
    hipEvent_t done_, begin_, copied_, first_;
#endif
};
void ensure_host_stager();

}
```

Before: 87710.

## Restructure packed-text upload with a chunk ledger, spinning pool, and split tail

Replaces the ad hoc upload chunk bookkeeping with a ChunkLedger that splits the last chunk into several units, so insert work can start on partial tail data. The upload thread pool now spin-waits briefly for new jobs and can be pre-armed, which cuts the wakeup latency of condition variables. Insert-kernel timing events are pooled and read at a later sync point, so the insert loop no longer blocks on an event synchronize. Host timestamp marks are added for diagnostics. The cost is spinning CPU threads and more complex synchronisation between upload and insert.

```diff
diff --git a/autocycler_amd/csrc/capi.cpp b/autocycler_amd/csrc/capi.cpp
--- a/autocycler_amd/csrc/capi.cpp
+++ b/autocycler_amd/csrc/capi.cpp
@@ -4,6 +4,7 @@
 
 #include "capi_common.hpp"
 #include "gfa_writer.hpp"
+#include "upload_sched.hpp"
 
 using namespace ac;
 using namespace ac::abi;
@@ -176,6 +177,8 @@
 
 int ac_compress_build(uint32_t k, uint32_t assembly_count, const ac_seq_view* seqs, uint32_t n_seqs, int device,
                       ac_graph** out) {
+    host_marks().reset();
+    host_marks().entry = steady_now_s();
     return guarded([&] {
         validate(k, seqs, n_seqs);
         DeviceCall call(device);
@@ -185,6 +188,8 @@
         b.set_sequences_host(v);
         build_graph(b, assembly_count, h.get());
         *out = h.release();
+        host_marks().ret = steady_now_s();
+        host_marks_print();
     });
 }
 
diff --git a/autocycler_amd/csrc/device_rt.hpp b/autocycler_amd/csrc/device_rt.hpp
--- a/autocycler_amd/csrc/device_rt.hpp
+++ b/autocycler_amd/csrc/device_rt.hpp
@@ -97,7 +97,7 @@
     return p ? *p : *process_wide;
 }
 inline void set_device_ctx(DeviceCtx* c) { tl_device_ctx() = c; }
-enum { CTX_ARENA = 0, CTX_FILLS, CTX_MAILBOX, CTX_SIDE, CTX_SCRATCH, CTX_STAGER, CTX_POOL, CTX_SCANPOOL_RESERVED, CTX_POOL2 };
+enum { CTX_ARENA = 0, CTX_FILLS, CTX_MAILBOX, CTX_SIDE, CTX_SCRATCH, CTX_STAGER, CTX_POOL, CTX_SCANPOOL_RESERVED, CTX_POOL2, CTX_INSERT_TIMER };
 template <class T> T& ctx_object(int slot) {
     DeviceCtx& c = device_ctx();
     if (!c.obj[slot]) { c.obj[slot] = new T(); c.del[slot] = [](void* p) { delete (T*)p; }; }
diff --git a/autocycler_amd/csrc/graph_build.hpp b/autocycler_amd/csrc/graph_build.hpp
--- a/autocycler_amd/csrc/graph_build.hpp
+++ b/autocycler_amd/csrc/graph_build.hpp
@@ -118,7 +118,8 @@
   private:
     void build_union_impl(uint32_t rank, uint32_t n_shards, const uint8_t* d_union_text, const void* d_staged_words, const uint64_t* first_word,
                           const uint64_t* n_words, uint64_t n_union_text, const void* d_meta, uint64_t n_frags_total);
-    void upload_packed(const std::vector<SeqView>& seqs, const std::vector<uint64_t>& off);
+    void upload_packed(const std::vector<SeqView>& seqs, const std::vector<uint64_t>& off, const std::vector<uint32_t>& len,
+                       const std::vector<uint16_t>& d1, const std::vector<uint16_t>& d2);
     Impl* impl_;
     BuildTimings tm_;
 };
@@ -217,6 +218,8 @@
 
 void pack_text_host(const uint8_t* text, uint64_t n_text, uint64_t* bits, uint32_t* mask32, bool force_scalar);
 
+void host_marks_print();
+
 void release_host_stager();
 
 int max_supported_k();
diff --git a/autocycler_amd/csrc/graph_impl.hpp b/autocycler_amd/csrc/graph_impl.hpp
--- a/autocycler_amd/csrc/graph_impl.hpp
+++ b/autocycler_amd/csrc/graph_impl.hpp
@@ -18,6 +18,7 @@
 #endif
 
 #include "device_rt.hpp"
+#include "upload_sched.hpp"
 
 namespace ac {
 
@@ -274,6 +275,8 @@
     u32 degree_region_cap;
     int upload_direct_mode;
     int upload_slots;
+    u64 upload_chunk_kb;
+    u32 upload_last_parts;
     int degree_flags;
     int table_shift;
     u64 wave_chunk_max;
@@ -323,6 +326,8 @@
         k.degree_region_cap = [&]() -> u32 { const char* e = getenv("AC_DEGREE_REGION_CAP"); int v = e ? atoi(e) : 0; return (u32)(v < 0 ? 0 : v); }();
         k.upload_direct_mode = [&]() -> int { const char* e = getenv("AC_UPLOAD_DIRECT"); return e ? (atoi(e) != 0 ? 1 : 0) : -1; }();
         k.upload_slots = [&]() -> int { const char* e = getenv("AC_UPLOAD_SLOTS"); int v = e ? atoi(e) : 1 << 20; return v < 1 ? 1 : v; }();
+        k.upload_chunk_kb = [&]() -> u64 { const char* e = getenv("AC_UPLOAD_CHUNK_KB"); const long v = e ? atol(e) : 0; return v < 4 ? 0 : (u64)std::min<long>(v, 1 << 20) & ~(u64)3; }();
+        k.upload_last_parts = [&]() -> u32 { const char* e = getenv("AC_UPLOAD_LAST_PARTS"); const int v = e ? atoi(e) : 1; return (u32)(v < 1 ? 1 : (v > 64 ? 64 : v)); }();
         k.degree_flags = [&]() -> int { const char* e = getenv("AC_DEGREE_FLAGS"); return e ? (atoi(e) != 0 ? 1 : 0) : 1; }();
         k.table_shift = [&]() -> int { const char* e = getenv("AC_TABLE_SHIFT"); if (!e) return -1; int v = atoi(e); return v < 0 ? 0 : (v > 3 ? 3 : v); }();
         k.wave_chunk_max = [&]() -> u64 { const char* e = getenv("AC_INSERT_CHUNK"); u64 x = e ? (u64)atoll(e) : 8192; return (std::max<u64>(x, 256) + 63) & ~63ULL; }();
@@ -394,8 +399,10 @@
 [[maybe_unused]] static u32 seed_max_group() { return knobs().seed_max_group; }
 [[maybe_unused]] static int seed_prefix_bits() { return knobs().seed_prefix_bits; }
 [[maybe_unused]] static u32 degree_region_cap() { return knobs().degree_region_cap; }
-[[maybe_unused]] static u64 upload_chunk_bytes() { return (u64)64 << 20; }
+[[maybe_unused]] static u64 upload_chunk_bytes() { return knobs().upload_chunk_kb ? knobs().upload_chunk_kb << 10 : (u64)64 << 20; }
 [[maybe_unused]] static int upload_direct_mode() { return knobs().upload_direct_mode; }
+[[maybe_unused]] static u64 upload_item_bytes() { return std::min<u64>((u64)1 << 20, upload_chunk_bytes() / 4); }
+[[maybe_unused]] static u32 upload_last_parts() { return knobs().upload_last_parts; }
 [[maybe_unused]] static int upload_slots() { return knobs().upload_slots; }
 [[maybe_unused]] static int degree_flags() { return knobs().degree_flags; }
 [[maybe_unused]] static int table_shift() { return knobs().table_shift; }
@@ -462,13 +469,17 @@
     void set_sums(u64 bases, u64 dotted, u64 dots) { n_bases = bases; n_dotted = dotted; any_dots = dotted ? 1 : 0; expected_nonbase = (u64)n_seqs + 1 + dots; }
     TextCtx ctx(int k) const { return TextCtx{bits.ptr(), mask.ptr(), n_text, k, seq_off.ptr(), seq_len.ptr(), seq_d1.ptr(), seq_d2.ptr(), n_seqs}; }
     bool packed = false;
-    void pack_alloc(stream_t s = 0) {
+    void pack_alloc(stream_t s = 0) { pack_reserve(); pack_fill(s); }
+    void pack_reserve() {
         u64 n_bits_words = n_text / 32 + 24, n_mask_words = n_text / 64 + 12;
         bits.alloc(n_bits_words); mask.alloc(n_mask_words);
+        if (check_alphabet) pack_bad.alloc(2);
+    }
+    void pack_fill(stream_t s = 0) {
         const u64 groups = (n_text + 31) / 32;
         bits.fill_bytes_from(groups * 8, 0, s);
         mask.fill_bytes_from(groups * 4, 0xFF, s);
-        if (check_alphabet) { pack_bad.alloc(2); pack_bad.fill_bytes(0xFF, s); }
+        if (check_alphabet) pack_bad.fill_bytes(0xFF, s);
     }
     void verify_alphabet(const u32* bad) const {
         if (!check_alphabet) return;
@@ -484,6 +495,57 @@
         launch((n_text + 31) / 32, PackFunctor{d_text, n_text, bits.ptr(), (u32*)mask.ptr(), 0, chk()});
         packed = true;
     }
+};
+
+class InsertTimer {
+  public:
+    static InsertTimer& get() { return ctx_object<InsertTimer>(CTX_INSERT_TIMER); }
+    InsertTimer() {}
+    InsertTimer(const InsertTimer&) = delete;
+    InsertTimer& operator=(const InsertTimer&) = delete;
+    ~InsertTimer() { destroy(); }
+    size_t pairs() const { return used_; }
+    void truncate(size_t n) { if (n < used_) used_ = n; }
+    void reset() { used_ = 0; }
+#ifndef AC_EMU
+    void next(hipEvent_t* a, hipEvent_t* b) {
+        int dev = 0;
+        AC_HIP_CHECK(hipGetDevice(&dev));
+        if (dev != dev_) { destroy(); dev_ = dev; }
+        while (ev_.size() < 2 * (used_ + 1)) { hipEvent_t e; AC_HIP_CHECK(hipEventCreate(&e)); ev_.push_back(e); }
+        *a = ev_[2 * used_]; *b = ev_[2 * used_ + 1];
+        used_++;
+    }
+    double settle(std::string* each = nullptr) {
+        double total = 0;
+        for (size_t i = 0; i < used_; i++) {
+            float ms = 0; AC_HIP_CHECK(hipEventElapsedTime(&ms, ev_[2 * i], ev_[2 * i + 1])); total += ms;
+            if (each) {
+                float gap = 0;
+                if (i) AC_HIP_CHECK(hipEventElapsedTime(&gap, ev_[2 * i - 1], ev_[2 * i]));
+                char buf[64]; snprintf(buf, sizeof buf, "%s%.3f (+%.3f)", i ? ", " : "", ms, gap);
+                *each += buf;
+            }
+        }
+        used_ = 0;
+        return total;
+    }
+#else
+    double settle(std::string* = nullptr) { used_ = 0; return 0; }
+#endif
+  private:
+    void destroy() {
+#ifndef AC_EMU
+        for (hipEvent_t e : ev_) (void)hipEventDestroy(e);
+        ev_.clear();
+#endif
+        used_ = 0;
+    }
+    size_t used_ = 0;
+#ifndef AC_EMU
+    std::vector<hipEvent_t> ev_;
+    int dev_ = -1;
+#endif
 };
 
 struct GraphBuilder::Impl {
@@ -523,6 +585,7 @@
     void begin(BuildTimings* t) {
         tm = t; t_begin = t0 = now_s();
         rt_counters() = RtCounters();
+        InsertTimer::get().reset();
         host_remap_allowed = false;
         counters.alloc(8); counters.fill_bytes(0);
         sort_flags.alloc(2); sort_flags.fill_bytes(0);
@@ -552,15 +615,16 @@
         hipStream_t up = nullptr, pk = nullptr;
         u64* d_bits = nullptr;
         bool direct = false;
-        double t_start = 0; std::atomic<u64> chunks_issued{0}; std::atomic<double> t_last{0};
+        double t_start = 0; std::atomic<double> t_last{0};
         hipEvent_t fills_done = nullptr;
-        std::atomic<u64> next{0}, nonbase{0}, bar_sink{0}; u64 expected_nonbase = 0;
-        std::vector<std::atomic<u32>> done, slot_state, issued;
+        std::atomic<u64> nonbase{0}, bar_sink{0}; u64 expected_nonbase = 0;
+        ChunkLedger ledger;
+        std::vector<std::atomic<u32>> slot_state;
         std::vector<hipEvent_t> landed;
-        std::mutex hip_mu; std::string fail; std::atomic<bool> stop{false};
+        std::mutex hip_mu; std::string fail;
         u64 ticket = 0;
         void* stager = nullptr;
-        u64 next_wait = 0;
+        HostMarks* marks = nullptr;
         void run();
 #endif
     };
diff --git a/autocycler_amd/csrc/graph_stages.hip b/autocycler_amd/csrc/graph_stages.hip
--- a/autocycler_amd/csrc/graph_stages.hip
+++ b/autocycler_amd/csrc/graph_stages.hip
@@ -29,6 +29,7 @@
     u64 n_distinct = 0;
     const Arena::Mark retry_mark = Arena::device().mark();
     std::vector<u64> phase_end;
+    const size_t timer_mark = InsertTimer::get().pairs();
     for (;;) {
         sl.alloc(c);
         sl.fill_bytes(0xFF);
@@ -44,7 +45,6 @@
         phase_end.clear();
         stream_sync();
 #ifndef AC_EMU
-        std::vector<hipEvent_t> evs;
         flush_fills();
 #endif
         u32 launches = 0;
@@ -96,8 +96,7 @@
                             (unsigned long long)h[5], h[5] ? (double)h[4] / h[5] : 0.0, h[7] ? (double)h[6] / h[7] : 0.0, (unsigned long long)h[8]);
                 } else {
                     hipEvent_t ea, eb;
-                    AC_HIP_CHECK(hipEventCreate(&ea)); AC_HIP_CHECK(hipEventCreate(&eb));
-                    evs.push_back(ea); evs.push_back(eb);
+                    InsertTimer::get().next(&ea, &eb);
                     flush_fills();
                     AC_HIP_CHECK(hipEventRecord(ea, 0));
                     launch_wave_kernel(insert_wave_kernel<W, false>, blocks, 0, t, tb, pb, pe, chunk, istats.ptr(), ierr, (u64*)nullptr);
@@ -116,7 +115,7 @@
                 if (&pt == &loc) {
                     if (job) {
                         need_text(std::min<u64>(p_end_all, pb + (1u << 20)) + (u64)k + 8192);
-                        const u64 avail = job ? std::min<u64>(job->n, job->next_wait * job->CH) : pt.n_text;
+                        const u64 avail = job->ledger.avail();
                         probe_end = std::min<u64>(p_end_all, avail > (u64)k + 64 ? avail - (u64)k - 64 : 0);
                     } else if (upload_pending) probe_end = std::min<u64>(p_end_all, upload_avail > (u64)k + 64 ? upload_avail - (u64)k - 64 : 0);
                 }
@@ -140,17 +139,12 @@
                 if (knobs().debug_arena) fprintf(stderr, "insert: second stretch %.4f new, one-launch rest %d, copying walk %d (mode %d)\n", r2, (int)rest_at_once, (int)want_runs, copy_mode);
             }
         }
+        tm->insert_launches += launches;
 #ifndef AC_EMU
-        flush_fills();
-        if (!evs.empty()) AC_HIP_CHECK(hipEventSynchronize(evs.back()));
-        for (size_t i = 0; i + 1 < evs.size(); i += 2) {
-            float ms = 0; AC_HIP_CHECK(hipEventElapsedTime(&ms, evs[i], evs[i + 1]));
-            tm->insert_kernel_ms += ms;
-        }
-        for (hipEvent_t e : evs) (void)hipEventDestroy(e);
-#endif
-        tm->insert_launches += launches;
+        if (job && &pt == &loc) { host_marks().last_piece = now_s(); finish_upload(); host_marks().joined = now_s(); }
+#endif
         std::vector<InsertStats> st = to_host(istats, 257);
+        if (&pt == &loc && host_marks().last_piece != 0 && host_marks().stats == 0) host_marks().stats = now_s();
         const bool ins_err = st[256].real != 0;
         const u64 full_at = ~st[256].claimed;
         st.pop_back();
@@ -171,7 +165,7 @@
             want = std::max(want, next_pow2((u64)std::min(need * 2.0, 9.0e18)));
         }
         c = std::min(want, c_max);
-        tm->insert_kernel_ms = 0; tm->insert_launches = 0;
+        InsertTimer::get().truncate(timer_mark); tm->insert_launches = 0;
         stream_sync();
         sl = DBuf<u64>(); sflags = DBuf<u64>();
         Arena::device().rewind(retry_mark);
@@ -222,6 +216,7 @@
         rb.add(&frag_err, counters.ptr() + 6, 4);
         if (loc.check_alphabet && loc.pack_bad.size()) rb.add(pack_bad, loc.pack_bad.ptr(), 8);
         rb.run();
+        tm->insert_kernel_ms += InsertTimer::get().settle();
         if (loc.pack_bad.size()) loc.verify_alphabet(pack_bad);
         if (frag_err) throw DeviceError("internal error: novel run outside a sequence");
     }
@@ -242,6 +237,7 @@
     else sib = DBuf<u64>();
     sibn = DBuf<u64>(); sib_pending = false;
     occupancy_bitmap(slots, cap, &occ, sib_by_pos ? sflags.ptr() : nullptr, sib_by_pos ? sib.ptr() : nullptr);
+    if (host_marks().stats != 0 && host_marks().first_tail == 0) host_marks().first_tail = now_s();
     if (n_owners <= 1) novel_list(N);
 }
 
diff --git a/autocycler_amd/csrc/graph_tail.hip b/autocycler_amd/csrc/graph_tail.hip
--- a/autocycler_amd/csrc/graph_tail.hip
+++ b/autocycler_amd/csrc/graph_tail.hip
@@ -537,6 +537,11 @@
             if (seq_as_codes) rb.add(&h_seq_bad, seq_bad.ptr(), 4);
             rb.run();
         }
+        {
+            std::string each;
+            m.tm->insert_kernel_ms += InsertTimer::get().settle(knobs().debug_arena ? &each : nullptr);
+            if (knobs().debug_arena) fprintf(stderr, "insert launches, ms on the device's clock (gap to the launch before): %s\n", each.c_str());
+        }
         const double t_main_done = now_s();
         side.sync();
         const double t_copies_done = now_s();
diff --git a/autocycler_amd/csrc/graph_upload.hip b/autocycler_amd/csrc/graph_upload.hip
--- a/autocycler_amd/csrc/graph_upload.hip
+++ b/autocycler_amd/csrc/graph_upload.hip
@@ -244,7 +244,7 @@
     SeqExpandJob* job = &j;
     j.started = true;
     j.t_start.store(now_s());
-    j.ticket = UploadPool::second().start(T, [job, BLOCK] {
+    j.ticket = upload_pool2().start(T, [job, BLOCK] {
         int expect = 0;
         if (job->ready.compare_exchange_strong(expect, 1)) {
             if (job->side) job->side->consumed(job->landed);
@@ -261,7 +261,7 @@
 }
 void seq_expand_finish(SeqExpandJob& j) noexcept {
     if (!j.started) return;
-    UploadPool::second().wait(j.ticket);
+    upload_pool2().wait(j.ticket);
     j.started = false;
 }
 #else
@@ -289,7 +289,7 @@
     const int T = (int)std::max<u64>(1, std::min<u64>({work_items, (u64)std::max(threads, 1), (u64)std::max(1u, std::thread::hardware_concurrency())}));
     PathRemapJob* job = &j;
     j.started = true;
-    j.ticket = UploadPool::get().start(T, [job, BLOCK] {
+    j.ticket = upload_pool().start(T, [job, BLOCK] {
         int expect = 0;
         if (job->ready.compare_exchange_strong(expect, 1)) {
             if (job->side) job->side->consumed(job->landed);
@@ -313,7 +313,7 @@
 }
 void path_remap_finish(PathRemapJob& j) noexcept {
     if (!j.started) return;
-    UploadPool::get().wait(j.ticket);
+    upload_pool().wait(j.ticket);
     j.started = false;
 }
 #else
@@ -374,18 +374,14 @@
     throw DeviceError("internal error: the packed text holds " + std::to_string(found) + " non-base positions, " + std::to_string(expected) + " expected");
 }
 
-void GraphBuilder::upload_packed(const std::vector<SeqView>& seqs, const std::vector<uint64_t>& off) {
+void GraphBuilder::upload_packed(const std::vector<SeqView>& seqs, const std::vector<uint64_t>& off, const std::vector<uint32_t>& len,
+                                 const std::vector<uint16_t>& d1, const std::vector<uint16_t>& d2) {
     const uint32_t k = impl_->k;
     PackedText& loc = impl_->loc;
     const u64 n = loc.n_text;
-    HostStager& st = HostStager::get();
-    st.ensure();
-    const u64 CH = upload_chunk_bytes(), SUB = (u64)1 << 20;
-    const u64 SLOT_BYTES = CH / 4;
-    [[maybe_unused]] const int NSLOT = std::max(1, std::min((int)((HostStager::SLOT * HostStager::NS) / SLOT_BYTES), upload_slots()));
-    [[maybe_unused]] const u64 n_chunks = (n + CH - 1) / CH, subs = CH / SUB;
-    [[maybe_unused]] auto chunk_len = [&](u64 c) { return std::min(n, (c + 1) * CH) - c * CH; };
+    const u64 CH = upload_chunk_bytes(), SUB = upload_item_bytes();
 #ifdef AC_EMU
+    loc.set_table(off, len, d1, d2);
     loc.pack_alloc();
     u64 nonbase = 0;
     for (u64 b = 0; b < n; b += SUB) {
@@ -402,37 +398,54 @@
         if (memcmp(derived.ptr(), loc.mask.ptr(), loc.mask.size() * 8) != 0) throw DeviceError("internal error: the mask plane derived from the sequence table differs from the packed one");
     }
 #else
+    HostStager& st = HostStager::get();
+    st.ensure();
+    const u64 SLOT_BYTES = CH / 4;
+    const int NSLOT = std::max(1, std::min((int)std::min<u64>((HostStager::SLOT * HostStager::NS) / SLOT_BYTES, 1u << 20), upload_slots()));
     Impl::UploadJob* job = new Impl::UploadJob();
     impl_->job = job;
-    job->seqs = &seqs; job->off = off; job->k = k; job->n = n; job->CH = CH; job->SUB = SUB; job->NSLOT = NSLOT; job->n_chunks = n_chunks;
+    job->seqs = &seqs; job->off = off; job->k = k; job->n = n; job->CH = CH; job->SUB = SUB; job->NSLOT = NSLOT;
     job->slot_bytes = SLOT_BYTES;
     job->stager = &st;
-    job->expected_nonbase = loc.expected_nonbase + ((n + 31) / 32 * 32 - n);
+    job->marks = &host_marks();
+    u64 dots = 0;
+    for (size_t i = 0; i < d1.size(); i++) dots += (u64)d1[i] + d2[i];
+    job->expected_nonbase = (u64)seqs.size() + 1 + dots + ((n + 31) / 32 * 32 - n);
     AC_HIP_CHECK(hipGetDevice(&job->dev));
     job->up = st.stream(); job->pk = st.pack_stream();
-    flush_fills();
-    AC_HIP_CHECK(hipEventRecord(st.begin(), 0));
-    AC_HIP_CHECK(hipStreamWaitEvent(job->pk, st.begin(), 0));
-    loc.pack_alloc(job->pk);
-    AC_HIP_CHECK(hipMemsetAsync(loc.mask.ptr(), 0, (size_t)((n + 63) / 64) * 8, job->pk));
-    launch((u64)loc.n_seqs + 1, MaskTableFunctor{loc.seq_off.ptr(), loc.seq_len.ptr(), loc.seq_d1.ptr(), loc.seq_d2.ptr(), loc.n_seqs, (int)k, n, loc.mask.ptr()}, job->pk);
-    AC_HIP_CHECK(hipEventRecord(st.copied(), job->pk));
-    AC_HIP_CHECK(hipStreamWaitEvent(job->up, st.copied(), 0));
+    job->fills_done = st.copied();
+    job->direct = upload_direct_for(job->dev);
+    job->ledger.init(n, CH, SUB, job->direct ? upload_last_parts() : 1);
+    const u64 n_chunks = job->ledger.n_chunks();
+    job->n_chunks = n_chunks;
+    if (!job->direct) {
+        st.ensure_ring();
+        job->slot_state = std::vector<std::atomic<u32>>(n_chunks);
+        for (u64 c = 0; c < n_chunks; c++) job->slot_state[c].store(0);
+        job->landed.assign(n_chunks, nullptr);
+        for (auto& e : job->landed) AC_HIP_CHECK(hipEventCreateWithFlags(&e, hipEventDisableTiming));
+    }
+    loc.pack_reserve();
     job->d_bits = loc.bits.ptr();
-    {
-        job->direct = upload_direct_for(job->dev);
-        if (!job->direct) st.ensure_ring();
-        job->fills_done = st.copied();
+    const int T = (int)std::max<u64>(1, std::min<u64>({(n + SUB - 1) / SUB, upload_threads(), (u64)std::max(1u, std::thread::hardware_concurrency())}));
+    job->t_start = now_s();
+    job->ticket = upload_pool().start(T, [job] { job->run(); });
+    try {
+        loc.set_table(off, len, d1, d2);
+        flush_fills();
+        AC_HIP_CHECK(hipEventRecord(st.begin(), 0));
+        AC_HIP_CHECK(hipStreamWaitEvent(job->pk, st.begin(), 0));
+        loc.pack_fill(job->pk);
+        AC_HIP_CHECK(hipMemsetAsync(loc.mask.ptr(), 0, (size_t)((n + 63) / 64) * 8, job->pk));
+        launch((u64)loc.n_seqs + 1, MaskTableFunctor{loc.seq_off.ptr(), loc.seq_len.ptr(), loc.seq_d1.ptr(), loc.seq_d2.ptr(), loc.n_seqs, (int)k, n, loc.mask.ptr()}, job->pk);
+        AC_HIP_CHECK(hipEventRecord(st.copied(), job->pk));
+        AC_HIP_CHECK(hipStreamWaitEvent(job->up, st.copied(), 0));
         if (job->direct) AC_HIP_CHECK(hipStreamWaitEvent(0, st.copied(), 0));
-        job->t_start = now_s();
-    }
-    job->done = std::vector<std::atomic<u32>>(n_chunks); job->slot_state = std::vector<std::atomic<u32>>(n_chunks);
-    job->issued = std::vector<std::atomic<u32>>(n_chunks);
-    for (u64 c = 0; c < n_chunks; c++) { job->done[c].store(0); job->slot_state[c].store(0); job->issued[c].store(0); }
-    job->landed.assign(n_chunks, nullptr);
-    if (!job->direct) for (auto& e : job->landed) AC_HIP_CHECK(hipEventCreateWithFlags(&e, hipEventDisableTiming));
-    const int T = (int)std::max<u64>(1, std::min<u64>({(n + SUB - 1) / SUB, upload_threads(), (u64)std::max(1u, std::thread::hardware_concurrency())}));
-    job->ticket = UploadPool::get().start(T, [job] { job->run(); });
+    } catch (...) {
+        job->ledger.fail();
+        throw;
+    }
+    job->ledger.open_gate();
     if (!upload_overlap()) { impl_->need_text(n); impl_->finish_upload(); }
 #endif
     loc.packed = true;
@@ -441,18 +454,18 @@
 #ifndef AC_EMU
 void GraphBuilder::Impl::UploadJob::run() {
     HostStager& st = *(HostStager*)stager;
-    const u64 subs = CH / SUB;
-    auto chunk_len = [&](u64 c) { return std::min(n, (c + 1) * CH) - c * CH; };
     auto slot_bits = [&](int sl) { return (u64*)(st.slot(0) + (u64)sl * slot_bytes); };
     try {
         AC_HIP_CHECK(hipSetDevice(dev));
-        for (u64 item; (item = next.fetch_add(1)) < n_chunks * subs && !stop.load();) {
-            const u64 c = item / subs, sub = item % subs;
-            const u64 clen = chunk_len(c);
-            if (sub * SUB >= clen) continue;
+        ChunkLedger::Item it;
+        while (ledger.take(&it)) {
+            const u64 c = it.chunk, b = it.b, e = it.e;
+            if (b == 0 && marks) marks->first_store.store(now_s());
             if (direct) {
-                const u64 b = c * CH + sub * SUB, e = std::min(c * CH + clen, b + SUB);
-                if (e >= n) AC_HIP_CHECK(hipEventSynchronize(fills_done));
+                if (e >= n) {
+                    if (!ledger.wait_gate()) break;
+                    AC_HIP_CHECK(hipEventSynchronize(fills_done));
+                }
                 u64* dst = d_bits + b / 32;
                 const u64 ng = (e + 31) / 32 - b / 32;
                 nonbase.fetch_add(pack_text_groups(*seqs, off, k, n, b / 32, (e + 31) / 32, dst, nullptr), std::memory_order_relaxed);
@@ -461,93 +474,98 @@
 #endif
                 std::atomic_thread_fence(std::memory_order_release);
                 if (ng) { const volatile u64* back = dst + (ng - 1); bar_sink.fetch_xor(*back, std::memory_order_relaxed); }
-                const u32 n_sub = (u32)((clen + SUB - 1) / SUB);
-                if (done[c].fetch_add(1, std::memory_order_acq_rel) + 1 == n_sub) {
-                    issued[c].store(1, std::memory_order_release);
-                    if (chunks_issued.fetch_add(1) + 1 == n_chunks) t_last.store(now_s());
-                }
+                if (ledger.complete(it) && ledger.announce(it.unit)) t_last.store(now_s());
                 continue;
             }
             const int sl = (int)(c % (u64)NSLOT);
             if (c >= (u64)NSLOT) {
                 u32 expect = 0;
                 if (slot_state[c].compare_exchange_strong(expect, 1)) {
-                    while (!issued[c - NSLOT].load(std::memory_order_acquire) && !stop.load()) std::this_thread::yield();
-                    if (!stop.load()) AC_HIP_CHECK(hipEventSynchronize(landed[c - NSLOT]));
+                    const bool sent = ledger.wait_announced(c - NSLOT);
+                    if (sent) AC_HIP_CHECK(hipEventSynchronize(landed[c - NSLOT]));
                     slot_state[c].store(2, std::memory_order_release);
                 } else {
-                    while (slot_state[c].load(std::memory_order_acquire) != 2 && !stop.load()) std::this_thread::yield();
+                    while (slot_state[c].load(std::memory_order_acquire) != 2 && !ledger.stopped()) std::this_thread::yield();
                 }
-                if (stop.load()) break;
+                if (ledger.stopped()) break;
             }
-            const u64 b = c * CH + sub * SUB, e = std::min(c * CH + clen, b + SUB);
-            nonbase.fetch_add(pack_text_groups(*seqs, off, k, n, b / 32, (e + 31) / 32, slot_bits(sl) + sub * SUB / 32, nullptr),
+            nonbase.fetch_add(pack_text_groups(*seqs, off, k, n, b / 32, (e + 31) / 32, slot_bits(sl) + it.sub * SUB / 32, nullptr),
                               std::memory_order_relaxed);
-            const u32 n_sub = (u32)((clen + SUB - 1) / SUB);
-            if (done[c].fetch_add(1, std::memory_order_acq_rel) + 1 == n_sub) {
-                const u64 g0 = c * CH / 32, ng = (clen + 31) / 32;
+            if (ledger.complete(it)) {
+                if (!ledger.wait_gate()) break;
+                const u64 g0 = c * CH / 32, ng = (ledger.chunk_len(c) + 31) / 32;
                 std::lock_guard<std::mutex> lock(hip_mu);
                 AC_HIP_CHECK(hipMemcpyAsync(d_bits + g0, slot_bits(sl), ng * 8, hipMemcpyHostToDevice, up));
                 AC_HIP_CHECK(hipEventRecord(landed[c], up));
-                issued[c].store(1, std::memory_order_release);
+                if (ledger.announce(it.unit)) t_last.store(now_s());
             }
         }
     } catch (const std::exception& ex) {
         std::lock_guard<std::mutex> lock(hip_mu);
         if (fail.empty()) fail = ex.what();
-        stop.store(true);
+        ledger.fail();
     }
 }
 void GraphBuilder::Impl::need_text(u64 upto) {
     if (!job) return;
-    while (job->next_wait < job->n_chunks && job->next_wait * job->CH < upto) {
-        const u64 c = job->next_wait;
-        while (!job->issued[c].load(std::memory_order_acquire) && !job->stop.load()) std::this_thread::yield();
-        if (job->stop.load()) finish_upload();
+    ChunkLedger& L = job->ledger;
+    while (L.pending_below(upto)) {
+        const u64 u = L.next_unit();
+        if (!L.wait_announced(u)) finish_upload();
         if (!job->direct) {
             flush_fills();
-            AC_HIP_CHECK(hipStreamWaitEvent(0, job->landed[c], 0));
-        }
-        job->next_wait++;
-    }
-    if (job->next_wait == job->n_chunks) finish_upload();
+            AC_HIP_CHECK(hipStreamWaitEvent(0, job->landed[u], 0));
+        }
+        L.advance();
+    }
 }
 u64 GraphBuilder::Impl::upload_rest_limit(u64 pb) const {
     if (!job) return ~0ULL;
-    for (u64 c = job->next_wait; c < job->n_chunks; c++) {
-        const u64 end = std::min(job->n, (c + 1) * job->CH);
-        if (c + 1 == job->n_chunks) break;
-        if (end > pb + (u64)k + 8192 + (1u << 20)) return end - (u64)k - 8192;
-    }
-    return ~0ULL;
+    return job->ledger.rest_limit(pb, (u64)k + 8192, (u64)1 << 20);
 }
 void GraphBuilder::Impl::finish_upload() {
     if (!job) return;
     UploadJob* j = job;
     job = nullptr;
-    UploadPool::get().wait(j->ticket);
+    upload_pool().wait(j->ticket);
     HostStager& st = HostStager::get();
     std::string fail = j->fail;
+    const bool stopped = j->ledger.stopped();
+    if (fail.empty() && stopped) fail = "the upload was abandoned";
     if (fail.empty() && j->direct) {
         st.direct_ms = j->t_last.load() > 0 ? (j->t_last.load() - j->t_start) * 1e3 : -1.0;
+        if (j->marks) j->marks->last_flush = j->t_last.load();
     } else if (fail.empty()) {
         if (hipEventRecord(st.done(), j->up) != hipSuccess) fail = "hipEventRecord failed";
         st.timed = true;
+        if (j->marks) j->marks->last_flush = j->t_last.load();
     } else { (void)hipStreamSynchronize(j->up); (void)hipStreamSynchronize(j->pk); }
-    if (fail.empty() && !j->stop.load() && j->nonbase.load() != j->expected_nonbase) {
+    if (fail.empty() && j->nonbase.load() != j->expected_nonbase) {
         try { throw_bad_alphabet(*j->seqs, j->k, j->expected_nonbase, j->nonbase.load(), loc.index_base); } catch (const std::exception& ex) { fail = ex.what(); }
     }
     for (auto& e : j->landed) if (e) (void)hipEventDestroy(e);
     delete j;
-    if (!fail.empty()) throw DeviceError(fail);
+    if (!fail.empty()) {
+        (void)hipStreamSynchronize(0);
+        throw DeviceError(fail);
+    }
+}
+void host_marks_print() {
+    const HostMarks& m = host_marks();
+    if (!knobs().debug_arena || m.entry == 0 || m.last_piece == 0) return;
+    auto us = [&](double t) { return t > 0 ? (t - m.entry) * 1e6 : -1.0; };
+    fprintf(stderr, "host marks: us from the entry of ac_compress_build: first packer store %.1f, last flush %.1f, last insert piece enqueued %.1f, packers joined %.1f, "
+            "insert statistics on the host %.1f, first kernel behind the insert enqueued %.1f, return %.1f\n",
+            us(m.first_store.load()), us(m.last_flush), us(m.last_piece), us(m.joined), us(m.stats), us(m.first_tail), us(m.ret));
 }
 GraphBuilder::Impl::~Impl() {
-    if (job) { job->stop.store(true); try { finish_upload(); } catch (...) {} }
+    if (job) { job->ledger.fail(); try { finish_upload(); } catch (...) {} }
 }
 #else
 void GraphBuilder::Impl::need_text(u64) {}
 u64 GraphBuilder::Impl::upload_rest_limit(u64) const { return ~0ULL; }
 void GraphBuilder::Impl::finish_upload() {}
+void host_marks_print() {}
 GraphBuilder::Impl::~Impl() {}
 #endif
 
@@ -555,6 +573,14 @@
     const double t0 = now_s();
     const uint32_t k = impl_->k;
     const size_t S = seqs.size();
+#ifndef AC_EMU
+    if (pack_now && host_pack() && upload_overlap()) {
+        u64 n_est = 1;
+        for (size_t i = 0; i < S; i++) n_est += (u64)seqs[i].length + k;
+        const u64 SUB = upload_item_bytes();
+        upload_pool().arm((int)std::max<u64>(1, std::min<u64>({(n_est + SUB - 1) / SUB, upload_threads(), (u64)std::max(1u, std::thread::hardware_concurrency())})));
+    }
+#endif
     std::vector<uint64_t> off(S); std::vector<uint32_t> len(S); std::vector<uint16_t> d1(S), d2(S);
     u64 n = 1;
     for (size_t i = 0; i < S; i++) {
@@ -572,8 +598,7 @@
         Arena::device().reserve(arena_estimate(n, false));
         loc.d_text = nullptr;
         loc.check_alphabet = false;
-        loc.set_table(off, len, d1, d2);
-        upload_packed(seqs, off);
+        upload_packed(seqs, off, len, d1, d2);
         tm_.h2d = now_s() - t0;
         return;
     }
diff --git a/autocycler_amd/csrc/upload_rt.hpp b/autocycler_amd/csrc/upload_rt.hpp
--- a/autocycler_amd/csrc/upload_rt.hpp
+++ b/autocycler_amd/csrc/upload_rt.hpp
@@ -4,49 +4,8 @@
 namespace ac {
 
 #ifndef AC_EMU
-class UploadPool {
-  public:
-    static UploadPool& get() { return ctx_object<UploadPool>(CTX_POOL); }
-    static UploadPool& second() { return ctx_object<UploadPool>(CTX_POOL2); }
-    UploadPool() {}
-    u64 start(int n, std::function<void()> fn) {
-        std::unique_lock<std::mutex> lock(mu_);
-        while ((int)threads_.size() < n) { const int idx = (int)threads_.size(); threads_.emplace_back([this, idx] { loop(idx); }); }
-        fn_ = std::move(fn); want_ = n; active_ = n; gen_++;
-        cv_.notify_all();
-        return gen_;
-    }
-    void wait(u64 ticket) {
-        std::unique_lock<std::mutex> lock(mu_);
-        done_cv_.wait(lock, [&] { return gen_ != ticket || active_ == 0; });
-    }
-    ~UploadPool() {
-        { std::unique_lock<std::mutex> lock(mu_); stop_ = true; cv_.notify_all(); }
-        for (auto& t : threads_) t.join();
-    }
-  private:
-    void loop(int idx) {
-        u64 seen = 0;
-        for (;;) {
-            std::function<void()> fn;
-            {
-                std::unique_lock<std::mutex> lock(mu_);
-                cv_.wait(lock, [&] { return stop_ || gen_ != seen; });
-                if (stop_) return;
-                seen = gen_;
-                if (idx >= want_) continue;
-                fn = fn_;
-            }
-            fn();
-            std::unique_lock<std::mutex> lock(mu_);
-            if (--active_ == 0) done_cv_.notify_all();
-        }
-    }
-    std::mutex mu_; std::condition_variable cv_, done_cv_;
-    std::vector<std::thread> threads_;
-    std::function<void()> fn_;
-    u64 gen_ = 0; int want_ = 0, active_ = 0; bool stop_ = false;
-};
+inline UploadPool& upload_pool() { return ctx_object<UploadPool>(CTX_POOL); }
+inline UploadPool& upload_pool2() { return ctx_object<UploadPool>(CTX_POOL2); }
 #endif
 
 class HostStager {
diff --git a/autocycler_amd/csrc/upload_sched.hpp b/autocycler_amd/csrc/upload_sched.hpp
--- /dev/null
+++ b/autocycler_amd/csrc/upload_sched.hpp
@@ -0,0 +1,186 @@
+#pragma once
+#include <algorithm>
+#include <atomic>
+#include <chrono>
+#include <condition_variable>
+#include <cstdint>
+#include <functional>
+#include <memory>
+#include <mutex>
+#include <thread>
+#include <vector>
+
+namespace ac {
+
+inline void cpu_relax() {
+#if defined(__x86_64__)
+    __builtin_ia32_pause();
+#else
+    std::this_thread::yield();
+#endif
+}
+
+class UploadPool {
+  public:
+    static constexpr int SPIN_US = 500;
+    UploadPool() {}
+    UploadPool(const UploadPool&) = delete;
+    UploadPool& operator=(const UploadPool&) = delete;
+    void arm(int n) {
+        std::unique_lock<std::mutex> lock(mu_);
+        grow(n);
+        arm_++;
+        cv_.notify_all();
+    }
+    uint64_t start(int n, std::function<void()> fn) {
+        std::unique_lock<std::mutex> lock(mu_);
+        done_cv_.wait(lock, [&] { return active_.load(std::memory_order_acquire) == 0; });
+        grow(n);
+        fn_ = std::move(fn);
+        active_.store(n, std::memory_order_relaxed);
+        gen_++;
+        job_.store((gen_ << 16) | (uint64_t)n, std::memory_order_release);
+        cv_.notify_all();
+        return gen_;
+    }
+    void wait(uint64_t ticket) {
+        std::unique_lock<std::mutex> lock(mu_);
+        done_cv_.wait(lock, [&] { return gen_ != ticket || active_.load(std::memory_order_acquire) == 0; });
+    }
+    ~UploadPool() {
+        { std::unique_lock<std::mutex> lock(mu_); stop_ = true; cv_.notify_all(); }
+        for (auto& t : threads_) t.join();
+    }
+  private:
+    void grow(int n) {
+        if (n > 0xFFFF) n = 0xFFFF;
+        while ((int)threads_.size() < n) { const int idx = (int)threads_.size(); threads_.emplace_back([this, idx] { loop(idx); }); }
+    }
+    void loop(int idx) {
+        uint64_t seen = 0, seen_arm = 0;
+        for (;;) {
+            {
+                std::unique_lock<std::mutex> lock(mu_);
+                cv_.wait(lock, [&] { return stop_ || (job_.load(std::memory_order_acquire) >> 16) != seen || arm_ != seen_arm; });
+                if (stop_) return;
+                seen_arm = arm_;
+            }
+            uint64_t j = job_.load(std::memory_order_acquire);
+            if ((j >> 16) == seen) {
+                const auto until = std::chrono::steady_clock::now() + std::chrono::microseconds(SPIN_US);
+                for (unsigned spins = 0; ((j = job_.load(std::memory_order_acquire)) >> 16) == seen; spins++) {
+                    cpu_relax();
+                    if ((spins & 63) == 63 && std::chrono::steady_clock::now() >= until) break;
+                }
+                if ((j >> 16) == seen) continue;
+            }
+            seen = j >> 16;
+            if (idx >= (int)(j & 0xFFFF)) continue;
+            fn_();
+            if (active_.fetch_sub(1, std::memory_order_acq_rel) == 1) { std::unique_lock<std::mutex> lock(mu_); done_cv_.notify_all(); }
+        }
+    }
+    std::mutex mu_; std::condition_variable cv_, done_cv_;
+    std::vector<std::thread> threads_;
+    std::function<void()> fn_;
+    std::atomic<uint64_t> job_{0};
+    std::atomic<int> active_{0};
+    uint64_t gen_ = 0, arm_ = 0; bool stop_ = false;
+};
+
+class ChunkLedger {
+  public:
+    struct Item { uint64_t chunk, sub, unit, b, e; };
+    ChunkLedger() {}
+    ChunkLedger(const ChunkLedger&) = delete;
+    ChunkLedger& operator=(const ChunkLedger&) = delete;
+    void init(uint64_t n_text, uint64_t chunk_bytes, uint64_t item_bytes, uint32_t parts) {
+        n_ = n_text; CH_ = chunk_bytes; SUB_ = item_bytes;
+        subs_ = CH_ / SUB_;
+        n_chunks_ = (n_ + CH_ - 1) / CH_;
+        const uint64_t last = n_chunks_ - 1, last_len = n_ - last * CH_, ns = (last_len + SUB_ - 1) / SUB_;
+        const uint64_t P = std::max<uint64_t>(1, std::min<uint64_t>(parts, ns));
+        n_units_ = last + P;
+        unit_end_.assign(n_units_, 0); need_.assign(n_units_, 0); part_of_sub_.assign(ns, 0);
+        for (uint64_t c = 0; c < last; c++) { unit_end_[c] = (c + 1) * CH_; need_[c] = (uint32_t)subs_; }
+        for (uint64_t p = 0; p < P; p++) {
+            const uint64_t s0 = p * ns / P, s1 = (p + 1) * ns / P;
+            for (uint64_t s = s0; s < s1; s++) part_of_sub_[s] = (uint32_t)p;
+            unit_end_[last + p] = std::min(n_, last * CH_ + s1 * SUB_);
+            need_[last + p] = (uint32_t)(s1 - s0);
+        }
+        done_.reset(new std::atomic<uint32_t>[n_units_]); announced_.reset(new std::atomic<uint32_t>[n_units_]);
+        for (uint64_t u = 0; u < n_units_; u++) { done_[u].store(0); announced_[u].store(0); }
+        next_.store(0); units_announced_.store(0); stop_.store(false); gate_.store(false);
+        next_wait_ = 0;
+    }
+    uint64_t n_text() const { return n_; }
+    uint64_t n_chunks() const { return n_chunks_; }
+    uint64_t n_units() const { return n_units_; }
+    uint64_t chunk_len(uint64_t c) const { return std::min(n_, (c + 1) * CH_) - c * CH_; }
+    uint64_t unit_begin(uint64_t u) const { return u ? unit_end_[u - 1] : 0; }
+    uint64_t unit_end(uint64_t u) const { return unit_end_[u]; }
+    bool take(Item* it) {
+        for (;;) {
+            if (stop_.load(std::memory_order_acquire)) return false;
+            const uint64_t i = next_.fetch_add(1, std::memory_order_relaxed);
+            if (i >= n_chunks_ * subs_) return false;
+            const uint64_t c = i / subs_, sub = i % subs_, clen = chunk_len(c);
+            if (sub * SUB_ >= clen) continue;
+            it->chunk = c; it->sub = sub;
+            it->b = c * CH_ + sub * SUB_; it->e = std::min(c * CH_ + clen, it->b + SUB_);
+            it->unit = c + 1 < n_chunks_ ? c : c + part_of_sub_[sub];
+            return true;
+        }
+    }
+    bool complete(const Item& it) { return done_[it.unit].fetch_add(1, std::memory_order_acq_rel) + 1 == need_[it.unit]; }
+    bool announce(uint64_t u) {
+        announced_[u].store(1, std::memory_order_release);
+        return units_announced_.fetch_add(1, std::memory_order_acq_rel) + 1 == n_units_;
+    }
+    bool is_announced(uint64_t u) const { return announced_[u].load(std::memory_order_acquire) != 0; }
+    void fail() { stop_.store(true, std::memory_order_release); }
+    bool stopped() const { return stop_.load(std::memory_order_acquire); }
+    void open_gate() { gate_.store(true, std::memory_order_release); }
+    bool wait_gate() const {
+        while (!gate_.load(std::memory_order_acquire)) { if (stopped()) return false; std::this_thread::yield(); }
+        return true;
+    }
+    bool pending_below(uint64_t upto) const { return next_wait_ < n_units_ && unit_begin(next_wait_) < upto; }
+    uint64_t next_unit() const { return next_wait_; }
+    bool wait_announced(uint64_t u) const {
+        while (!is_announced(u)) { if (stopped()) return false; std::this_thread::yield(); }
+        return true;
+    }
+    void advance() { next_wait_++; }
+    bool all_waited() const { return next_wait_ == n_units_; }
+    uint64_t avail() const { return std::min(n_, unit_begin(next_wait_)); }
+    uint64_t rest_limit(uint64_t pb, uint64_t reach, uint64_t min_piece) const {
+        for (uint64_t u = next_wait_; u + 1 < n_units_; u++)
+            if (unit_end_[u] > pb + reach + min_piece) return unit_end_[u] - reach;
+        return ~(uint64_t)0;
+    }
+  private:
+    uint64_t n_ = 0, CH_ = 1, SUB_ = 1, subs_ = 1, n_chunks_ = 0, n_units_ = 0;
+    std::vector<uint64_t> unit_end_; std::vector<uint32_t> need_, part_of_sub_;
+    std::unique_ptr<std::atomic<uint32_t>[]> done_, announced_;
+    std::atomic<uint64_t> next_{0}, units_announced_{0};
+    std::atomic<bool> stop_{false}, gate_{false};
+    uint64_t next_wait_ = 0;
+};
+
+struct HostMarks {
+    double entry = 0;
+    std::atomic<double> first_store{0};
+    double last_flush = 0;
+    double last_piece = 0;
+    double joined = 0;
+    double stats = 0;
+    double first_tail = 0;
+    double ret = 0;
+    void reset() { entry = last_flush = last_piece = joined = stats = first_tail = ret = 0; first_store.store(0); }
+};
+inline HostMarks& host_marks() { static thread_local HostMarks m; return m; }
+inline double steady_now_s() { return std::chrono::duration<double>(std::chrono::steady_clock::now().time_since_epoch()).count(); }
+
+}
```

Result: slower. 84610 (-3.5%).
